# mcdermatt/ICET

Measured on AMD Instinct MI355X. Metric: scan-pairs/sec + ms/pair, 64-ch 75x24 voxels 7 iters; HBM GB/s vs peak, higher is better.
Workload: dtype f32; 1 GPU; configs[2]/[3]: 256 independent 64-ch synthetic scan pairs per GPU (~116k pts/scan, ring-major), 75x24 voxels, 7 iters, pair k -> rank k mod N, RCCL all-gather of 48 floats/pair when N>1; pairs_per_gpu=256, pairs_total=256, points_scan1_mean=116273, points_scan2_mean=116258, bins_theta=75, bins_phi=24, iters=7, parallelism=pairs round-robin x1, processes=1, mode=one process per GPU, rccl_ranks=0

## Files before the change

icet_amd/csrc/icet_accumulate.hip:

```cpp
#include <hip/hip_runtime.h>
#include <math.h>
#include "icet_internal.h"
#include "icet_device_common.h"
#include "icet_solve_body.h"
#include <algorithm>
#include <type_traits>

namespace icet {
namespace {

#ifndef ICET_ACC_BLOCK
#define ICET_ACC_BLOCK 512
#endif
#ifndef ICET_ACC_WAVES
#define ICET_ACC_WAVES 6
#endif
#ifndef ICET_ACC_PTS
#define ICET_ACC_PTS 4
#endif
static_assert(ICET_ACC_PTS == 4, "phase C of k_gn_accumulate is written for 4 consecutive points per lane");
constexpr int kAccPts = ICET_ACC_PTS;
constexpr int kAccBlock = ICET_ACC_BLOCK;
constexpr int kAccWavesPerSimd = ICET_ACC_WAVES;
constexpr int kHotWords = 8;

__device__ __noinline__ void spill_flush(uint32_t* A, uint32_t nraw, uint32_t nin, float S0, float S1, float S2, float S3, float S4,
                                         float S5, float S6, float S7, float S8) {
    acc_add_hbm(A, nraw, nin, S0, S1, S2, S3, S4, S5, S6, S7, S8);
}

__device__ __noinline__ void flush_wide(unsigned long long* F, float a0, float a1, float a2, float a3, float a4, float a5, float a6, float a7, float a8) {
    atomicAdd(&F[1], to_fix_wide_biased(a0)); atomicAdd(&F[2], to_fix_wide_biased(a1)); atomicAdd(&F[3], to_fix_wide_biased(a2)); atomicAdd(&F[4], to_fix_wide_biased(a3));
    atomicAdd(&F[5], to_fix_wide_biased(a4)); atomicAdd(&F[6], to_fix_wide_biased(a5)); atomicAdd(&F[7], to_fix_wide_biased(a6)); atomicAdd(&F[8], to_fix_wide_biased(a7));
    atomicAdd(&F[9], to_fix_wide_biased(a8));
}

constexpr int kCntBits = 21;
constexpr unsigned long long kCntMask = (1ull << kCntBits) - 1ull;
constexpr uint32_t kNearCap = 512;
constexpr uint32_t kNearCapSmall = 2048;

typedef __attribute__((address_space(1))) const float gfloat;
typedef float vfloat4 __attribute__((ext_vector_type(4)));
typedef __attribute__((address_space(1))) const vfloat4 gfloat4;

struct KeepDev { unsigned long long* mask; const uint32_t* list; const float* edges; const int32_t* modes; float c1, c2, capT, capP, invT; };
__device__ __forceinline__ int keep_pair_of_slot(const int32_t* __restrict__ modes, int n_pairs, int s, int& mode_word) {
    const int lane = (int)(threadIdx.x & 63u);
    const int gb = s & ~255, ng = min(256, n_pairs - gb), sl = s - gb;
    int m[4];
#pragma unroll
    for (int c = 0; c < 4; c++) m[c] = (c * 64 + lane < ng) ? modes[gb + c * 64 + lane] : -1;
    int hi = 0, lo = 0x7FFFFFFF;
#pragma unroll
    for (int c = 0; c < 4; c++) { hi = max(hi, m[c]); lo = min(lo, m[c] > 0 ? m[c] : 0x7FFFFFFF); }
    hi = wave_reduce_max_i(hi); lo = wave_reduce_min_i(lo);
    const float scale = 7.999f / (float)max(hi - lo + 1, 1);
    int cls[4], cnt[9];
#pragma unroll
    for (int k = 0; k < 9; k++) cnt[k] = 0;
#pragma unroll
    for (int c = 0; c < 4; c++) {
        cls[c] = m[c] < 0 ? 9 : (m[c] == 0 ? 0 : 1 + (int)((float)(hi - m[c]) * scale));
#pragma unroll
        for (int k = 0; k < 9; k++) cnt[k] += __popcll(__ballot(cls[c] == k));
    }
    int k_of = 0, r = sl;
#pragma unroll
    for (int k = 0; k < 8; k++) { const bool past = (k_of == k) & (r >= cnt[k]); r -= past ? cnt[k] : 0; k_of += past ? 1 : 0; }
    int found = -1, word = 0;
#pragma unroll
    for (int c = 0; c < 4; c++) {
        const unsigned long long bm = __ballot(cls[c] == k_of);
        const int rk = (int)__builtin_amdgcn_mbcnt_hi((uint32_t)(bm >> 32), __builtin_amdgcn_mbcnt_lo((uint32_t)bm, 0u));
        const unsigned long long hit = __ballot(cls[c] == k_of && rk == r);
        if (found < 0 && hit != 0ull) { const int l = __builtin_ctzll(hit); found = gb + c * 64 + l; word = __builtin_amdgcn_readlane(m[c], l); }
        r -= __popcll(bm);
    }
    mode_word = word;
    return found;
}
constexpr int kKeepOwn = 63;

template <bool kVec4, bool kRT2, bool kSmall, bool kKeep, bool kIdx = false>
__device__ __forceinline__ void gn_accumulate_body(const PairDesc* __restrict__ desc, const float* __restrict__ xf_all,
                                                          const int16_t* __restrict__ slot_of_voxel, const int32_t* __restrict__ n_slots,
                                                          const SlotHot* __restrict__ hotS, uint32_t* __restrict__ acc,
                                                          const float* __restrict__ thr, const LutCell* __restrict__ lut,
                                                          int T, int P, int Mt, int Mp, float guard_t, float guard_p,
                                                          int lds_slots, int chunks, int n_pairs, int force_exact,
                                                          uint32_t* __restrict__ near_over, uint32_t* __restrict__ near_over_count, const KeepDev& kd,
                                                          const int32_t* __restrict__ kf_of = nullptr) {
    constexpr uint32_t near_cap = kSmall ? kNearCapSmall : kNearCap;
    constexpr int kW = kAccBlock / 64;
    extern __shared__ __attribute__((aligned(16))) unsigned char smem[];
    const int V = T * P;
    int pair, chunk;
    if (!decode_block(n_pairs, chunks, pair, chunk)) return;
    [[maybe_unused]] int mode_word = 0;
    if constexpr (kKeep) { pair = keep_pair_of_slot(kd.modes, n_pairs, pair, mode_word); if (pair < 0) return; }
    const PairDesc d = desc[pair];
    int cs = (d.n2 + chunks - 1) / chunks;
    cs = (cs + kAccPts * 64 - 1) / (kAccPts * 64) * (kAccPts * 64);
    const int begin = chunk * cs;
    int list_mode = 0, nk = 0, tau_begin = 0, tau_end = 0;
    if constexpr (kKeep) { list_mode = mode_word > 0; nk = mode_word - 1; }
    if (kKeep && list_mode) {
        const int n_trips = nk / kKeepOwn + 1;
        int tpb = (n_trips + chunks - 1) / chunks; tpb = (tpb + kW - 1) / kW * kW;
        tau_begin = chunk * tpb; tau_end = min(n_trips, tau_begin + tpb);
        if (tau_begin >= n_trips) return;
    } else if (begin >= d.n2) return;
    const int end = (kKeep && list_mode) ? d.n2 : min(d.n2, begin + cs);
    const int lane = (int)(threadIdx.x & 63u);
    const uint32_t* L = kd.list + ((size_t)d.off2 >> 2) + pair;
    const int e_max = max(nk - 1, 0);
    auto entry_raw = [&](int tau) -> int { return (int)L[min(max(kKeepOwn * tau - 1 + lane, 0), e_max)]; };
    auto entry_ok = [&](int tau) -> bool { return (tau < tau_end) & ((unsigned)(kKeepOwn * tau - 1 + lane) < (unsigned)nk); };
    [[maybe_unused]] int gc_first = -1, gn_first = -1;
    if (kKeep && list_mode) { gc_first = entry_raw(tau_begin + (int)(threadIdx.x >> 6)); gn_first = entry_raw(tau_begin + (int)(threadIdx.x >> 6) + kW); }

    LutCell* lut_t = reinterpret_cast<LutCell*>(smem);
    LutCell* lut_p = lut_t + (Mt + 1);
    unsigned long long* lacc = reinterpret_cast<unsigned long long*>(lut_p + (Mp + 1));
    float* hot = reinterpret_cast<float*>(smem + (((size_t)(Mt + Mp + 2) * sizeof(LutCell) + (size_t)80 * lds_slots + 15) & ~(size_t)15));
    int16_t* map = reinterpret_cast<int16_t*>(hot + lds_slots * kHotWords);
    const int map_words = (V + 1) / 2;
    uint32_t* nearq = reinterpret_cast<uint32_t*>(map) + (V + T + 4) / 2;
    [[maybe_unused]] float* k_edge_t = reinterpret_cast<float*>(nearq + near_cap + 5);
    [[maybe_unused]] float* k_edge_p = k_edge_t + (T + 2);
    [[maybe_unused]] uint8_t* k_nb = reinterpret_cast<uint8_t*>(k_edge_p + (P + 2)) + T;
    int kf = pair;
    if constexpr (kIdx) kf = __builtin_amdgcn_readfirstlane(kf_of[pair]);
    const int ns = n_slots[kf];
    const int nl = min(ns, lds_slots);
    const SlotHot* hs = hotS + (size_t)kf * V;
    {
        const uint32_t* gm = reinterpret_cast<const uint32_t*>(slot_of_voxel + (size_t)kf * ((V + 1) & ~1));
        uint32_t* lm = reinterpret_cast<uint32_t*>(map);
        const uint2* gl = reinterpret_cast<const uint2*>(lut);
        uint2* ll = reinterpret_cast<uint2*>(lut_t);
        const int n_lut = Mt + Mp + 2;
        constexpr int kMapAhead = 2, kLutAhead = 3;
        uint32_t mreg[kMapAhead]; uint2 lreg[kLutAhead];
#pragma unroll
        for (int k = 0; k < kMapAhead; k++) { const int i = (int)threadIdx.x + k * kAccBlock; mreg[k] = (i < map_words) ? gm[i] : 0u; }
#pragma unroll
        for (int k = 0; k < kLutAhead; k++) { const int i = (int)threadIdx.x + k * kAccBlock; lreg[k] = (i < n_lut) ? gl[i] : make_uint2(0u, 0u); }
        SlotHot g0{};
        if ((int)threadIdx.x < nl) g0 = hs[threadIdx.x];
#pragma unroll
        for (int k = 0; k < kMapAhead; k++) { const int i = (int)threadIdx.x + k * kAccBlock; if (i < map_words) lm[i] = mreg[k]; }
        for (int i = (int)threadIdx.x + kMapAhead * kAccBlock; i < map_words; i += kAccBlock) lm[i] = gm[i];
        for (int i = 2 * map_words + threadIdx.x; i < V + T + 2; i += kAccBlock) map[i] = (int16_t)-1;
#pragma unroll
        for (int k = 0; k < kLutAhead; k++) { const int i = (int)threadIdx.x + k * kAccBlock; if (i < n_lut) ll[i] = lreg[k]; }
        for (int i = (int)threadIdx.x + kLutAhead * kAccBlock; i < n_lut; i += kAccBlock) ll[i] = gl[i];
        for (int i = threadIdx.x; i < nl; i += kAccBlock) {
            const SlotHot g = (i == (int)threadIdx.x) ? g0 : hs[i];
            float* h = hot + i * kHotWords;
            h[0] = g.inner; h[1] = g.outer; h[2] = g.mu[0]; h[3] = g.mu[1]; h[4] = g.mu[2];
        }
        for (int i = threadIdx.x; i < 10 * nl; i += kAccBlock) lacc[i] = 0ull;
        if (threadIdx.x < 5) nearq[near_cap + threadIdx.x] = 0u;
    }
    const float* xf = xf_all + pair * kXf;
    const float tx = xf[0], ty = xf[1], tz = xf[2];
    const float R00 = xf[3], R01 = xf[4], R02 = xf[5], R10 = xf[6], R11 = xf[7], R12 = xf[8], R20 = xf[9], R21 = xf[10], R22 = xf[11];
    const float cell_t = (float)Mt * 0.25f, cell_p = (float)Mp * 0.5f;
    __syncthreads();
    if constexpr (kKeep) {
        if (!list_mode) {
            for (int i = threadIdx.x; i < T + P + 4; i += kAccBlock) {
                const int k = i < T + 2 ? i : i - (T + 2);
                k_edge_t[i] = (i < T + 2) ? kd.edges[min(k, T)] : kd.edges[T + 1 + min(k, P)];
            }
            for (int v = (int)threadIdx.x - T; v < V + 2 * T + 1; v += kAccBlock) {
                uint32_t code = 0u;
                if (v >= 0 && v < V) {
                    const int bt = v % T, r0 = v - bt;
                    code = (map[v] >= 0 ? 1u : 0u) | (map[r0 + (bt == 0 ? T - 1 : bt - 1)] >= 0 ? 2u : 0u) | (map[r0 + (bt == T - 1 ? 0 : bt + 1)] >= 0 ? 4u : 0u);
                }
                k_nb[v] = (uint8_t)code;
            }
            __syncthreads();
        }
    }

    gfloat* px = (gfloat*)d.s2; gfloat* py = px + d.ld2; gfloat* pz = px + 2 * (size_t)d.ld2;
    uint32_t* gacc = acc + (size_t)pair * V * kAccWords;

    auto load4 = [&](int i0, float (&X)[4], float (&Y)[4], float (&Z)[4]) {
        if (kVec4 && i0 + 3 < end) {
            const vfloat4 a = __builtin_nontemporal_load((gfloat4*)(px + i0)), b = __builtin_nontemporal_load((gfloat4*)(py + i0)), c = __builtin_nontemporal_load((gfloat4*)(pz + i0));
            X[0] = a.x; X[1] = a.y; X[2] = a.z; X[3] = a.w; Y[0] = b.x; Y[1] = b.y; Y[2] = b.z; Y[3] = b.w; Z[0] = c.x; Z[1] = c.y; Z[2] = c.z; Z[3] = c.w;
        } else {
#pragma unroll
            for (int j = 0; j < 4; j++) { const bool ok = i0 + j < end; X[j] = ok ? px[i0 + j] : __builtin_nanf(""); Y[j] = ok ? py[i0 + j] : 0.f; Z[j] = ok ? pz[i0 + j] : 0.f; }
        }
    };
#ifndef ICET_ACC_PHASE
#define ICET_ACC_PHASE 9
#endif
    [[maybe_unused]] float sink = 0.f;
    float XN[4], YN[4], ZN[4];
    auto trip = [&](auto mode_c, const int i0, const bool have_next, const int i0_next, [[maybe_unused]] const int grp) {
      constexpr int kMode = decltype(mode_c)::value;
      [[maybe_unused]] const bool ghost = kMode == 2 && lane == 0;
      auto flush = [&](int slot, uint32_t cr, uint32_t ci, float a0, float a1, float a2, float a3, float a4, float a5, float a6, float a7, float a8) {
          if (ICET_ACC_PHASE == 4) { sink += (float)(slot + (int)cr + (int)ci) + a0 + a1 + a2 + a3 + a4 + a5 + a6 + a7 + a8; return; }
          if (slot >= 0) {
              if (slot < nl) {
                  unsigned long long* F = lacc + slot * 10;
                  atomicAdd(&F[0], (unsigned long long)cr | ((unsigned long long)ci << kCntBits) | ((ci ? 1ull : 0ull) << (2 * kCntBits)));
                  if (ci) {
                      if (__ballot(!(fmaxf(fmaxf(a3, a6), a8) < kFixFastMax)) == 0ull) {
                          atomicAdd(&F[1], to_fix_biased(a0)); atomicAdd(&F[2], to_fix_biased(a1)); atomicAdd(&F[3], to_fix_biased(a2)); atomicAdd(&F[4], to_fix_biased(a3));
                          atomicAdd(&F[5], to_fix_biased(a4)); atomicAdd(&F[6], to_fix_biased(a5)); atomicAdd(&F[7], to_fix_biased(a6)); atomicAdd(&F[8], to_fix_biased(a7));
                          atomicAdd(&F[9], to_fix_biased(a8));
                      } else {
                          flush_wide(F, a0, a1, a2, a3, a4, a5, a6, a7, a8);
                      }
                  }
              } else {
                  spill_flush(gacc + (size_t)slot * kAccWords, cr, ci, a0, a1, a2, a3, a4, a5, a6, a7, a8);
              }
          }
      };
      {
        PointClass pc[4];
        float QX[4], QY[4], QZ[4], RR[4];
        {
            typedef float f2 __attribute__((ext_vector_type(2)));
            f2 q[6];
#pragma unroll
            for (int h = 0; h < 2; h++) {
                const f2 a = f2{XN[2 * h], XN[2 * h + 1]} + f2{tx, tx}, b = f2{YN[2 * h], YN[2 * h + 1]} + f2{ty, ty}, c = f2{ZN[2 * h], ZN[2 * h + 1]} + f2{tz, tz};
                q[3 * h + 0] = __builtin_elementwise_fma(c, f2{R20, R20}, __builtin_elementwise_fma(b, f2{R10, R10}, a * f2{R00, R00}));
                q[3 * h + 1] = __builtin_elementwise_fma(c, f2{R21, R21}, __builtin_elementwise_fma(b, f2{R11, R11}, a * f2{R01, R01}));
                q[3 * h + 2] = __builtin_elementwise_fma(c, f2{R22, R22}, __builtin_elementwise_fma(b, f2{R12, R12}, a * f2{R02, R02}));
            }
            asm volatile("" : "+v"(q[0]), "+v"(q[1]), "+v"(q[2]), "+v"(q[3]), "+v"(q[4]), "+v"(q[5]) : : "memory");
#pragma unroll
            for (int h = 0; h < 2; h++) { QX[2 * h] = q[3 * h].x; QX[2 * h + 1] = q[3 * h].y; QY[2 * h] = q[3 * h + 1].x; QY[2 * h + 1] = q[3 * h + 1].y; QZ[2 * h] = q[3 * h + 2].x; QZ[2 * h + 1] = q[3 * h + 2].y; }
        }
        if (have_next) load4(i0_next, XN, YN, ZN);
        if (ICET_ACC_PHASE == 0) { sink += (QX[0] + QX[1] + QX[2] + QX[3]) + (QY[0] + QY[1] + QY[2] + QY[3]) + (QZ[0] + QZ[1] + QZ[2] + QZ[3]); return; }
        int SM[4];
        bool nr[4];
        float R2[4];
        [[maybe_unused]] bool keep_any = false;
#pragma unroll
        for (int j = 0; j < 4; j++) {
            const float qx = QX[j], qy = QY[j], qz = QZ[j];
            const float r2 = qx * qx + qy * qy + qz * qz;
            const float rs = __builtin_amdgcn_rsqf(r2);
            RR[j] = r2 * rs;
            const float w = -qz * rs;
            const float q1 = qy * __builtin_amdgcn_rcpf(fabsf(qx) + fabsf(qy));
            const float pa = (qx >= 0.f) ? ((qy >= 0.f) ? q1 : 4.f + q1) : 2.f - q1;
            const LutCell et = lut_t[static_cast<int>(pa * cell_t)];
            const LutCell ep = lut_p[static_cast<int>((w + 1.f) * cell_p)];
            const int bt = et.idx - ((pa < et.edge) ? 1 : 0);
            const int row = ep.idx - ((w < ep.edge) ? T : 0);
            SM[j] = map[row + bt];
            nr[j] = (force_exact != 0) | !(fabsf(pa - et.edge) >= guard_t) | !(fabsf(w - ep.edge) >= guard_p);
            R2[j] = r2;
            if constexpr (kMode == 1) {
                const float irho = __builtin_amdgcn_rsqf(fmaf(qx, qx, qy * qy));
                const float Mpol = fmaf(kd.c2, rs, kd.c1), Maz = fmaf(kd.c1, RR[j], kd.c2) * irho;
                const float lo_t = k_edge_t[bt], hi_t = k_edge_t[bt + 1];
                const int bpi = static_cast<int>(fmaf((float)row, kd.invT, 0.5f));
                const float lo_p = k_edge_p[bpi], hi_p = k_edge_p[bpi + 1];
                const bool nlt = !((pa - lo_t) >= Maz), nht = !((hi_t - pa) >= Maz), nlp = !((w - lo_p) >= Mpol), nhp = !((hi_p - w) >= Mpol);
                const bool unsure = !(Maz <= kd.capT) | !(Mpol <= kd.capP) | (bt >= T) | (row >= V) | nr[j] | !((r2 >= kR2Min) & (r2 <= kR2Max));
                const int v = row + bt;
                const uint32_t c0 = k_nb[v], cm = k_nb[v - T], cp = k_nb[v + T];
                const uint32_t msk = 1u | (nlt ? 2u : 0u) | (nht ? 4u : 0u);
                const uint32_t hit = (c0 & msk) | (nlp ? (cm & msk) : 0u) | (nhp ? (cp & msk) : 0u);
                keep_any |= (i0 + j < end) & (unsure | (hit != 0u));
            }
        }
        if constexpr (kMode == 1) {
            const unsigned long long km = __ballot(keep_any);
            if (lane == 0 && i0 < end) kd.mask[((size_t)d.off2 >> 8) + pair + (i0 >> 8)] = km;
        }
#pragma unroll
        for (int j = 0; j < 4; j++) nr[j] |= !((R2[j] >= kR2Min) & (R2[j] <= kR2Max));
        const int E0 = nr[0] ? -1 : SM[0], E1 = nr[1] ? -1 : SM[1], E2 = nr[2] ? -1 : SM[2], E3 = nr[3] ? -1 : SM[3];
        if (ICET_ACC_PHASE == 1) { sink += (float)(E0 + E1 + E2 + E3) + RR[0] + RR[1] + RR[2] + RR[3] + QX[0] + QY[1] + QZ[2]; return; }
        if (__ballot((E0 & E1 & E2 & E3) >= 0) != 0ull) {
            const bool beyond = __ballot(max(max(E0, E1), max(E2, E3)) >= nl) != 0ull;
            const int E[4] = {E0, E1, E2, E3};
#pragma unroll
            for (int j = 0; j < 4; j++) {
                const int sm = E[j];
                const bool has = sm >= 0;
                const float* h = hot + min(max(sm, 0), lds_slots - 1) * kHotWords;
                float inner = h[0], outer = h[1], m0 = h[2], m1 = h[3], m2 = h[4];
                if (beyond) {
                    if (sm >= nl) { const SlotHot g = hs[sm]; inner = g.inner; outer = g.outer; m0 = g.mu[0]; m1 = g.mu[1]; m2 = g.mu[2]; }
                    asm volatile("" : "+v"(inner), "+v"(outer), "+v"(m0), "+v"(m1), "+v"(m2));
                }
                const float r = RR[j];
                const float gr = 1e-6f * r;
                const float m = fminf(r - inner, outer - r);
                const bool edge = has & !(fabsf(m) >= gr);
                nr[j] |= edge;
                pc[j].s = edge ? -1 : sm;
                pc[j].inb = has & (m >= 0.f);
                float ux = QX[j], uy = QY[j], uz = QZ[j];
                if (kRT2) { if (pc[j].inb & !edge) roundtrip_any(ux, uy, uz, ux, uy, uz); }
                pc[j].dx = ux - m0; pc[j].dy = uy - m1; pc[j].dz = uz - m2;
            }
        } else {
#pragma unroll
            for (int j = 0; j < 4; j++) { pc[j].s = -1; pc[j].inb = false; pc[j].dx = pc[j].dy = pc[j].dz = 0.f; }
        }
        if (ICET_ACC_PHASE == 2) { for (int j = 0; j < 4; j++) sink += (float)pc[j].s + pc[j].dx + pc[j].dy + pc[j].dz + (pc[j].inb ? 1.f : 0.f) + (nr[j] ? 1.f : 0.f); return; }
        if (__ballot(nr[0] | nr[1] | nr[2] | nr[3]) != 0ull) {
            if (__ballot((R2[0] == 0.f) | (R2[1] == 0.f) | (R2[2] == 0.f) | (R2[3] == 0.f)) != 0ull) {
#pragma unroll
                for (int j = 0; j < 4; j++) {
                    const bool zq = (R2[j] == 0.f) & (QX[j] == 0.f) & (QY[j] == 0.f) & (i0 + j < end);
                    const bool zc = zq & !ghost;
                    const int patt = (__builtin_signbit(QY[j]) ? 2 : 0) | (__builtin_signbit(QX[j]) ? 1 : 0);
#pragma unroll
                    for (int k = 0; k < 4; k++) {
                        const unsigned long long m = __ballot(zc & (patt == k));
                        if (m != 0ull && (threadIdx.x & 63) == 0) atomicAdd(&nearq[near_cap + 1 + k], (uint32_t)__popcll(m));
                    }
                    nr[j] &= !zq;
                }
            }
#pragma unroll
            for (int j = 0; j < 4; j++) {
                if (nr[j] & (i0 + j < end) & !ghost) {
                    const uint32_t e = atomicAdd(&nearq[near_cap], 1u);
                    if (e < near_cap) nearq[e] = (uint32_t)(i0 + j);
                    else near_over[(size_t)d.off2 + atomicAdd(&near_over_count[pair], 1u)] = (uint32_t)(i0 + j);
                }
            }
        }
        if (ICET_ACC_PHASE == 3) { for (int j = 0; j < 4; j++) sink += (float)pc[j].s + pc[j].dx + pc[j].dy + pc[j].dz + (pc[j].inb ? 1.f : 0.f); return; }
        const int s0 = pc[0].s, s1 = pc[1].s, s2 = pc[2].s, s3 = pc[3].s;
        if (__ballot((s0 >= 0) | (s1 >= 0) | (s2 >= 0) | (s3 >= 0)) == 0ull) return;
        {
            const bool e1 = s1 == s0, e2 = s2 == s1, e3 = s3 == s2;
            const bool a1 = e1, a2 = a1 & e2, a3 = a2 & e3;
            const bool z3 = !a3, z2 = z3 & e3, z1 = z2 & e2;
            const bool i0 = pc[0].inb, i1 = pc[1].inb, i2 = pc[2].inb, i3 = pc[3].inb;
            typedef float f2 __attribute__((ext_vector_type(2)));
            const uint32_t zr = 1u + (z2 ? 1u : 0u) + (z1 ? 1u : 0u);
            const uint32_t zi = (i3 ? 1u : 0u) + ((z2 & i2) ? 1u : 0u) + ((z1 & i1) ? 1u : 0u);
            bool fw = z3 & (s3 >= 0) & (wave_shl1(s0, -2) == s3);
            if constexpr (kMode == 2) fw &= (wave_shl1(grp, -7) == grp + 1) & (((grp + 1) & 63) != 0);
            const bool h1 = fw & z1 & i1, h2 = fw & z2 & i2, h3 = fw & i3;
            const float g1x = wave_shr1_zero(h1 ? pc[1].dx : 0.f), g1y = wave_shr1_zero(h1 ? pc[1].dy : 0.f), g1z = wave_shr1_zero(h1 ? pc[1].dz : 0.f);
            const float g2x = wave_shr1_zero(h2 ? pc[2].dx : 0.f), g2y = wave_shr1_zero(h2 ? pc[2].dy : 0.f), g2z = wave_shr1_zero(h2 ? pc[2].dz : 0.f);
            const float g3x = wave_shr1_zero(h3 ? pc[3].dx : 0.f), g3y = wave_shr1_zero(h3 ? pc[3].dy : 0.f), g3z = wave_shr1_zero(h3 ? pc[3].dz : 0.f);
            const uint32_t gc = (uint32_t)wave_shr1_zero((int)(fw ? (zr | (zi << 8)) : 0u));
            f2 Axy, Asq, Acz; float A2, A4, A8;
            {
                Axy = f2{g1x, g1y}; A2 = g1z; Asq = Axy * Axy; Acz = f2{g1z, g1z} * Axy; A4 = g1x * g1y; A8 = g1z * g1z;
            }
#define ICET_ACC_ADD(S, vx_, vy_, vz_)                                                                                                       \
            {                                                                                                                                \
                const f2 vxy = f2{vx_, vy_}; const float vz = vz_;                                                                           \
                S##xy += vxy; S##2 += vz;                                                                                                    \
                S##sq = __builtin_elementwise_fma(vxy, vxy, S##sq); S##cz = __builtin_elementwise_fma(vxy, f2{vz, vz}, S##cz);               \
                S##4 = fmaf(vxy.x, vxy.y, S##4); S##8 = fmaf(vz, vz, S##8);                                                                  \
            }
            ICET_ACC_ADD(A, g2x, g2y, g2z)
            ICET_ACC_ADD(A, g3x, g3y, g3z)
            { const bool m = i0;      ICET_ACC_ADD(A, m ? pc[0].dx : 0.f, m ? pc[0].dy : 0.f, m ? pc[0].dz : 0.f) }
            { const bool m = a1 & i1; ICET_ACC_ADD(A, m ? pc[1].dx : 0.f, m ? pc[1].dy : 0.f, m ? pc[1].dz : 0.f) }
            { const bool m = a2 & i2; ICET_ACC_ADD(A, m ? pc[2].dx : 0.f, m ? pc[2].dy : 0.f, m ? pc[2].dz : 0.f) }
            { const bool m = a3 & i3; ICET_ACC_ADD(A, m ? pc[3].dx : 0.f, m ? pc[3].dy : 0.f, m ? pc[3].dz : 0.f) }
            const float A0 = Axy.x, A1 = Axy.y, A3 = Asq.x, A6 = Asq.y, A5 = Acz.x, A7 = Acz.y;
            const uint32_t ar = 1u + (a1 ? 1u : 0u) + (a2 ? 1u : 0u) + (a3 ? 1u : 0u) + (gc & 0xFFu);
            const uint32_t ai = (i0 ? 1u : 0u) + ((a1 & i1) ? 1u : 0u) + ((a2 & i2) ? 1u : 0u) + ((a3 & i3) ? 1u : 0u) + (gc >> 8);
            flush(ghost ? -1 : s0, ar, ai, A0, A1, A2, A3, A4, A5, A6, A7, A8);
            if (__ballot(z3 & (s3 >= 0) & !fw) != 0ull) {
                f2 Zxy, Zsq, Zcz; float Z2, Z4, Z8;
                { const bool m = z1 & i1; const float x = m ? pc[1].dx : 0.f, y = m ? pc[1].dy : 0.f, z = m ? pc[1].dz : 0.f;
                  Zxy = f2{x, y}; Z2 = z; Zsq = Zxy * Zxy; Zcz = f2{z, z} * Zxy; Z4 = x * y; Z8 = z * z; }
                { const bool m = z2 & i2; ICET_ACC_ADD(Z, m ? pc[2].dx : 0.f, m ? pc[2].dy : 0.f, m ? pc[2].dz : 0.f) }
                { const bool m = i3;      ICET_ACC_ADD(Z, m ? pc[3].dx : 0.f, m ? pc[3].dy : 0.f, m ? pc[3].dz : 0.f) }
                flush((z3 & !fw & !(kMode == 2 && lane == 63)) ? s3 : -1, zr, zi, Zxy.x, Zxy.y, Z2, Zsq.x, Z4, Zcz.x, Zsq.y, Zcz.y, Z8);
            }
#undef ICET_ACC_ADD
            const bool m1 = !a1 & !z1, m2 = !a2 & !z2;
            if (__ballot((m1 & (s1 >= 0)) | (m2 & (s2 >= 0))) != 0ull) {
                const bool joint = m1 & m2 & e2;
                const float bx = i1 ? pc[1].dx : 0.f, by = i1 ? pc[1].dy : 0.f, bz = i1 ? pc[1].dz : 0.f;
                const float cx = i2 ? pc[2].dx : 0.f, cy = i2 ? pc[2].dy : 0.f, cz = i2 ? pc[2].dz : 0.f;
                if (m1 & !joint) flush(ghost ? -1 : s1, 1u, i1 ? 1u : 0u, bx, by, bz, bx * bx, bx * by, bx * bz, by * by, by * bz, bz * bz);
                if (m2) {
                    const float jx = joint ? bx : 0.f, jy = joint ? by : 0.f, jz = joint ? bz : 0.f;
                    flush(ghost ? -1 : s2, joint ? 2u : 1u, (i2 ? 1u : 0u) + ((joint & i1) ? 1u : 0u), jx + cx, jy + cy, jz + cz,
                          fmaf(cx, cx, jx * jx), fmaf(cx, cy, jx * jy), fmaf(cx, cz, jx * jz), fmaf(cy, cy, jy * jy), fmaf(cy, cz, jy * jz), fmaf(cz, cz, jz * jz));
                }
            }
        }
      }
    };
    if (kKeep && list_mode) {
        int tau = tau_begin + (int)(threadIdx.x >> 6);
        int gc = gc_first, gn_raw = gn_first;
        gc = entry_ok(tau) ? gc : -1;
        load4(gc >= 0 ? 4 * gc : end, XN, YN, ZN);
        for (; tau < tau_end; tau += kW) {
            const int gnn_raw = entry_raw(tau + 2 * kW);
            const int gn = entry_ok(tau + kW) ? gn_raw : -1;
            trip(std::integral_constant<int, 2>{}, gc >= 0 ? 4 * gc : end, tau + kW < tau_end, gn >= 0 ? 4 * gn : end, gc);
            gc = gn; gn_raw = gnn_raw;
        }
    } else {
        load4(begin + kAccPts * (int)threadIdx.x, XN, YN, ZN);
        for (int t0 = begin + kAccPts * threadIdx.x; t0 < begin + cs; t0 += kAccPts * kAccBlock)
            trip(std::integral_constant<int, kKeep ? 1 : 0>{}, t0, t0 + kAccPts * kAccBlock < begin + cs, t0 + kAccPts * kAccBlock, -1);
    }
    if (ICET_ACC_PHASE != 9 && sink == 1.2345e-30f) near_over_count[pair] = 1u;
    __syncthreads();
    {
        const uint32_t nq = min(nearq[near_cap], near_cap);
        for (uint32_t e = threadIdx.x; e < nq; e += kAccBlock) {
            const int i = (int)nearq[e];
            float qx, qy, qz;
            transform_point(px[i], py[i], pz[i], xf, qx, qy, qz);
            PointClass pc1;
            classify_literal(qx, qy, qz, map, thr, T, P, hs, pc1, kRT2);
            if (pc1.s >= 0) {
                const float dx = pc1.dx, dy = pc1.dy, dz = pc1.dz;
                unsigned long long* F = lacc + min(pc1.s, nl > 0 ? nl - 1 : 0) * 10;
                if (pc1.s < nl) {
                    atomicAdd(&F[0], 1ull | ((unsigned long long)(pc1.inb ? 1u : 0u) << kCntBits));
                    if (pc1.inb) {
                        atomicAdd(&F[1], to_fix(dx)); atomicAdd(&F[2], to_fix(dy)); atomicAdd(&F[3], to_fix(dz));
                        atomicAdd(&F[4], to_fix(dx * dx)); atomicAdd(&F[5], to_fix(dx * dy)); atomicAdd(&F[6], to_fix(dx * dz));
                        atomicAdd(&F[7], to_fix(dy * dy)); atomicAdd(&F[8], to_fix(dy * dz)); atomicAdd(&F[9], to_fix(dz * dz));
                    }
                } else {
                    acc_add_hbm(gacc + (size_t)pc1.s * kAccWords, 1u, pc1.inb ? 1u : 0u, dx, dy, dz, dx * dx, dx * dy, dx * dz, dy * dy, dy * dz, dz * dz);
                }
            }
        }
        if (threadIdx.x < 4 && nearq[near_cap + 1 + threadIdx.x] != 0u) {
            PointClass pz;
            classify_literal((threadIdx.x & 1) ? -0.f : 0.f, (threadIdx.x & 2) ? -0.f : 0.f, 0.f, map, thr, T, P, hs, pz, false);
            const uint32_t cnt = nearq[near_cap + 1 + threadIdx.x];
            if (pz.s >= 0) {
                if (pz.s < nl) atomicAdd(&lacc[pz.s * 10], (unsigned long long)cnt);
                else atomicAdd(reinterpret_cast<unsigned long long*>(gacc + (size_t)pz.s * kAccWords), (unsigned long long)cnt);
            }
        }
    }
    __syncthreads();
    for (int s = threadIdx.x; s < nl; s += kAccBlock) {
        const unsigned long long* L = lacc + s * 10;
        const unsigned long long cnt = L[0];
        const unsigned long long raw = cnt & kCntMask, in = (cnt >> kCntBits) & kCntMask, conv = cnt >> (2 * kCntBits);
        if (raw == 0ull) continue;
        unsigned long long* G = reinterpret_cast<unsigned long long*>(gacc + (size_t)s * kAccWords);
        atomicAdd(&G[0], raw | (in << 32));
        if (in) {
            const unsigned long long bias = conv * kFixBias;
#pragma unroll
            for (int k = 1; k < 10; k++) atomicAdd(&G[k], L[k] - bias);
        }
    }
}

template <bool kVec4, bool kRT2, bool kSmall>
__global__ __launch_bounds__(kAccBlock, kRT2 ? 1 : (kSmall ? 2 : kAccWavesPerSimd)) void k_gn_accumulate(const PairDesc* __restrict__ desc, const float* __restrict__ xf_all,
                                                          const int16_t* __restrict__ slot_of_voxel, const int32_t* __restrict__ n_slots,
                                                          const SlotHot* __restrict__ hotS, uint32_t* __restrict__ acc,
                                                          const float* __restrict__ thr, const LutCell* __restrict__ lut,
                                                          int T, int P, int Mt, int Mp, float guard_t, float guard_p,
                                                          int lds_slots, int chunks, int n_pairs, int force_exact,
                                                          uint32_t* __restrict__ near_over, uint32_t* __restrict__ near_over_count) {
    gn_accumulate_body<kVec4, kRT2, kSmall, false>(desc, xf_all, slot_of_voxel, n_slots, hotS, acc, thr, lut, T, P, Mt, Mp, guard_t, guard_p, lds_slots, chunks, n_pairs, force_exact, near_over, near_over_count, KeepDev{});
}

template <bool kVec4, bool kRT2, bool kSmall>
__global__ __launch_bounds__(kAccBlock, kRT2 ? 1 : (kSmall ? 2 : kAccWavesPerSimd)) void k_gn_accumulate_indexed(const PairDesc* __restrict__ desc, const float* __restrict__ xf_all,
                                                          const int16_t* __restrict__ slot_of_voxel, const int32_t* __restrict__ n_slots,
                                                          const SlotHot* __restrict__ hotS, uint32_t* __restrict__ acc,
                                                          const float* __restrict__ thr, const LutCell* __restrict__ lut,
                                                          int T, int P, int Mt, int Mp, float guard_t, float guard_p,
                                                          int lds_slots, int chunks, int n_pairs, int force_exact,
                                                          uint32_t* __restrict__ near_over, uint32_t* __restrict__ near_over_count, const int32_t* __restrict__ kf_of) {
    gn_accumulate_body<kVec4, kRT2, kSmall, false, true>(desc, xf_all, slot_of_voxel, n_slots, hotS, acc, thr, lut, T, P, Mt, Mp, guard_t, guard_p, lds_slots, chunks, n_pairs, force_exact, near_over, near_over_count, KeepDev{}, kf_of);
}

template <bool kVec4>
__global__ __launch_bounds__(kAccBlock, kAccWavesPerSimd) void k_gn_accumulate_keep(const PairDesc* __restrict__ desc, const float* __restrict__ xf_all,
                                                          const int16_t* __restrict__ slot_of_voxel, const int32_t* __restrict__ n_slots,
                                                          const SlotHot* __restrict__ hotS, uint32_t* __restrict__ acc,
                                                          const float* __restrict__ thr, const LutCell* __restrict__ lut,
                                                          int T, int P, int Mt, int Mp, float guard_t, float guard_p,
                                                          int lds_slots, int chunks, int n_pairs, int force_exact,
                                                          uint32_t* __restrict__ near_over, uint32_t* __restrict__ near_over_count, KeepDev kd) {
    gn_accumulate_body<kVec4, false, false, true>(desc, xf_all, slot_of_voxel, n_slots, hotS, acc, thr, lut, T, P, Mt, Mp, guard_t, guard_p, lds_slots, chunks, n_pairs, force_exact, near_over, near_over_count, kd);
}

struct SolveFuse { const SlotFit* fitS; float* X; float* out; AuxDev aux; int n, iter, runlen, reject_moving; float cond_bound2; uint32_t* done; };
template <bool kVec4>
__global__ __launch_bounds__(kAccBlock, 2) void k_gn_accumulate_solve(const PairDesc* desc, float* xf_all, const int16_t* slot_of_voxel, const int32_t* n_slots,
                                                                      const SlotHot* hotS, uint32_t* acc, const float* thr, const LutCell* lut,
                                                                      int T, int P, int Mt, int Mp, float guard_t, float guard_p,
                                                                      int lds_slots, int chunks, int n_pairs, int force_exact,
                                                                      uint32_t* near_over, uint32_t* near_over_count, SolveFuse sf) {
    gn_accumulate_body<kVec4, false, true, false>(desc, xf_all, slot_of_voxel, n_slots, hotS, acc, thr, lut, T, P, Mt, Mp, guard_t, guard_p, lds_slots, chunks, n_pairs, force_exact, near_over, near_over_count, KeepDev{});
    int pair, chunk;
    if (!decode_block(n_pairs, chunks, pair, chunk)) return;
    __shared__ uint32_t s_last;
    __builtin_amdgcn_fence(__ATOMIC_RELEASE, "workgroup");
    __syncthreads();
    if (threadIdx.x == 0) {
        __builtin_amdgcn_fence(__ATOMIC_RELEASE, "agent");
        const uint32_t t = atomicAdd(&sf.done[pair], 1u);
        s_last = (t == (uint32_t)chunks - 1u) ? 1u : 0u;
        if (s_last) { sf.done[pair] = 0u; __builtin_amdgcn_fence(__ATOMIC_ACQUIRE, "agent"); }
    }
    __syncthreads();
    if (!s_last) return;
    __builtin_amdgcn_fence(__ATOMIC_ACQUIRE, "workgroup");
    const NearOverflow over{desc, slot_of_voxel, hotS, thr, near_over, near_over_count, T, P, 0};
    gn_solve_body<256, 0, kAccBlock, true>(n_slots, sf.fitS, acc, sf.X, xf_all, sf.out, sf.aux, T * P, sf.n, sf.iter, sf.runlen, over, sf.reject_moving, nullptr, 1, sf.cond_bound2, KeepArgs{}, pair);
}

inline int chunks_for(int n_pairs, int max_n, int per_block_min, int target_blocks) {
    int by_work = (max_n + per_block_min - 1) / per_block_min;
    int want = (target_blocks + n_pairs - 1) / n_pairs;
    int c = want < by_work ? want : by_work;
    return c < 1 ? 1 : c;
}

}

#define ICET_LAUNCH_CHECK() do { hipError_t e_ = hipGetLastError(); if (e_ != hipSuccess) return e_; } while (0)

hipError_t init_accumulate_kernels() {
    hipError_t e = hipSuccess;
#define ICET_ACC_ATTR(V4, RT, SM) if (e == hipSuccess) e = hipFuncSetAttribute(reinterpret_cast<const void*>(k_gn_accumulate<V4, RT, SM>), hipFuncAttributeMaxDynamicSharedMemorySize, 160 * 1024)
    ICET_ACC_ATTR(true, false, false); ICET_ACC_ATTR(false, false, false); ICET_ACC_ATTR(true, true, false); ICET_ACC_ATTR(false, true, false);
    ICET_ACC_ATTR(true, false, true); ICET_ACC_ATTR(false, false, true); ICET_ACC_ATTR(true, true, true); ICET_ACC_ATTR(false, true, true);
#undef ICET_ACC_ATTR
#define ICET_ACC_ATTR(V4, RT, SM) if (e == hipSuccess) e = hipFuncSetAttribute(reinterpret_cast<const void*>(k_gn_accumulate_indexed<V4, RT, SM>), hipFuncAttributeMaxDynamicSharedMemorySize, 160 * 1024)
    ICET_ACC_ATTR(true, false, false); ICET_ACC_ATTR(false, false, false); ICET_ACC_ATTR(true, true, false); ICET_ACC_ATTR(false, true, false);
    ICET_ACC_ATTR(true, false, true); ICET_ACC_ATTR(false, false, true); ICET_ACC_ATTR(true, true, true); ICET_ACC_ATTR(false, true, true);
#undef ICET_ACC_ATTR
    if (e == hipSuccess) e = hipFuncSetAttribute(reinterpret_cast<const void*>(k_gn_accumulate_keep<true>), hipFuncAttributeMaxDynamicSharedMemorySize, 160 * 1024);
    if (e == hipSuccess) e = hipFuncSetAttribute(reinterpret_cast<const void*>(k_gn_accumulate_keep<false>), hipFuncAttributeMaxDynamicSharedMemorySize, 160 * 1024);
    if (e == hipSuccess) e = hipFuncSetAttribute(reinterpret_cast<const void*>(k_gn_accumulate_solve<true>), hipFuncAttributeMaxDynamicSharedMemorySize, 150 * 1024);
    if (e == hipSuccess) e = hipFuncSetAttribute(reinterpret_cast<const void*>(k_gn_accumulate_solve<false>), hipFuncAttributeMaxDynamicSharedMemorySize, 150 * 1024);
    return e;
}

__global__ __launch_bounds__(kBlock) void k_rt2_prepare(const PairDesc* __restrict__ desc, const PairDesc* __restrict__ desc_rt, int n_pairs, int chunks) {
    int pair, chunk;
    if (!decode_block(n_pairs, chunks, pair, chunk)) return;
    const PairDesc d = desc[pair], o = desc_rt[pair];
    float* ox = const_cast<float*>(o.s2); float* oy = ox + o.ld2; float* oz = ox + 2 * (size_t)o.ld2;
    const float* px = d.s2; const float* py = px + d.ld2; const float* pz = px + 2 * (size_t)d.ld2;
    int cs = (d.n2 + chunks - 1) / chunks; cs = (cs + kBlock - 1) / kBlock * kBlock;
    const int lo = chunk * cs, hi = min(d.n2, lo + cs);
    for (int i = lo + threadIdx.x; i < hi; i += kBlock) {
        float x, y, z;
        roundtrip_any(px[i], py[i], pz[i], x, y, z);
        ox[i] = x; oy[i] = y; oz[i] = z;
    }
}

hipError_t launch_rt2_prepare(const Workspace& w, const LaunchCfg& c, hipStream_t st) {
    const int chunks = std::max(1, std::min(64, (c.max_n2 + 4 * kBlock - 1) / (4 * kBlock)));
    k_rt2_prepare<<<grid_groups(c.n_pairs) * chunks, kBlock, 0, st>>>(w.desc, w.desc_rt, c.n_pairs, chunks);
    ICET_LAUNCH_CHECK();
    return hipSuccess;
}

size_t acc_fixed_lds_bytes(int T, int P, int Mt, int Mp, bool small_batch, bool keep) {
    const uint32_t near_cap = small_batch ? kNearCapSmall : kNearCap;
    const size_t keep_bytes = keep ? (size_t)(T + P + 4) * 4 + (((size_t)T * P + 3 * (size_t)T + 1 + 3) & ~(size_t)3) : 0;
    return (size_t)(Mt + Mp + 2) * sizeof(LutCell) + (size_t)(((size_t)T * P + T + 4) / 2) * 4 + (near_cap + 5) * 4 + 32 + keep_bytes;
}
size_t acc_row_lds_bytes() { return (kHotWords + kAccLds) * 4; }

hipError_t launch_gn_accumulate(const Workspace& w, const LaunchCfg& c, hipStream_t st, const FuseArgs* fuse, bool* fused, int keep_pass) {
    if (fused) *fused = false;
    if ((keep_pass || fuse) && c.kf_of) return hipErrorInvalidValue;
    if (keep_pass && (c.n_pairs < 32 || c.rt2 || !w.keep_state || !w.keep_mask || !w.keep_list || !w.edges || !w.keep_modes)) return hipErrorInvalidValue;
    const uint32_t near_cap = (c.n_pairs >= 32) ? kNearCap : kNearCapSmall;
    const size_t fixed = acc_fixed_lds_bytes(c.T, c.P, w.lut_Mt, w.lut_Mp, near_cap == kNearCapSmall, keep_pass != 0);
    const size_t row = acc_row_lds_bytes();
    const bool fuse_it = fuse && c.fuse_solve && near_cap == kNearCapSmall && c.V <= 4096 && !c.rt2 && c.ref_w && w.gn_done() && fixed + 32 * row <= (size_t)148 * 1024;
    const size_t budget = (c.n_pairs >= 32) ? fixed + 320 * row : (fuse_it ? 144 : 156) * 1024;
    int lds_slots = c.lds_slots > 0 ? c.lds_slots : (int)((budget > fixed ? budget - fixed : 0) / row);
    lds_slots = lds_slots < 32 ? 32 : lds_slots;
    const int fit = (int)(((fuse_it ? 148 : 160) * 1024 - fixed) / row);
    if (lds_slots > fit) lds_slots = fit;
    if (lds_slots > c.V) lds_slots = c.V;
    int chunks = chunks_for(c.n_pairs, c.max_n2, kAccBlock * c.acc_min_pts_per_thread, c.acc_target_blocks);
    chunks = std::max(chunks, (int)(((long long)c.max_n2 + (1 << 20) - 1) >> 20));
    const size_t lds = fixed + (size_t)lds_slots * row;
    dim3 grid(grid_groups(c.n_pairs) * chunks), blk(kAccBlock);
    const LutCell* lut = reinterpret_cast<const LutCell*>(w.lut);
#define ICET_ACC_LAUNCH(V4, RT, SM) do { if (c.kf_of) k_gn_accumulate_indexed<V4, RT, SM><<<grid, blk, lds, st>>>(w.desc, w.xf, w.slot_of_voxel, w.n_slots, w.hotS, w.acc, w.thr, lut, c.T, c.P, w.lut_Mt, w.lut_Mp, \
                                                     w.guard_t, w.guard_p, lds_slots, chunks, c.n_pairs, c.force_exact, w.near_over, w.near_over_count, c.kf_of); \
                                      else k_gn_accumulate<V4, RT, SM><<<grid, blk, lds, st>>>(w.desc, w.xf, w.slot_of_voxel, w.n_slots, w.hotS, w.acc, w.thr, lut, c.T, c.P, w.lut_Mt, w.lut_Mp, \
                                                     w.guard_t, w.guard_p, lds_slots, chunks, c.n_pairs, c.force_exact, w.near_over, w.near_over_count); } while (0)
    if (fuse_it) {
        AuxDev aux{}; if (fuse->aux) aux = *fuse->aux;
        aux.pair_user = c.pair_user; aux.done_flag = (fuse->iter == c.runlen - 1) ? c.done_flag : nullptr;
        aux.done_count = aux.done_flag ? w.done_count() : nullptr; aux.done_pairs = c.n_pairs;
        const SolveFuse sf{w.fitS, w.X, fuse->d_out, aux, c.n, fuse->iter, c.runlen, c.reject_moving, c.gn_cond_bound2, w.gn_done()};
        if (c.vec4_ok) k_gn_accumulate_solve<true><<<grid, blk, lds, st>>>(w.desc, w.xf, w.slot_of_voxel, w.n_slots, w.hotS, w.acc, w.thr, lut, c.T, c.P, w.lut_Mt, w.lut_Mp, w.guard_t, w.guard_p, lds_slots, chunks, c.n_pairs, c.force_exact, w.near_over, w.near_over_count, sf);
        else k_gn_accumulate_solve<false><<<grid, blk, lds, st>>>(w.desc, w.xf, w.slot_of_voxel, w.n_slots, w.hotS, w.acc, w.thr, lut, c.T, c.P, w.lut_Mt, w.lut_Mp, w.guard_t, w.guard_p, lds_slots, chunks, c.n_pairs, c.force_exact, w.near_over, w.near_over_count, sf);
        ICET_LAUNCH_CHECK();
        if (fused) *fused = true;
        return hipSuccess;
    }
    if (keep_pass) {
        const double two_pi = 6.283185307179586476925286766559;
        const KeepDev kd{w.keep_mask, w.keep_list, w.edges, w.keep_modes + (size_t)(keep_pass >> 1) * c.n_pairs, 1.05f * c.keep_br + 1e-4f, 1.05f * c.keep_bt,
                         (float)std::min(two_pi / c.T, 0.5), (float)std::min(0.5 * two_pi / c.P, 0.5), 1.0f / (float)c.T};
        if (c.vec4_ok) k_gn_accumulate_keep<true><<<grid, blk, lds, st>>>(w.desc, w.xf, w.slot_of_voxel, w.n_slots, w.hotS, w.acc, w.thr, lut, c.T, c.P, w.lut_Mt, w.lut_Mp, w.guard_t, w.guard_p, lds_slots, chunks, c.n_pairs, c.force_exact, w.near_over, w.near_over_count, kd);
        else k_gn_accumulate_keep<false><<<grid, blk, lds, st>>>(w.desc, w.xf, w.slot_of_voxel, w.n_slots, w.hotS, w.acc, w.thr, lut, c.T, c.P, w.lut_Mt, w.lut_Mp, w.guard_t, w.guard_p, lds_slots, chunks, c.n_pairs, c.force_exact, w.near_over, w.near_over_count, kd);
        ICET_LAUNCH_CHECK();
        return hipSuccess;
    }
#define ICET_ACC_LAUNCH2(V4, RT) do { if (near_cap == kNearCapSmall) ICET_ACC_LAUNCH(V4, RT, true); else ICET_ACC_LAUNCH(V4, RT, false); } while (0)
    if (c.rt2) { if (c.vec4_ok) ICET_ACC_LAUNCH2(true, true); else ICET_ACC_LAUNCH2(false, true); }
    else { if (c.vec4_ok) ICET_ACC_LAUNCH2(true, false); else ICET_ACC_LAUNCH2(false, false); }
#undef ICET_ACC_LAUNCH2
#undef ICET_ACC_LAUNCH
    ICET_LAUNCH_CHECK();
    return hipSuccess;
}

}
```

icet_amd/csrc/icet_capi.hip:

```cpp
#include "../../include/icet_hip.h"
#include "../../include/icet_nodes.h"
#include "icet_internal.h"
#include "icet_layout.h"
#include "icet_closure.h"
#include "icet_appearance.h"

#include <hip/hip_runtime.h>
#include <cstdio>
#include <cstdlib>
#include <cmath>
#include <cstring>
#include <string>
#include <vector>
#include <algorithm>
#include <cstdint>
#include <new>
#include <atomic>

using namespace icet;

struct icet_ctx {
    int device = 0;
    hipStream_t stream = nullptr;
    bool own_stream = false;
    Workspace w;
    Tuning tune;
    int32_t kf_pairs = 0; icet_params kf_params{};
    int max_lds = 160 * 1024;
    int lds_rank_ok = 0;
    std::string err;
    PairDesc* h_desc = nullptr; int32_t* h_seg = nullptr; int32_t h_cap_pairs = 0;
    bool desc_kf_valid = false, desc_reg_valid = false;
    PairDesc* h_desc_rt = nullptr; int32_t h_cap_rt = 0;
    PairDesc* h_desc_reg = nullptr; int32_t* h_kf_of = nullptr;
    int64_t ws_gen = 0;
    float* d_stage1 = nullptr; float* d_stage2 = nullptr; int64_t cap_stage1 = 0, cap_stage2 = 0;
    float* d_out = nullptr; float* d_x0 = nullptr; int32_t cap_out_pairs = 0;
    float* h_out = nullptr;
    AuxDev aux_dev{}; int aux_V = 0, aux_runlen = 0;
    uint32_t* d_pack = nullptr; uint32_t* h_pack = nullptr; size_t cap_pack = 0;
    float* h_pts2 = nullptr; float* d_pts2 = nullptr; size_t cap_pts2 = 0;
    float* h_x0 = nullptr;
    icet_score* d_score = nullptr; icet_score* h_score = nullptr; int32_t cap_score = 0;
    int32_t* d_sel = nullptr; int32_t* h_sel = nullptr; int64_t cap_sel = 0;
    hipEvent_t ev_sel = nullptr; bool sel_in_flight = false;
    float* d_sph1 = nullptr; int32_t* d_idx1 = nullptr; size_t cap_side1 = 0;
    float* d_sph2 = nullptr; int32_t* d_vox2 = nullptr; size_t cap_side2 = 0;
    hipStream_t st_copy = nullptr; hipEvent_t ev_s2 = nullptr;
    hipEvent_t ev_kf = nullptr, ev_kfd = nullptr, ev_prev = nullptr, ev_pts2 = nullptr;
    struct Pending { bool active = false; float* x_out = nullptr; float* ps_out = nullptr; float* cov_out = nullptr; icet_aux aux{}; bool has_aux = false;
                     int V = 0, rl = 0; int64_t n2 = 0; bool kf_tables = false, kf_done = false, pts2 = false, pts2_dev = false, tail_ints = false, side1 = false, side2 = false; int64_t n1 = 0;
                     const float* scan2 = nullptr; int64_t ld2 = 0; } pend;
    hipEvent_t ev_a = nullptr, ev_b = nullptr, ev_c = nullptr;
    std::vector<hipEvent_t> ev_acc;
    float last_ms[4] = {0, 0, 0, 0};
    bool timing_valid = false;
    int last_iters = 0;
    std::vector<icet_ctx*> helpers;
    hipEvent_t ev_fork = nullptr, ev_join = nullptr;
    hipEvent_t ev_stage = nullptr; int stage_at = 0;
    hipEvent_t ev_desc = nullptr; bool desc_in_flight = false;
    struct GraphKey { int64_t v[47]; };
    struct GraphSlot { hipGraph_t graph = nullptr; hipGraphExec_t exec = nullptr; GraphKey key{}, seen{}; bool have_seen = false, have_graph = false; };
    bool capturing = false; int graph_mode = -1;
    GraphSlot g_solve, g_keyframe, g_loop, g_indexed;
    GraphSlot g_scored, g_score;
    hipEvent_t ev_graph = nullptr; bool graph_in_flight = false;
    bool perm_active = false; int32_t perm_pairs = 0;
    hipError_t (*prologue)(void*, hipStream_t) = nullptr; void* prologue_user = nullptr; int64_t prologue_key = 0;
    int32_t* done_flag = nullptr;
    int32_t* h_sync_word = nullptr; int armed_calls = 2;
};

struct icet_keyframe_store {
    icet_ctx* ctx = nullptr;
    icet_params shape{};
    int V = 0; int32_t capacity = 0;
    SlotHot* hotS = nullptr; SlotFit* fitS = nullptr; int16_t* slot_of_voxel = nullptr; int32_t* n_slots = nullptr;
    std::vector<uint8_t> occupied;
    int64_t id = 0, gen = 0;
    std::string err;
    int64_t* pose_stamp = nullptr;
    PoseTable pose_table() const { return PoseTable{pose_stamp, reinterpret_cast<float*>(pose_stamp + capacity), capacity}; }
    PoseUpload* h_pose = nullptr; int32_t cap_h_pose = 0; hipEvent_t ev_pose = nullptr; bool pose_in_flight = false;
    unsigned long long* q_part = nullptr; size_t cap_part = 0;
    unsigned long long* q_keys = nullptr; int32_t* q_cand = nullptr; int32_t cap_qk = 0;
    float* q_x0 = nullptr; float* q_out = nullptr; icet_score* q_score = nullptr; int32_t* q_kf_of = nullptr; int32_t* q_rows = nullptr; int32_t* q_members = nullptr; int32_t cap_qr = 0;
    int32_t* q_offs = nullptr; int32_t* q_best = nullptr;
    struct Appearance {
        icet_appearance_rule::Consts k{}; int Rp = 0;
        uint32_t* desc = nullptr; float* w = nullptr; int32_t* has = nullptr;
        std::vector<uint8_t> has_h;
        uint32_t* scratch = nullptr;
        uint32_t* qdesc = nullptr; float* qw = nullptr; int32_t* qhas = nullptr;
        unsigned long long* keys_all = nullptr; uint16_t* shift_all = nullptr; size_t cap_all = 0;
        int32_t* shift_of = nullptr;
    };
    Appearance* app = nullptr;
    AppTable app_table() const { return AppTable{app->desc, app->w, app->has, capacity, app->k.A, app->Rp}; }
};

namespace {

#define HIPCHK(ctx, call) do { hipError_t e_ = (call); if (e_ != hipSuccess) { \
    (ctx)->err = std::string(#call) + ": " + hipGetErrorString(e_); \
    return e_ == hipErrorOutOfMemory ? ICET_ERR_NOMEM : ICET_ERR_HIP; } } while (0)

template <typename T> hipError_t dev_realloc(T*& p, size_t count) {
    if (p) { hipError_t e = hipFree(p); p = nullptr; if (e != hipSuccess) return e; }
    if (count == 0) return hipSuccess;
    return hipMalloc(reinterpret_cast<void**>(&p), count * sizeof(T));
}

bool params_ok(const icet_params* p) {
    if (!p) return false;
    if (p->runlen < 0 || p->runlen > 4096) return false;
    if (p->bins_phi <= 0 || p->bins_theta <= 0 || p->n < 1) return false;
    return true;
}

icet_status ensure_regs(icet_ctx* c, int32_t n_regs, int V) {
    Workspace& w = c->w;
    if (n_regs <= w.cap_regs && V <= w.cap_reg_V) return ICET_OK;
    const int np = n_regs > w.cap_regs ? n_regs : w.cap_regs;
    const int VV = V > w.cap_reg_V ? V : w.cap_reg_V;
    const size_t pv = (size_t)np * VV;
    HIPCHK(c, hipStreamSynchronize(c->stream));
    HIPCHK(c, dev_realloc(w.acc, pv * kAccWords));
    HIPCHK(c, hipMemset(w.acc, 0, pv * kAccWords * sizeof(uint32_t)));
    HIPCHK(c, dev_realloc(w.near_over_count, 2 * (size_t)np + 1));
    HIPCHK(c, hipMemset(w.near_over_count, 0, (2 * (size_t)np + 1) * sizeof(uint32_t)));
    HIPCHK(c, dev_realloc(w.xf, (size_t)np * 48));
    HIPCHK(c, dev_realloc(w.X, (size_t)np * 6));
    HIPCHK(c, dev_realloc(w.desc_reg, np));
    HIPCHK(c, dev_realloc(w.kf_of, (size_t)np + 1));
    if (c->h_desc_reg) { HIPCHK(c, hipHostFree(c->h_desc_reg)); c->h_desc_reg = nullptr; }
    if (c->h_kf_of) { HIPCHK(c, hipHostFree(c->h_kf_of)); c->h_kf_of = nullptr; }
    HIPCHK(c, hipHostMalloc(reinterpret_cast<void**>(&c->h_desc_reg), sizeof(PairDesc) * np));
    HIPCHK(c, hipHostMalloc(reinterpret_cast<void**>(&c->h_kf_of), sizeof(int32_t) * ((size_t)np + 1)));
    w.cap_regs = np; w.cap_reg_V = VV;
    c->ws_gen++;
    return ICET_OK;
}

icet_status ensure_scan2(icet_ctx* c, int64_t total_n2) {
    Workspace& w = c->w;
    if (total_n2 >= (int64_t)1 << 31) { c->err = "total scan-2 points per call must be < 2^31"; return ICET_ERR_UNSUPPORTED; }
    if (total_n2 > w.cap_n2) {
        HIPCHK(c, hipStreamSynchronize(c->stream));
        HIPCHK(c, dev_realloc(w.near_over, (size_t)total_n2));
        w.cap_n2 = total_n2;
        c->ws_gen++;
    }
    return ICET_OK;
}

icet_status ensure_workspace(icet_ctx* c, const icet_params* p, int32_t n_pairs, int64_t total_n1, int64_t total_n2) {
    Workspace& w = c->w;
    const int V = p->bins_phi * p->bins_theta;
    if ((int64_t)p->bins_phi * p->bins_theta > kMaxVoxels) { c->err = "bins_phi*bins_theta exceeds the voxel limit (10000: the multi-split keeps 12 B per voxel, the Gauss-Newton pass a 2-byte map entry and its look-up tables, in one block's LDS)"; return ICET_ERR_UNSUPPORTED; }
    if ((size_t)V * 12 + 8 + 4096 > (size_t)c->max_lds) { c->err = "grid too fine for this device's LDS (k_bin_scatter keeps 12 B per voxel in one block)"; return ICET_ERR_UNSUPPORTED; }
    if (total_n1 >= (int64_t)1 << 31) { c->err = "total scan-1 points per call must be < 2^31"; return ICET_ERR_UNSUPPORTED; }
    const bool grow_pairs = n_pairs > w.cap_pairs || V > w.cap_V;
    if (grow_pairs) {
        c->kf_pairs = 0;
        const int np = n_pairs > w.cap_pairs ? n_pairs : w.cap_pairs;
        const int VV = V > w.cap_V ? V : w.cap_V;
        const size_t pv = (size_t)np * VV;
        HIPCHK(c, hipStreamSynchronize(c->stream));
        HIPCHK(c, dev_realloc(w.desc, np));
        HIPCHK(c, dev_realloc(w.seg_off, 2 * (size_t)np + 1));
        HIPCHK(c, dev_realloc(w.bin_count, pv));
        HIPCHK(c, dev_realloc(w.bin_start, (size_t)np * (VV + 1)));
        HIPCHK(c, dev_realloc(w.live_bins, pv * 4)); HIPCHK(c, dev_realloc(w.n_live, np));
        HIPCHK(c, dev_realloc(w.hotD, pv)); HIPCHK(c, dev_realloc(w.fitD, pv)); HIPCHK(c, dev_realloc(w.activeD, pv)); HIPCHK(c, dev_realloc(w.midD, pv));
        HIPCHK(c, dev_realloc(w.hotS, pv)); HIPCHK(c, dev_realloc(w.fitS, pv));
        HIPCHK(c, dev_realloc(w.slot_of_voxel, (size_t)np * ((VV + 1) & ~1)));
        HIPCHK(c, dev_realloc(w.n_slots, np));
        HIPCHK(c, dev_realloc(w.gn_part, (size_t)kGnPartWords));
        HIPCHK(c, dev_realloc(w.flags, np));
        HIPCHK(c, dev_realloc(w.zero_rows, (size_t)np * 4));
        HIPCHK(c, dev_realloc(w.vrange, (size_t)np * 2));
        HIPCHK(c, dev_realloc(w.splitters, (size_t)np * kRankSortMaxBuckets)); HIPCHK(c, dev_realloc(w.n_buckets, np)); HIPCHK(c, dev_realloc(w.bucket_start, (size_t)np * (kRankSortMaxBuckets + 1)));
        if (c->h_desc) { HIPCHK(c, hipHostFree(c->h_desc)); c->h_desc = nullptr; }
        if (c->h_seg) { HIPCHK(c, hipHostFree(c->h_seg)); c->h_seg = nullptr; }
        HIPCHK(c, hipHostMalloc(reinterpret_cast<void**>(&c->h_desc), sizeof(PairDesc) * np));
        std::memset(c->h_desc, 0, sizeof(PairDesc) * np); c->desc_kf_valid = c->desc_reg_valid = false;
        HIPCHK(c, hipHostMalloc(reinterpret_cast<void**>(&c->h_seg), sizeof(int32_t) * (2 * (size_t)np + 1)));
        c->h_cap_pairs = np;
        w.cap_pairs = np; w.cap_V = VV;
        c->ws_gen++;
    }
    { const icet_status rs = ensure_regs(c, n_pairs, V); if (rs != ICET_OK) return rs; }
    { const icet_status ss = ensure_scan2(c, total_n2); if (ss != ICET_OK) return ss; }
    if (total_n1 > w.cap_n1 || grow_pairs) {
        c->ws_gen++;
        const int64_t n = total_n1 > w.cap_n1 ? total_n1 : w.cap_n1;
        HIPCHK(c, hipStreamSynchronize(c->stream));
        if (n > w.cap_n1) {
            c->kf_pairs = 0;
            HIPCHK(c, dev_realloc(w.r1, n)); HIPCHK(c, dev_realloc(w.cart1, (size_t)3 * n));
            HIPCHK(c, dev_realloc(w.key64A, n)); HIPCHK(c, dev_realloc(w.key64B, n)); HIPCHK(c, dev_realloc(w.bin16, n)); HIPCHK(c, dev_realloc(w.binpos, n)); HIPCHK(c, dev_realloc(w.bkt, n));
            HIPCHK(c, dev_realloc(w.keyA, n)); HIPCHK(c, dev_realloc(w.keyB, n)); HIPCHK(c, dev_realloc(w.valA, n)); HIPCHK(c, dev_realloc(w.valB, n));
            HIPCHK(c, dev_realloc(w.pred, n)); HIPCHK(c, dev_realloc(w.src, n));
            w.cap_n1 = n;
        }
        HIPCHK(c, dev_realloc(w.execbits, (size_t)(w.cap_n1 / 64 + w.cap_pairs + 2)));
        {
            const size_t need_items = (size_t)(w.cap_n1 / 64 + (int64_t)w.cap_pairs * (w.cap_V + 1) + 64);
            if (need_items > w.cap_fit_items) {
                if (w.fit_items) { HIPCHK(c, hipFree(w.fit_items)); w.fit_items = nullptr; }
                HIPCHK(c, hipMalloc(&w.fit_items, need_items * 16));
                w.cap_fit_items = need_items;
            }
            HIPCHK(c, dev_realloc(w.fit_n_items, (size_t)w.cap_pairs));
        }
#ifdef ICET_DIAG_LIBSORT
        const size_t need = sort_temp_bytes(w.cap_n1);
        if (need > w.sort_tmp_bytes) {
            if (w.sort_tmp) { HIPCHK(c, hipFree(w.sort_tmp)); w.sort_tmp = nullptr; }
            HIPCHK(c, hipMalloc(&w.sort_tmp, need));
            w.sort_tmp_bytes = need;
        }
#endif
    }
    return ICET_OK;
}

void build_thresholds(int nb, double period, float* out) {
    auto bin = [&](float t) { return static_cast<long long>(((double)t / period) * nb); };
    out[0] = 0.f;
    for (int k = 1; k <= nb; k++) {
        float t = (float)(period * (double)k / (double)nb);
        while (bin(t) >= k) t = std::nextafterf(t, -INFINITY);
        while (bin(t) < k) t = std::nextafterf(t, INFINITY);
        out[k] = t;
    }
}

struct HostCell { float edge; int32_t idx; };
int build_lut(const std::vector<double>& edges, double lo, double range, double quantile, double guard, std::vector<HostCell>& out, int max_cells = 1 << 16) {
    std::vector<double> widths;
    for (size_t k = 1; k < edges.size(); k++) widths.push_back(edges[k] - edges[k - 1]);
    std::sort(widths.begin(), widths.end());
    const double w_ref = widths.empty() ? range : widths[(size_t)(quantile * (double)(widths.size() - 1))];
    int M = 64;
    while (range / M > 0.45 * w_ref && 2 * M <= max_cells) M *= 2;
    out.resize(M);
    const double cw = range / M, slack = 0.02 * cw + guard;
    for (int c = 0; c < M; c++) {
        const double ctr = lo + (c + 0.5) * cw;
        size_t best = 0;
        for (size_t k = 1; k < edges.size(); k++) if (std::fabs(edges[k] - ctr) < std::fabs(edges[best] - ctr)) best = k;
        const double e = edges[best];
        const double h0 = std::min(lo + c * cw - slack, e) - guard, h1 = std::max(lo + (c + 1) * cw + slack, e) + guard;
        bool ambiguous = false;
        for (size_t k = 0; k < edges.size(); k++) if (k != best && edges[k] >= h0 && edges[k] <= h1) ambiguous = true;
        out[c].edge = ambiguous ? std::nanf("") : (float)e; out[c].idx = (int32_t)best;
    }
    return M;
}

icet_status ensure_thresholds(icet_ctx* c, int T, int P) {
    Workspace& w = c->w;
    if (w.thr && w.thr_T == T && w.thr_P == P) return ICET_OK;
    HIPCHK(c, hipStreamSynchronize(c->stream));
    {
        std::vector<double> et(T + 1), ep(P + 1);
        for (int k = 0; k <= T; k++) {
            const double th = 2 * M_PI * k / T, x = std::cos(th), y = std::sin(th), q = y / (std::fabs(x) + std::fabs(y));
            et[k] = (k == T) ? 4.0 : (k == 0 ? 0.0 : (x >= 0 ? (y >= 0 ? q : 4.0 + q) : 2.0 - q));
        }
        for (int k = 0; k <= P; k++) ep[k] = (k == 0) ? -1.0 : (k == P ? 1.0 : -std::cos(M_PI * k / P));
        w.guard_t = 5e-6f * (float)c->tune.guard_scale; w.guard_p = 2.5e-6f * (float)c->tune.guard_scale;
        std::vector<HostCell> lt, lp;
        const double qp = c->tune.lut_polar_quantile;
        int cap_t = 1 << 16, cap_p = 1 << 16, Mt = 0, Mp = 0;
        for (;;) {
            Mt = build_lut(et, 0.0, 4.0, 0.0, w.guard_t, lt, cap_t); Mp = build_lut(ep, -1.0, 2.0, qp, w.guard_p, lp, cap_p);
            const size_t need_acc = acc_fixed_lds_bytes(T, P, Mt, Mp, true) + 32 * acc_row_lds_bytes();
            const size_t need_scan1 = (size_t)(Mt + Mp + 2) * sizeof(HostCell) + 4096;
            if (std::max(need_acc, need_scan1) <= (size_t)c->max_lds) break;
            if (Mt <= 64 && Mp <= 64) { c->err = "grid too fine for this device's LDS (voxel map + look-up tables of one block)"; return ICET_ERR_UNSUPPORTED; }
            if (Mt >= Mp) cap_t = Mt / 2; else cap_p = Mp / 2;
        }
        for (HostCell& c : lp) c.idx *= T;
        std::vector<HostCell> all(lt); all.push_back(HostCell{4.0f, T}); all.insert(all.end(), lp.begin(), lp.end()); all.push_back(HostCell{1.0f, P * T});
        if (w.lut) { HIPCHK(c, hipFree(w.lut)); w.lut = nullptr; }
        HIPCHK(c, hipMalloc(&w.lut, all.size() * sizeof(HostCell)));
        HIPCHK(c, hipMemcpy(w.lut, all.data(), all.size() * sizeof(HostCell), hipMemcpyHostToDevice));
        w.lut_Mt = Mt; w.lut_Mp = Mp;
        std::vector<float> ef; for (double e : et) ef.push_back((float)e); for (double e : ep) ef.push_back((float)e);
        HIPCHK(c, dev_realloc(w.edges, ef.size()));
        HIPCHK(c, hipMemcpy(w.edges, ef.data(), ef.size() * sizeof(float), hipMemcpyHostToDevice));
    }
    std::vector<float> h((size_t)T + P + 2);
    build_thresholds(T, 2 * M_PI, h.data());
    build_thresholds(P, M_PI, h.data() + T + 1);
    HIPCHK(c, dev_realloc(w.thr, h.size()));
    HIPCHK(c, hipMemcpy(w.thr, h.data(), h.size() * sizeof(float), hipMemcpyHostToDevice));
    for (int k = 0; k < 4; k++) {
        float th = (float)std::atan2((k & 2) ? -0.0 : 0.0, (k & 1) ? -0.0 : 0.0);
        if (th < 0.0f) th = (float)((double)th + 2.0 * M_PI);
        const float ph = 1000.0f;
        const int bt = static_cast<int>(((double)th / (2.0 * M_PI)) * (double)T) % T, bp = static_cast<int>(((double)ph / M_PI) * (double)P) % P;
        w.zero_voxel[k] = T * bp + bt;
    }
    w.thr_T = T; w.thr_P = P;
    return ICET_OK;
}

icet_status ensure_out(icet_ctx* c, int32_t n_pairs) {
    if (n_pairs <= c->cap_out_pairs) return ICET_OK;
    HIPCHK(c, hipStreamSynchronize(c->stream));
    HIPCHK(c, dev_realloc(c->d_out, (size_t)n_pairs * 48));
    HIPCHK(c, dev_realloc(c->d_x0, (size_t)n_pairs * 6));
    if (c->h_out) { HIPCHK(c, hipHostFree(c->h_out)); c->h_out = nullptr; }
    if (c->h_x0) { HIPCHK(c, hipHostFree(c->h_x0)); c->h_x0 = nullptr; }
    HIPCHK(c, hipHostMalloc(reinterpret_cast<void**>(&c->h_out), sizeof(float) * 48 * (size_t)n_pairs));
    HIPCHK(c, hipHostMalloc(reinterpret_cast<void**>(&c->h_x0), sizeof(float) * 6 * (size_t)n_pairs));
    c->cap_out_pairs = n_pairs;
    return ICET_OK;
}

icet_status ensure_host_path(icet_ctx* c) {
    if (!c->st_copy) HIPCHK(c, hipStreamCreateWithFlags(&c->st_copy, hipStreamNonBlocking));
    for (hipEvent_t* e : {&c->ev_s2, &c->ev_kf, &c->ev_kfd, &c->ev_prev, &c->ev_pts2})
        if (!*e) HIPCHK(c, hipEventCreateWithFlags(e, hipEventDisableTiming));
    return ICET_OK;
}

hipError_t upload_scan(float* dst, int64_t l, const float* src, int64_t n, int64_t ld, hipStream_t st) {
    if (n <= 0) return hipSuccess;
    return hipMemcpy2DAsync(dst, l * sizeof(float), src, ld * sizeof(float), n * sizeof(float), 3, hipMemcpyHostToDevice, st);
}

#define ICET_POINTS2_BODY                                                                                                     \
    const float tx = xf[0], ty = xf[1], tz = xf[2];                                                                           \
    const float R00 = xf[3], R01 = xf[4], R02 = xf[5], R10 = xf[6], R11 = xf[7], R12 = xf[8], R20 = xf[9], R21 = xf[10], R22 = xf[11]; \
    const float* __restrict__ px = s; const float* __restrict__ py = s + ld; const float* __restrict__ pz = s + 2 * ld;      \
    float* __restrict__ ox = out; float* __restrict__ oy = out + n; float* __restrict__ oz = out + 2 * n;                    \
    for (int64_t i = 0; i < n; i++) {                                                                                         \
        const float a = px[i] + tx, b = py[i] + ty, c = pz[i] + tz;                                                           \
        ox[i] = a * R00 + b * R10 + c * R20; oy[i] = a * R01 + b * R11 + c * R21; oz[i] = a * R02 + b * R12 + c * R22;       \
    }
#if defined(__x86_64__)
__attribute__((target("avx2,fma"))) void host_points2_avx2(const float* xf, const float* s, int64_t ld, int64_t n, float* out) { ICET_POINTS2_BODY }
#endif
void host_points2(const float* xf, const float* s, int64_t ld, int64_t n, float* out) {
#if defined(__x86_64__)
    if (__builtin_cpu_supports("avx2") && __builtin_cpu_supports("fma")) { host_points2_avx2(xf, s, ld, n, out); return; }
#endif
    ICET_POINTS2_BODY
}
#undef ICET_POINTS2_BODY

struct AuxLayout { size_t out, xf_last, x_hist, htwh, htwdz, cond, small_end, bounds, has_fit, mu1, sigma1, evecs1, l_diag, test_points, kf_end, n1_raw, n2_raw, n2_in, ints_end, total; };
AuxLayout aux_layout(int V, int runlen) {
    AuxLayout L{}; size_t o = 0;
    auto take = [&o](size_t n) { const size_t at = o; o += (n + 3) & ~(size_t)3; return at; };
    const size_t rl = runlen > 0 ? runlen : 1, v = (size_t)V;
    L.out = take(48); L.x_hist = take(rl * 6); L.htwh = take(rl * 36); L.htwdz = take(rl * 6); L.cond = take(rl * 8); L.small_end = o; L.xf_last = take(48);
    L.bounds = take(v * 6); L.has_fit = take(v); L.mu1 = take(v * 3); L.sigma1 = take(v * 9); L.evecs1 = take(v * 9); L.l_diag = take(v * 3);
    L.test_points = take(v * 18); L.kf_end = o; L.n1_raw = take(v); L.n2_raw = take(rl * v); L.n2_in = take(rl * v); L.ints_end = o;
    L.total = o;
    return L;
}

void free_aux(icet_ctx* c) {
    if (c->d_pack) { (void)hipFree(c->d_pack); c->d_pack = nullptr; }
    if (c->h_pack) { (void)hipHostFree(c->h_pack); c->h_pack = nullptr; }
    c->cap_pack = 0;
    c->aux_dev = AuxDev{};
    c->aux_V = 0; c->aux_runlen = 0;
}

icet_status ensure_pack(icet_ctx* c, int V, int runlen) {
    const AuxLayout L = aux_layout(V, runlen);
    if (L.total > c->cap_pack) {
        HIPCHK(c, hipStreamSynchronize(c->stream));
        free_aux(c);
        HIPCHK(c, dev_realloc(c->d_pack, L.total));
        HIPCHK(c, hipHostMalloc(reinterpret_cast<void**>(&c->h_pack), L.total * sizeof(uint32_t)));
        c->cap_pack = L.total;
    }
    if (c->aux_V != V || c->aux_runlen != runlen) {
        AuxDev& a = c->aux_dev; uint32_t* d = c->d_pack;
        auto F = [d](size_t at) { return reinterpret_cast<float*>(d + at); };
        auto I = [d](size_t at) { return reinterpret_cast<int32_t*>(d + at); };
        float* hs = reinterpret_cast<float*>(c->h_pack);
        a.bounds = F(L.bounds); a.n1_raw = I(L.n1_raw); a.has_fit = I(L.has_fit); a.mu1 = F(L.mu1); a.sigma1 = F(L.sigma1); a.evecs1 = F(L.evecs1);
        a.l_diag = F(L.l_diag); a.x_hist = F(L.x_hist); a.htwh = F(L.htwh); a.htwdz = F(L.htwdz); a.cond = F(L.cond); a.n2_raw = I(L.n2_raw); a.n2_in = I(L.n2_in);
        a.test_points = F(L.test_points); a.xf_last = hs + L.xf_last;
        c->aux_V = V; c->aux_runlen = runlen;
    }
    return ICET_OK;
}

LaunchCfg make_cfg(icet_ctx* c, const icet_params* p, int32_t n_pairs, PairDesc* hd = nullptr, int32_t* hs = nullptr) {
    if (!hd) { hd = c->h_desc; hs = c->h_seg; }
    LaunchCfg cfg{};
    cfg.T = p->bins_theta; cfg.P = p->bins_phi; cfg.V = cfg.T * cfg.P; cfg.n = p->n; cfg.runlen = p->runlen;
    cfg.thresh = p->thresh; cfg.buff = p->buff; cfg.n_pairs = n_pairs;
    cfg.half_gap = (p->flags & ICET_FLAG_HALF_GAP_BOUNDS) ? 1 : 0;
    cfg.true_sort = (p->flags & (ICET_FLAG_TRUE_SORT | ICET_FLAG_HALF_GAP_BOUNDS)) ? 1 : 0;
    cfg.reject_moving = (p->flags & ICET_FLAG_REJECT_MOVING) ? 1 : 0;
    cfg.rt2 = (p->flags & ICET_FLAG_ROUNDTRIP_SCAN2) ? 1 : 0;
    cfg.ref_w = (p->flags & ICET_FLAG_DOUBLE_W) ? 0 : 1;
    cfg.lds_slots = c->tune.lds_slots; cfg.acc_min_pts_per_thread = c->tune.acc_pts; cfg.acc_target_blocks = c->tune.acc_blocks;
    cfg.force_exact = c->tune.force_exact; cfg.use_library_sort = c->tune.library_sort; cfg.kf_pts_per_thread = c->tune.kf_pts; cfg.rs_cap = c->tune.rs_cap; cfg.rs_max_cell = c->tune.rs_max_cell; cfg.exec_bits_lds = c->tune.exec_bits_lds; cfg.exec_pairwise = c->tune.exec_pairwise; cfg.fuse_solve = c->tune.fuse_solve != 0 ? 1 : 0; cfg.lds_rank = (c->tune.lds_rank != 0 && c->lds_rank_ok) ? 1 : 0;
    cfg.gn_cond_bound2 = (float)(c->tune.gn_cond_bound * c->tune.gn_cond_bound);
    cfg.pair_user = (c->perm_active && c->perm_pairs == n_pairs) ? c->w.seg_off + n_pairs + 1 : nullptr;
    cfg.done_flag = c->done_flag;
    cfg.keep_from = c->tune.keep_from < 0 ? 0 : c->tune.keep_from; cfg.keep_bt = (float)c->tune.keep_budget_t; cfg.keep_br = (float)c->tune.keep_budget_r; cfg.keep_check_scale = (float)c->tune.keep_check_scale;
    cfg.keep = (c->tune.keep != 0 && n_pairs >= 32 && !cfg.rt2 && p->runlen >= cfg.keep_from + 3 && c->w.lut_Mt > 0 &&
                acc_fixed_lds_bytes(cfg.T, cfg.P, c->w.lut_Mt, c->w.lut_Mp, false, true) + 64 * acc_row_lds_bytes() <= (size_t)c->max_lds) ? 1 : 0;
    if (cfg.kf_pts_per_thread > kKfMaxPtsPerThread) cfg.kf_pts_per_thread = kKfMaxPtsPerThread;
    if (cfg.kf_pts_per_thread < 1) cfg.kf_pts_per_thread = 1;
    cfg.stage_event = c->stage_at ? c->ev_stage : nullptr; cfg.stage_at = c->stage_at;
    cfg.vec4_ok = 1;
    int64_t tot = 0, tot2 = 0; int mx1 = 0, mx2 = 0;
    for (int k = 0; k < n_pairs; k++) {
        if ((reinterpret_cast<uintptr_t>(hd[k].s2) & 15u) || (hd[k].ld2 & 3)) cfg.vec4_ok = 0;
        if (hs) hs[k] = (int32_t)tot;
        hd[k].off1 = (int32_t)tot; tot += hd[k].n1;
        hd[k].off2 = (int32_t)tot2; tot2 += hd[k].n2;
        if (hd[k].n1 > mx1) mx1 = hd[k].n1;
        if (hd[k].n2 > mx2) mx2 = hd[k].n2;
    }
    if (hs) hs[n_pairs] = (int32_t)tot;
    cfg.total_n1 = tot; cfg.max_n1 = mx1; cfg.max_n2 = mx2;
    if (cfg.kf_pts_per_thread == kKfMaxPtsPerThread && kKfMaxPtsPerThread >= 8 && (int64_t)n_pairs * ((mx1 + 256 * kKfMaxPtsPerThread - 1) / (256 * kKfMaxPtsPerThread)) < 128)
        cfg.kf_pts_per_thread = kKfMaxPtsPerThread / 2;
    cfg.kf_chunks = (mx1 + 256 * cfg.kf_pts_per_thread - 1) / (256 * cfg.kf_pts_per_thread);
    if (cfg.kf_chunks < 1) cfg.kf_chunks = 1;
    return cfg;
}

icet_status upload_desc(icet_ctx* c, int32_t n_pairs, bool by_next_kernel = false) {
    Workspace& w = c->w;
    if (by_next_kernel) {
    } else if (n_pairs <= kUploadDescMaxPairs) {
        HIPCHK(c, launch_upload_desc(w, c->h_desc, c->h_seg, n_pairs, c->stream));
    } else {
        HIPCHK(c, hipMemcpyAsync(w.desc, c->h_desc, sizeof(PairDesc) * n_pairs, hipMemcpyHostToDevice, c->stream));
        HIPCHK(c, hipMemcpyAsync(w.seg_off, c->h_seg, sizeof(int32_t) * (n_pairs + 1 + (c->perm_active ? n_pairs : 0)), hipMemcpyHostToDevice, c->stream));
    }
    if (!c->ev_desc) HIPCHK(c, hipEventCreateWithFlags(&c->ev_desc, hipEventDisableTiming));
    if (!c->capturing) { HIPCHK(c, hipEventRecord(c->ev_desc, c->stream)); c->desc_in_flight = true; }
    return ICET_OK;
}

icet_status enqueue_keyframe(icet_ctx* c, const icet_params* p, int32_t n_pairs, const AuxDev* aux, const int32_t* d_counts1 = nullptr) {
    Workspace& w = c->w;
    { icet_status ts = ensure_thresholds(c, p->bins_theta, p->bins_phi); if (ts != ICET_OK) return ts; }
    const LaunchCfg cfg = make_cfg(c, p, n_pairs);
    {
        const size_t need = (size_t)n_pairs * cfg.kf_chunks * (cfg.V > kRankSortMaxBuckets ? cfg.V : kRankSortMaxBuckets);
        if (need > w.cap_counts) {
            HIPCHK(c, hipStreamSynchronize(c->stream));
            HIPCHK(c, dev_realloc(w.counts, need)); HIPCHK(c, dev_realloc(w.tile_base, need));
            w.cap_counts = need;
        }
        const size_t need_vr = (size_t)n_pairs * cfg.kf_chunks * 2;
        if (need_vr > w.cap_tile_vr) {
            HIPCHK(c, hipStreamSynchronize(c->stream));
            HIPCHK(c, dev_realloc(w.tile_vr, need_vr));
            w.cap_tile_vr = need_vr;
        }
    }
    const bool first_uploads = n_pairs <= kUploadDescMaxPairs && !cfg.use_library_sort;
    { icet_status us = upload_desc(c, n_pairs, first_uploads); if (us != ICET_OK) return us; }
    if (!c->capturing) HIPCHK(c, hipEventRecord(c->ev_a, c->stream));
    LaunchCfg kcfg = cfg; if (first_uploads) { kcfg.h_desc_up = c->h_desc; kcfg.h_seg_up = c->h_seg; }
    HIPCHK(c, launch_keyframe(w, kcfg, aux, c->stream, d_counts1));
    if (first_uploads && !c->capturing) { HIPCHK(c, hipEventRecord(c->ev_desc, c->stream)); c->desc_in_flight = true; }
    return ICET_OK;
}

icet_status enqueue_rt2(icet_ctx* c, const LaunchCfg& cfg, int32_t n_pairs, const PairDesc* hd, Workspace& wl, hipEvent_t scan2_ready) {
    Workspace& w = c->w;
    int64_t tot = 0;
    for (int k = 0; k < n_pairs; k++) tot += (hd[k].n2 + 63) / 64 * 64;
    if (tot > w.cap_rt2 || !w.desc_rt || n_pairs > c->h_cap_rt) {
        HIPCHK(c, hipStreamSynchronize(c->stream));
        if (tot > w.cap_rt2) { HIPCHK(c, dev_realloc(w.rt2, (size_t)3 * tot)); w.cap_rt2 = tot; }
        if (n_pairs > c->h_cap_rt || !w.desc_rt) {
            const int np = n_pairs > w.cap_pairs ? n_pairs : w.cap_pairs;
            HIPCHK(c, dev_realloc(w.desc_rt, np));
            if (c->h_desc_rt) { HIPCHK(c, hipHostFree(c->h_desc_rt)); c->h_desc_rt = nullptr; }
            HIPCHK(c, hipHostMalloc(reinterpret_cast<void**>(&c->h_desc_rt), sizeof(PairDesc) * np));
            c->h_cap_rt = np;
        }
    } else if (c->desc_in_flight) { HIPCHK(c, hipEventSynchronize(c->ev_desc)); c->desc_in_flight = false; }
    int64_t o = 0;
    for (int k = 0; k < n_pairs; k++) {
        const int64_t l = (hd[k].n2 + 63) / 64 * 64;
        PairDesc dr = hd[k];
        dr.s2 = w.rt2 + 3 * o; dr.ld2 = (int32_t)l;
        c->h_desc_rt[k] = dr; o += l;
    }
    HIPCHK(c, hipMemcpyAsync(w.desc_rt, c->h_desc_rt, sizeof(PairDesc) * n_pairs, hipMemcpyHostToDevice, c->stream));
    HIPCHK(c, hipEventRecord(c->ev_desc, c->stream)); c->desc_in_flight = true;
    if (scan2_ready) HIPCHK(c, hipStreamWaitEvent(c->stream, scan2_ready, 0));
    wl.desc_rt = w.desc_rt; wl.rt2 = w.rt2; wl.cap_rt2 = w.cap_rt2;
    HIPCHK(c, launch_rt2_prepare(wl, cfg, c->stream));
    wl.desc = w.desc_rt;
    return ICET_OK;
}

icet_status enqueue_loop(icet_ctx* c, const icet_params* p, int32_t n_pairs, const float* d_x0, float* d_out, const AuxDev* aux, bool reupload, float* pts2_out = nullptr, hipEvent_t scan2_ready = nullptr, const int32_t* d_counts2 = nullptr) {
    const bool want_pts2 = aux && aux->xf_last && p->runlen > 0;
    Workspace& w = c->w;
    const LaunchCfg cfg = make_cfg(c, p, n_pairs);
    const bool init_uploads = reupload && n_pairs <= kUploadDescMaxPairs && !cfg.rt2 && !cfg.keep;
    if (reupload) { icet_status us = upload_desc(c, n_pairs, init_uploads); if (us != ICET_OK) return us; }
    if (d_counts2 && cfg.rt2) HIPCHK(c, launch_patch_counts(w, cfg, nullptr, d_counts2, c->stream));
    while ((int)c->ev_acc.size() < 2 * p->runlen) { hipEvent_t e; HIPCHK(c, hipEventCreate(&e)); c->ev_acc.push_back(e); }
    Workspace wl = w;
    if (!c->capturing) HIPCHK(c, hipEventRecord(c->ev_b, c->stream));
    if (cfg.rt2) { const icet_status rs = enqueue_rt2(c, cfg, n_pairs, c->h_desc, wl, scan2_ready); if (rs != ICET_OK) return rs; }
    LaunchCfg lcfg = cfg; if (cfg.rt2) lcfg.vec4_ok = 1;
    if (cfg.keep) {
        int64_t tot2 = 0; for (int k = 0; k < n_pairs; k++) tot2 += c->h_desc[k].n2;
        const size_t need_mask = (size_t)(tot2 >> 8) + (size_t)n_pairs + 2, need_list = (size_t)(tot2 >> 2) + (size_t)n_pairs + 4;
        if (need_mask > w.cap_keep_mask || need_list > w.cap_keep_list || n_pairs > w.cap_keep_pairs) {
            if (c->capturing) { c->err = "keep list: workspace growth during capture"; return ICET_ERR_HIP; }
            HIPCHK(c, hipStreamSynchronize(c->stream));
            if (need_mask > w.cap_keep_mask) { HIPCHK(c, dev_realloc(w.keep_mask, need_mask)); w.cap_keep_mask = need_mask; }
            if (need_list > w.cap_keep_list) { HIPCHK(c, dev_realloc(w.keep_list, need_list)); w.cap_keep_list = need_list; }
            if (n_pairs > w.cap_keep_pairs) { HIPCHK(c, dev_realloc(w.keep_state, (size_t)n_pairs)); HIPCHK(c, dev_realloc(w.keep_modes, 2 * (size_t)n_pairs)); w.cap_keep_pairs = n_pairs; }
            wl.keep_modes = w.keep_modes; wl.keep_mask = w.keep_mask; wl.keep_list = w.keep_list; wl.keep_state = w.keep_state; wl.cap_keep_mask = w.cap_keep_mask; wl.cap_keep_list = w.cap_keep_list; wl.cap_keep_pairs = w.cap_keep_pairs;
        }
    }
    HIPCHK(c, launch_init_state(w, cfg, d_x0, c->stream, want_pts2 ? aux->xf_last : nullptr, cfg.rt2 ? nullptr : d_counts2, init_uploads ? c->h_desc : nullptr, init_uploads ? c->h_seg : nullptr));
    if (init_uploads && !c->capturing) { HIPCHK(c, hipEventRecord(c->ev_desc, c->stream)); c->desc_in_flight = true; }
    auto enqueue_points2 = [&]() -> icet_status {
        HIPCHK(c, hipEventRecord(c->ev_prev, c->stream));
        if (!pts2_out) return ICET_OK;
        HIPCHK(c, hipStreamWaitEvent(c->st_copy, c->ev_prev, 0));
        HIPCHK(c, launch_points2(wl, lcfg, aux->xf_last, c->d_pts2, c->st_copy));
        HIPCHK(c, hipMemcpyAsync(pts2_out, c->d_pts2, sizeof(float) * 3 * (size_t)c->h_desc[0].n2, hipMemcpyDeviceToHost, c->st_copy));
        HIPCHK(c, hipEventRecord(c->ev_pts2, c->st_copy));
        return ICET_OK;
    };
    if (scan2_ready) HIPCHK(c, hipStreamWaitEvent(c->stream, scan2_ready, 0));
    if (want_pts2 && p->runlen == 1) { const icet_status ps = enqueue_points2(); if (ps != ICET_OK) return ps; }
    const bool per_iter = (p->flags & ICET_FLAG_TIMING) != 0;
    for (int it = 0; it < p->runlen; it++) {
        if (per_iter) HIPCHK(c, hipEventRecord(c->ev_acc[2 * it], c->stream));
        const FuseArgs fa{it, d_out, aux};
        bool fused = false;
        const int keep_pass = (lcfg.keep && it >= lcfg.keep_from) ? 1 : 0;
        HIPCHK(c, launch_gn_accumulate(wl, lcfg, c->stream, per_iter ? nullptr : &fa, &fused, keep_pass ? 1 + 2 * (it & 1) : 0));
        if (per_iter) HIPCHK(c, hipEventRecord(c->ev_acc[2 * it + 1], c->stream));
        if (!fused) HIPCHK(c, launch_gn_solve(wl, lcfg, it, d_out, aux, c->stream, keep_pass ? (it + 1 < p->runlen ? 1 : 2) : 0));
        if (want_pts2 && it == p->runlen - 2) { const icet_status ps = enqueue_points2(); if (ps != ICET_OK) return ps; }
    }
    if (!c->capturing) { HIPCHK(c, hipEventRecord(c->ev_c, c->stream)); c->timing_valid = true; c->last_iters = per_iter ? p->runlen : 0; }
    return ICET_OK;
}

icet_status enqueue(icet_ctx* c, const icet_params* p, int32_t n_pairs, const float* d_x0, float* d_out, const AuxDev* aux) {
    c->kf_pairs = 0;
    icet_status s = enqueue_keyframe(c, p, n_pairs, aux);
    if (s != ICET_OK) return s;
    return enqueue_loop(c, p, n_pairs, d_x0, d_out, aux, false);
}

struct IndexedDev { const int32_t* kf_of; const int32_t* rows; };
icet_status enqueue_indexed(icet_ctx* c, const icet_params* p, int32_t n_regs, const float* d_x0, float* d_out, icet_score* d_score = nullptr, int iters = -1,
                            const icet_keyframe_store* src = nullptr, const IndexedDev* dev = nullptr) {
    if (iters < 0) iters = p->runlen;
    Workspace& w = c->w;
    LaunchCfg cfg = make_cfg(c, p, n_regs, c->h_desc_reg, nullptr);
    cfg.pair_user = nullptr; cfg.done_flag = nullptr; cfg.keep = 0; cfg.fuse_solve = 0; cfg.kf_of = w.kf_of;
    Workspace wl = w; wl.desc = w.desc_reg; wl.seg_off = w.kf_of;
    if (src) { wl.hotS = src->hotS; wl.fitS = src->fitS; wl.slot_of_voxel = src->slot_of_voxel; wl.n_slots = src->n_slots; }
    const bool init_uploads = n_regs <= kUploadDescMaxPairs && !cfg.rt2;
    if (!init_uploads) {
        if (n_regs <= kUploadDescMaxPairs) HIPCHK(c, launch_upload_desc(wl, c->h_desc_reg, c->h_kf_of, n_regs, c->stream));
        else {
            HIPCHK(c, hipMemcpyAsync(w.desc_reg, c->h_desc_reg, sizeof(PairDesc) * n_regs, hipMemcpyHostToDevice, c->stream));
            HIPCHK(c, hipMemcpyAsync(w.kf_of, c->h_kf_of, sizeof(int32_t) * (n_regs + 1), hipMemcpyHostToDevice, c->stream));
        }
        if (!c->ev_desc) HIPCHK(c, hipEventCreateWithFlags(&c->ev_desc, hipEventDisableTiming));
        HIPCHK(c, hipEventRecord(c->ev_desc, c->stream)); c->desc_in_flight = true;
    }
    while ((int)c->ev_acc.size() < 2 * p->runlen) { hipEvent_t e; HIPCHK(c, hipEventCreate(&e)); c->ev_acc.push_back(e); }
    if (!c->capturing) HIPCHK(c, hipEventRecord(c->ev_a, c->stream));
    if (!c->capturing) HIPCHK(c, hipEventRecord(c->ev_b, c->stream));
    if (cfg.rt2 && dev) HIPCHK(c, launch_patch_counts(wl, cfg, nullptr, dev->rows, c->stream));
    if (cfg.rt2) { const icet_status rs = enqueue_rt2(c, cfg, n_regs, c->h_desc_reg, wl, nullptr); if (rs != ICET_OK) return rs; }
    LaunchCfg lcfg = cfg; if (cfg.rt2) lcfg.vec4_ok = 1;
    HIPCHK(c, launch_init_state(wl, lcfg, d_x0, c->stream, nullptr, dev ? dev->rows : nullptr, init_uploads ? c->h_desc_reg : nullptr, init_uploads ? c->h_kf_of : nullptr));
    if (dev) HIPCHK(c, launch_closure_apply(w.kf_of, dev->kf_of, n_regs, c->stream));
    if (init_uploads && !c->capturing) {
        if (!c->ev_desc) HIPCHK(c, hipEventCreateWithFlags(&c->ev_desc, hipEventDisableTiming));
        HIPCHK(c, hipEventRecord(c->ev_desc, c->stream)); c->desc_in_flight = true;
    }
    const bool per_iter = (p->flags & ICET_FLAG_TIMING) != 0;
    for (int it = 0; it < iters; it++) {
        if (per_iter) HIPCHK(c, hipEventRecord(c->ev_acc[2 * it], c->stream));
        HIPCHK(c, launch_gn_accumulate(wl, lcfg, c->stream));
        if (per_iter) HIPCHK(c, hipEventRecord(c->ev_acc[2 * it + 1], c->stream));
        HIPCHK(c, launch_gn_solve(wl, lcfg, it, d_out, nullptr, c->stream));
    }
    if (d_score) {
        HIPCHK(c, launch_gn_accumulate(wl, lcfg, c->stream));
        HIPCHK(c, launch_gn_score(wl, lcfg, p->runlen, d_score, c->stream));
    }
    if (!c->capturing) { HIPCHK(c, hipEventRecord(c->ev_c, c->stream)); c->timing_valid = true; c->last_iters = per_iter ? p->runlen : 0; }
    return ICET_OK;
}

icet_status ensure_stage(icet_ctx* c, int64_t tot1, int64_t tot2) {
    if (3 * tot1 > c->cap_stage1 || 3 * tot2 > c->cap_stage2) {
        HIPCHK(c, hipStreamSynchronize(c->stream));
        if (c->st_copy) HIPCHK(c, hipStreamSynchronize(c->st_copy));
        if (3 * tot1 > c->cap_stage1) { HIPCHK(c, dev_realloc(c->d_stage1, (size_t)3 * tot1)); c->cap_stage1 = 3 * tot1; }
        if (3 * tot2 > c->cap_stage2) { HIPCHK(c, dev_realloc(c->d_stage2, (size_t)3 * tot2)); c->cap_stage2 = 3 * tot2; }
    }
    return ICET_OK;
}

icet_status write_runlen0(icet_ctx* c, int32_t n_pairs, const float* d_x0, float* d_out) {
    HIPCHK(c, hipMemsetAsync(d_out, 0, sizeof(float) * 48 * (size_t)n_pairs, c->stream));
    if (d_x0) HIPCHK(c, hipMemcpy2DAsync(d_out, 48 * sizeof(float), d_x0, 6 * sizeof(float), 6 * sizeof(float), n_pairs, hipMemcpyDeviceToDevice, c->stream));
    return ICET_OK;
}

}

extern "C" {

const char* icet_version(void) { return "icet_hip 0.1 (gfx950)"; }

const char* icet_last_error(const icet_ctx* ctx) { return ctx ? ctx->err.c_str() : "null context"; }

icet_status icet_create(icet_ctx** out, int device_id, void* hip_stream) {
    if (!out) return ICET_ERR_BAD_ARG;
    *out = nullptr;
    int ndev = 0;
    if (hipGetDeviceCount(&ndev) != hipSuccess || ndev <= 0) return ICET_ERR_NO_DEVICE;
    if (device_id < 0 || device_id >= ndev) return ICET_ERR_NO_DEVICE;
    if (hipSetDevice(device_id) != hipSuccess) return ICET_ERR_NO_DEVICE;
    icet_ctx* c = new (std::nothrow) icet_ctx();
    if (!c) return ICET_ERR_NOMEM;
    c->device = device_id;
    if (hip_stream) { c->stream = reinterpret_cast<hipStream_t>(hip_stream); c->own_stream = false; }
    else {
        if (hipStreamCreateWithFlags(&c->stream, hipStreamNonBlocking) != hipSuccess) { delete c; return ICET_ERR_HIP; }
        c->own_stream = true;
    }
    if (hipEventCreate(&c->ev_a) != hipSuccess || hipEventCreate(&c->ev_b) != hipSuccess || hipEventCreate(&c->ev_c) != hipSuccess) { delete c; return ICET_ERR_HIP; }
    int lds = 0;
    if (hipDeviceGetAttribute(&lds, hipDeviceAttributeMaxSharedMemoryPerBlock, device_id) == hipSuccess && lds > 0) c->max_lds = lds;
    if (init_keyframe_kernels() != hipSuccess || init_accumulate_kernels() != hipSuccess || init_rank_sort_kernels() != hipSuccess) {
        (void)hipGetLastError();
        if (c->own_stream) (void)hipStreamDestroy(c->stream);
        delete c; return ICET_ERR_HIP;
    }
    {
        int32_t* d_t = nullptr; int ok = 0;
        if (hipMalloc(reinterpret_cast<void**>(&d_t), sizeof(int32_t)) == hipSuccess) { if (lds_rank_selftest(d_t, c->stream, &ok) != hipSuccess) { ok = 0; (void)hipGetLastError(); } (void)hipFree(d_t); }
        c->lds_rank_ok = ok;
    }
    if (hipHostMalloc(reinterpret_cast<void**>(&c->h_sync_word), sizeof(int32_t), hipHostMallocCoherent) == hipSuccess) *c->h_sync_word = 0;
    else { c->h_sync_word = nullptr; (void)hipGetLastError(); }
    *out = c;
    return ICET_OK;
}

icet_status icet_destroy(icet_ctx* c) {
    if (!c) return ICET_ERR_BAD_ARG;
    (void)hipSetDevice(c->device);
    (void)hipStreamSynchronize(c->stream);
    Workspace& w = c->w;
    void* ps[] = {w.key64A, w.key64B, w.bin16, w.execbits, w.binpos, w.bkt, w.splitters, w.n_buckets, w.bucket_start, w.counts, w.tile_base, w.desc, w.seg_off, w.r1, w.cart1, w.keyA, w.keyB, w.valA, w.valB, w.pred, w.src,
                  w.desc_rt, w.rt2, w.gn_part, w.bin_count, w.bin_start, w.hotD, w.fitD, w.activeD, w.midD, w.hotS, w.fitS, w.slot_of_voxel, w.n_slots, w.near_over, w.near_over_count, w.acc, w.xf, w.X, w.flags, w.zero_rows, w.vrange, w.tile_vr,
                  w.sort_tmp, w.fit_items, w.fit_n_items, w.live_bins, w.n_live, w.thr, w.lut, w.keep_mask, w.keep_list, w.keep_state, w.keep_modes, w.edges, w.desc_reg, w.kf_of, c->d_stage1, c->d_stage2, c->d_out, c->d_x0};
    for (void* p : ps) if (p) (void)hipFree(p);
    free_aux(c);
    if (c->st_copy) (void)hipStreamSynchronize(c->st_copy);
    if (c->h_pts2) (void)hipHostFree(c->h_pts2);
    if (c->d_pts2) (void)hipFree(c->d_pts2);
    for (void* q : {(void*)c->d_sph1, (void*)c->d_idx1, (void*)c->d_sph2, (void*)c->d_vox2}) if (q) (void)hipFree(q);
    if (c->h_x0) (void)hipHostFree(c->h_x0);
    if (c->d_score) (void)hipFree(c->d_score);
    if (c->h_score) (void)hipHostFree(c->h_score);
    if (c->d_sel) (void)hipFree(c->d_sel);
    if (c->h_sel) (void)hipHostFree(c->h_sel);
    if (c->ev_sel) (void)hipEventDestroy(c->ev_sel);
    if (c->h_sync_word) (void)hipHostFree(c->h_sync_word);
    for (hipEvent_t e : {c->ev_s2, c->ev_kf, c->ev_kfd, c->ev_prev, c->ev_pts2}) if (e) (void)hipEventDestroy(e);
    if (c->st_copy) (void)hipStreamDestroy(c->st_copy);
    if (c->h_desc) (void)hipHostFree(c->h_desc);
    if (c->h_seg) (void)hipHostFree(c->h_seg);
    if (c->h_desc_rt) (void)hipHostFree(c->h_desc_rt);
    if (c->h_desc_reg) (void)hipHostFree(c->h_desc_reg);
    if (c->h_kf_of) (void)hipHostFree(c->h_kf_of);
    if (c->h_out) (void)hipHostFree(c->h_out);
    for (hipEvent_t e : c->ev_acc) (void)hipEventDestroy(e);
    if (c->ev_a) (void)hipEventDestroy(c->ev_a);
    if (c->ev_b) (void)hipEventDestroy(c->ev_b);
    if (c->ev_c) (void)hipEventDestroy(c->ev_c);
    for (icet_ctx* h : c->helpers) (void)icet_destroy(h);
    if (c->ev_fork) (void)hipEventDestroy(c->ev_fork);
    if (c->ev_desc) (void)hipEventDestroy(c->ev_desc);
    for (icet_ctx::GraphSlot* g : {&c->g_solve, &c->g_keyframe, &c->g_loop, &c->g_indexed, &c->g_scored, &c->g_score}) if (g->have_graph) { (void)hipGraphExecDestroy(g->exec); (void)hipGraphDestroy(g->graph); }
    if (c->ev_graph) (void)hipEventDestroy(c->ev_graph);
    if (c->ev_stage) (void)hipEventDestroy(c->ev_stage);
    if (c->ev_join) (void)hipEventDestroy(c->ev_join);
    if (c->own_stream && c->stream) (void)hipStreamDestroy(c->stream);
    delete c;
    return ICET_OK;
}

icet_status icet_sync(icet_ctx* c) {
    if (!c) return ICET_ERR_BAD_ARG;
    if (c->armed_calls == 1 && c->h_sync_word) {
        volatile int32_t* w = c->h_sync_word;
        for (long spins = 1; *w == 0; spins++)
            if ((spins & 8191) == 0 && hipStreamQuery(c->stream) != hipErrorNotReady) break;
        (void)hipGetLastError();
        if (*w != 0) { __atomic_thread_fence(__ATOMIC_ACQUIRE); c->armed_calls = 0; return ICET_OK; }
    }
    HIPCHK(c, hipStreamSynchronize(c->stream));
    c->armed_calls = 0;
    return ICET_OK;
}

static int batch_parts(const icet_ctx* c, const icet_params* p, int32_t n_pairs);
static icet_status ensure_helpers(icet_ctx* c, int parts);

icet_status icet_reserve(icet_ctx* c, const icet_params* p, int32_t n_pairs, int64_t total_n1, int64_t total_n2) {
    if (!c || !params_ok(p) || n_pairs < 0 || total_n1 < 0 || total_n2 < 0) return ICET_ERR_BAD_ARG;
    HIPCHK(c, hipSetDevice(c->device));
    const int parts = batch_parts(c, p, n_pairs);
    if (parts > 1) {
        icet_status hs = ensure_helpers(c, parts);
        if (hs != ICET_OK) return hs;
        const int np = (n_pairs + parts - 1) / parts;
        const int64_t n1 = total_n1 / parts + total_n1 / (8 * parts) + 1;
        const int64_t n2 = total_n2 / parts + total_n2 / (8 * parts) + 1;
        for (icet_ctx* h : c->helpers) { hs = ensure_workspace(h, p, np, n1, n2); if (hs != ICET_OK) { c->err = h->err; return hs; } }
        hs = ensure_workspace(c, p, np, n1, n2);
        if (hs != ICET_OK) return hs;
        return ensure_out(c, n_pairs);
    }
    icet_status s = ensure_workspace(c, p, n_pairs, total_n1, total_n2);
    if (s != ICET_OK) return s;
    return ensure_out(c, n_pairs);
}

static int batch_parts(const icet_ctx* c, const icet_params* p, int32_t n_pairs) {
    if (p->flags & ICET_FLAG_TIMING) return 1;
    int parts = 1;
    if (c->tune.batch_parts > 0) parts = c->tune.batch_parts > 8 ? 8 : c->tune.batch_parts;
    if (parts > n_pairs) parts = n_pairs > 0 ? n_pairs : 1;
    return parts;
}

static icet_status ensure_helpers(icet_ctx* c, int parts) {
    while ((int)c->helpers.size() < parts - 1) {
        icet_ctx* h = nullptr;
        icet_status s = icet_create(&h, c->device, nullptr);
        if (s != ICET_OK) { c->err = "helper context: cannot create"; return s; }
        if (hipEventCreateWithFlags(&h->ev_join, hipEventDisableTiming) != hipSuccess) { icet_destroy(h); c->err = "helper context: event"; return ICET_ERR_HIP; }
        c->helpers.push_back(h);
    }
    if (!c->ev_fork) HIPCHK(c, hipEventCreateWithFlags(&c->ev_fork, hipEventDisableTiming));
    return ICET_OK;
}

static icet_status solve_device_part(icet_ctx* c, const icet_params* p, int32_t n_pairs, const icet_dev_scan* scan1, const icet_dev_scan* scan2,
                                     const float* d_x0, float* d_out, int64_t tot1);

icet_status icet_solve_batch_device(icet_ctx* c, const icet_params* p, int32_t n_pairs,
                                    const icet_dev_scan* scan1, const icet_dev_scan* scan2,
                                    const float* d_x0, float* d_out) {
    if (!c) return ICET_ERR_BAD_ARG;
    if (!params_ok(p) || n_pairs < 0 || (n_pairs > 0 && (!scan1 || !scan2 || !d_out))) { c->err = "bad argument"; return ICET_ERR_BAD_ARG; }
    if (n_pairs == 0) return ICET_OK;
    for (int k = 0; k < n_pairs; k++) {
        const icet_dev_scan &a = scan1[k], &b = scan2[k];
        if (a.n < 0 || b.n < 0 || a.ld < a.n || b.ld < b.n || (a.n > 0 && !a.ptr) || (b.n > 0 && !b.ptr) ||
            a.ld >= ((int64_t)1 << 30) || b.ld >= ((int64_t)1 << 30)) { c->err = "bad scan descriptor"; return ICET_ERR_BAD_ARG; }
    }
    HIPCHK(c, hipSetDevice(c->device));
    const int parts = (p->runlen == 0) ? 1 : batch_parts(c, p, n_pairs);
    auto range_tot = [&](int b, int e) { int64_t t = 0; for (int k = b; k < e; k++) t += scan1[k].n; return t; };
    if (parts == 1) return solve_device_part(c, p, n_pairs, scan1, scan2, d_x0, d_out, range_tot(0, n_pairs));
    c->armed_calls = 2;
    { icet_status s = ensure_helpers(c, parts); if (s != ICET_OK) return s; }
    HIPCHK(c, hipEventRecord(c->ev_fork, c->stream));
    const int stage = c->tune.batch_stage;
    icet_status status = ICET_OK;
    int started = 0;
    for (int i = 0; i < parts && status == ICET_OK; i++) {
        const int b = (int)((int64_t)n_pairs * i / parts), e = (int)((int64_t)n_pairs * (i + 1) / parts);
        icet_ctx* h = (i == 0) ? c : c->helpers[i - 1];
        if (h != c) { const bool relut = h->tune.guard_scale != c->tune.guard_scale || h->tune.lut_polar_quantile != c->tune.lut_polar_quantile; h->tune = c->tune; if (relut) h->w.thr_T = 0; }
        hipError_t he = hipSuccess;
        if (stage && !h->ev_stage) he = hipEventCreateWithFlags(&h->ev_stage, hipEventDisableTiming);
        h->stage_at = (i + 1 < parts) ? stage : 0;
        if (he == hipSuccess && i > 0) {
            he = hipStreamWaitEvent(h->stream, c->ev_fork, 0);
            if (he == hipSuccess && stage) { icet_ctx* prev = (i == 1) ? c : c->helpers[i - 2]; he = hipStreamWaitEvent(h->stream, prev->ev_stage, 0); }
        }
        if (he != hipSuccess) { c->err = std::string("batch part fork: ") + hipGetErrorString(he); status = ICET_ERR_HIP; break; }
        if (i > 0) started = i;
        status = solve_device_part(h, p, e - b, scan1 + b, scan2 + b, d_x0 ? d_x0 + 6 * (size_t)b : nullptr, d_out + 48 * (size_t)b, range_tot(b, e));
        if (status != ICET_OK && h != c) c->err = h->err;
    }
    for (int i = 1; i <= started; i++) {
        icet_ctx* h = c->helpers[i - 1];
        if (hipEventRecord(h->ev_join, h->stream) != hipSuccess || hipStreamWaitEvent(c->stream, h->ev_join, 0) != hipSuccess) {
            (void)hipStreamSynchronize(h->stream);
            if (status == ICET_OK) { c->err = "batch part join failed"; status = ICET_ERR_HIP; }
        }
    }
    return status;
}

extern "C++" {
static icet_ctx::GraphKey graph_key_of(icet_ctx* c, const icet_params* p, int32_t n_pairs, const void* a0, const void* a1, const void* a2, const void* a3, PairDesc* hd = nullptr,
                                       int64_t src_id = 0, int64_t src_gen = 0) {
    icet_ctx::GraphKey key{};
    const LaunchCfg k = make_cfg(c, p, n_pairs, hd, hd ? nullptr : c->h_seg);
    auto bits = [](float f) { int32_t i; std::memcpy(&i, &f, 4); return (int64_t)i; };
    const int64_t vals[] = {k.T, k.P, k.V, k.n, k.runlen, bits(k.thresh), bits(k.buff), k.n_pairs, k.max_n1, k.max_n2, k.total_n1, k.lds_slots, k.acc_min_pts_per_thread,
                            k.acc_target_blocks, k.kf_chunks, k.kf_pts_per_thread, k.use_library_sort, k.vec4_ok, k.true_sort, k.force_exact, k.rs_cap, k.rs_max_cell,
                            k.exec_bits_lds, k.exec_pairwise, k.lds_rank, k.reject_moving, k.half_gap, k.rt2 + 2 * k.ref_w, p->flags, (int64_t)(intptr_t)a0, (int64_t)(intptr_t)a1, (int64_t)(intptr_t)a2, (int64_t)(intptr_t)a3,
                            (int64_t)(intptr_t)c->w.desc, (int64_t)(intptr_t)c->w.thr, (int64_t)(intptr_t)c->w.lut, (int64_t)(intptr_t)c->w.r1, (int64_t)(intptr_t)c->w.counts,
                            (int64_t)(intptr_t)c->w.near_over, (int64_t)(intptr_t)c->w.acc, (int64_t)(intptr_t)c->w.fit_items, (int64_t)(intptr_t)c->w.sort_tmp, (int64_t)(intptr_t)c->w.tile_vr,
                            c->prologue ? c->prologue_key : 0, (int64_t)(intptr_t)c->done_flag, src_id, src_gen};
    static_assert(sizeof(vals) == sizeof(key.v), "GraphKey size");
    std::memcpy(key.v, vals, sizeof(vals));
    return key;
}
static bool graph_eligible(const icet_ctx* c, const icet_params* p, int32_t n_pairs) {
#ifdef ICET_DIAG_ENV
    static const bool env_off = getenv("ICET_NO_GRAPH") != nullptr;
#else
    constexpr bool env_off = false;
#endif
    return !env_off && c->graph_mode && n_pairs <= 8 && !(p->flags & (ICET_FLAG_TIMING | ICET_FLAG_ROUNDTRIP_SCAN2)) && !c->stage_at;
}
template <typename Enq> static icet_status run_or_replay(icet_ctx* c, icet_ctx::GraphSlot& slot, const icet_ctx::GraphKey& key, Enq enq) {
    auto same = [](const icet_ctx::GraphKey& a, const icet_ctx::GraphKey& b) { return std::memcmp(&a, &b, sizeof(a)) == 0; };
    if (slot.have_graph && same(key, slot.key)) {
        HIPCHK(c, hipGraphLaunch(slot.exec, c->stream));
        HIPCHK(c, hipEventRecord(c->ev_graph, c->stream)); c->graph_in_flight = true;
        c->timing_valid = false;
        return ICET_OK;
    }
    if (slot.have_seen && same(key, slot.seen)) {
        if (slot.have_graph) { (void)hipGraphExecDestroy(slot.exec); (void)hipGraphDestroy(slot.graph); slot.have_graph = false; }
        if (!c->ev_graph) HIPCHK(c, hipEventCreateWithFlags(&c->ev_graph, hipEventDisableTiming));
        HIPCHK(c, hipStreamBeginCapture(c->stream, hipStreamCaptureModeThreadLocal));
        c->capturing = true;
        const icet_status es = enq();
        c->capturing = false;
        hipGraph_t g = nullptr;
        const hipError_t ee = hipStreamEndCapture(c->stream, &g);
        if (es != ICET_OK || ee != hipSuccess || !g) {
            if (g) (void)hipGraphDestroy(g);
            (void)hipGetLastError();
            slot.have_seen = false;
            return enq();
        }
        hipGraphExec_t ge = nullptr;
        if (hipGraphInstantiate(&ge, g, nullptr, nullptr, 0) != hipSuccess) { (void)hipGraphDestroy(g); (void)hipGetLastError(); slot.have_seen = false; return enq(); }
        slot.graph = g; slot.exec = ge; slot.key = key; slot.have_graph = true;
        HIPCHK(c, hipGraphLaunch(slot.exec, c->stream));
        HIPCHK(c, hipEventRecord(c->ev_graph, c->stream)); c->graph_in_flight = true;
        c->timing_valid = false;
        return ICET_OK;
    }
    slot.seen = key; slot.have_seen = true;
    return enq();
}
}

static icet_status solve_device_part(icet_ctx* c, const icet_params* p, int32_t n_pairs, const icet_dev_scan* scan1, const icet_dev_scan* scan2,
                                     const float* d_x0, float* d_out, int64_t tot1) {
    int64_t tot2 = 0; for (int k = 0; k < n_pairs; k++) tot2 += scan2[k].n;
    c->kf_pairs = 0;
    icet_status s = ensure_workspace(c, p, n_pairs, tot1, tot2);
    if (s != ICET_OK) return s;
    if (c->desc_in_flight) { HIPCHK(c, hipEventSynchronize(c->ev_desc)); c->desc_in_flight = false; }
    if (c->graph_in_flight) { HIPCHK(c, hipEventSynchronize(c->ev_graph)); c->graph_in_flight = false; }
    c->desc_kf_valid = c->desc_reg_valid = false;
    c->perm_active = false; c->perm_pairs = n_pairs;
    std::vector<int32_t> order((size_t)n_pairs);
    for (int k = 0; k < n_pairs; k++) order[(size_t)k] = k;
    if (n_pairs > kUploadDescMaxPairs && p->runlen > 0) {
        std::vector<int64_t> size((size_t)n_pairs);
        for (int k = 0; k < n_pairs; k++) size[(size_t)k] = scan1[k].n + scan2[k].n;
        if (icet_layout::is_ragged(size)) {
            order = icet_layout::balanced_slot_order(size);
            for (int s = 0; s < n_pairs; s++) c->h_seg[n_pairs + 1 + s] = order[(size_t)s];
            c->perm_active = true;
        }
    }
    for (int s = 0; s < n_pairs; s++) {
        const int k = order[(size_t)s];
        PairDesc& d = c->h_desc[s];
        d.s1 = scan1[k].ptr; d.s2 = scan2[k].ptr;
        d.n1 = (int32_t)scan1[k].n; d.ld1 = (int32_t)scan1[k].ld; d.n2 = (int32_t)scan2[k].n; d.ld2 = (int32_t)scan2[k].ld;
        d.off1 = 0; d.off2 = 0;
    }
    if (p->runlen == 0) { c->armed_calls = 2; return write_runlen0(c, n_pairs, d_x0, d_out); }
    if (graph_eligible(c, p, n_pairs)) {
        icet_status ts = ensure_thresholds(c, p->bins_theta, p->bins_phi);
        if (ts != ICET_OK) return ts;
        const bool own_word = !c->done_flag && c->h_sync_word;
        if (own_word) { if (c->armed_calls == 0) *static_cast<volatile int32_t*>(c->h_sync_word) = 0; c->done_flag = c->h_sync_word; }
        const icet_status rs = run_or_replay(c, c->g_solve, graph_key_of(c, p, n_pairs, d_x0, d_out, nullptr, nullptr), [&]() { return enqueue(c, p, n_pairs, d_x0, d_out, nullptr); });
        if (own_word) { c->done_flag = nullptr; c->armed_calls = (rs == ICET_OK && c->g_solve.have_graph) ? c->armed_calls + 1 : 2; }
        return rs;
    }
    c->armed_calls = 2;
    return enqueue(c, p, n_pairs, d_x0, d_out, nullptr);
}

icet_status icet_keyframe_device(icet_ctx* c, const icet_params* p, int32_t n_pairs, const icet_dev_scan* scan1) {
    return icet_keyframe_device_n(c, p, n_pairs, scan1, nullptr);
}

icet_status icet_keyframe_device_n(icet_ctx* c, const icet_params* p, int32_t n_pairs, const icet_dev_scan* scan1, const int32_t* d_rows) {
    if (!c) return ICET_ERR_BAD_ARG;
    if (!params_ok(p) || n_pairs < 1 || !scan1) { c->err = "bad argument"; return ICET_ERR_BAD_ARG; }
    int64_t tot1 = 0;
    for (int k = 0; k < n_pairs; k++) {
        const icet_dev_scan& a = scan1[k];
        if (a.n < 0 || a.ld < a.n || (a.n > 0 && !a.ptr) || a.ld >= ((int64_t)1 << 30)) { c->err = "bad scan descriptor"; return ICET_ERR_BAD_ARG; }
        tot1 += a.n;
    }
    HIPCHK(c, hipSetDevice(c->device));
    c->kf_pairs = 0; c->perm_active = false; c->armed_calls = 2;
    icet_status s = ensure_workspace(c, p, n_pairs, tot1, 0);
    if (s != ICET_OK) return s;
    bool same_desc = c->desc_kf_valid;
    for (int k = 0; k < n_pairs && same_desc; k++) {
        const PairDesc& d = c->h_desc[k];
        same_desc = d.s1 == scan1[k].ptr && d.n1 == (int32_t)scan1[k].n && d.ld1 == (int32_t)scan1[k].ld;
    }
    if (!same_desc) {
        c->desc_reg_valid = false;
        if (c->desc_in_flight) { HIPCHK(c, hipEventSynchronize(c->ev_desc)); c->desc_in_flight = false; }
        if (c->graph_in_flight) { HIPCHK(c, hipEventSynchronize(c->ev_graph)); c->graph_in_flight = false; }
        for (int k = 0; k < n_pairs; k++) {
            PairDesc& d = c->h_desc[k];
            d.s1 = scan1[k].ptr; d.n1 = (int32_t)scan1[k].n; d.ld1 = (int32_t)scan1[k].ld;
            d.s2 = nullptr; d.n2 = 0; d.ld2 = 0; d.off1 = 0; d.off2 = 0;
        }
        c->desc_kf_valid = true;
    }
    if (graph_eligible(c, p, n_pairs)) {
        s = ensure_thresholds(c, p->bins_theta, p->bins_phi);
        if (s == ICET_OK) s = run_or_replay(c, c->g_keyframe, graph_key_of(c, p, n_pairs, d_rows, nullptr, nullptr, (const void*)1), [&]() { return enqueue_keyframe(c, p, n_pairs, nullptr, d_rows); });
    } else s = enqueue_keyframe(c, p, n_pairs, nullptr, d_rows);
    if (s != ICET_OK) return s;
    c->kf_pairs = n_pairs; c->kf_params = *p;
    return ICET_OK;
}

icet_status icet_register_device(icet_ctx* c, const icet_params* p, int32_t n_pairs, const icet_dev_scan* scan2, const float* d_x0, float* d_out) {
    return icet_register_device_n(c, p, n_pairs, scan2, nullptr, d_x0, d_out);
}

icet_status icet_register_device_n(icet_ctx* c, const icet_params* p, int32_t n_pairs, const icet_dev_scan* scan2, const int32_t* d_rows, const float* d_x0, float* d_out) {
    if (!c) return ICET_ERR_BAD_ARG;
    if (!params_ok(p) || n_pairs < 1 || !scan2 || !d_out) { c->err = "bad argument"; return ICET_ERR_BAD_ARG; }
    const icet_params& q = c->kf_params;
    if (c->kf_pairs != n_pairs || q.bins_phi != p->bins_phi || q.bins_theta != p->bins_theta || q.n != p->n || q.thresh != p->thresh || q.buff != p->buff ||
        ((q.flags ^ p->flags) & (ICET_FLAG_TRUE_SORT | ICET_FLAG_HALF_GAP_BOUNDS))) { c->err = "no keyframe with these parameters is parked in this context (icet_keyframe_device)"; return ICET_ERR_BAD_ARG; }
    int64_t tot2 = 0;
    for (int k = 0; k < n_pairs; k++) {
        const icet_dev_scan& b = scan2[k];
        if (b.n < 0 || b.ld < b.n || (b.n > 0 && !b.ptr) || b.ld >= ((int64_t)1 << 30)) { c->err = "bad scan descriptor"; return ICET_ERR_BAD_ARG; }
        tot2 += b.n;
    }
    HIPCHK(c, hipSetDevice(c->device));
    c->armed_calls = 2;
    if (p->runlen == 0) return write_runlen0(c, n_pairs, d_x0, d_out);
    icet_status s = ensure_workspace(c, p, n_pairs, 0, tot2);
    if (s != ICET_OK) return s;
    bool same_desc = c->desc_reg_valid;
    for (int k = 0; k < n_pairs && same_desc; k++) {
        const PairDesc& d = c->h_desc[k];
        same_desc = d.s2 == scan2[k].ptr && d.n2 == (int32_t)scan2[k].n && d.ld2 == (int32_t)scan2[k].ld;
    }
    if (!same_desc) {
        if (c->desc_in_flight) { HIPCHK(c, hipEventSynchronize(c->ev_desc)); c->desc_in_flight = false; }
        if (c->graph_in_flight) { HIPCHK(c, hipEventSynchronize(c->ev_graph)); c->graph_in_flight = false; }
        for (int k = 0; k < n_pairs; k++) { PairDesc& d = c->h_desc[k]; d.s2 = scan2[k].ptr; d.n2 = (int32_t)scan2[k].n; d.ld2 = (int32_t)scan2[k].ld; }
        c->desc_reg_valid = true;
    }
    s = ensure_thresholds(c, p->bins_theta, p->bins_phi);
    if (s != ICET_OK) return s;
    auto enq = [&]() -> icet_status {
        if (c->prologue) HIPCHK(c, c->prologue(c->prologue_user, c->stream));
        return enqueue_loop(c, p, n_pairs, d_x0, d_out, nullptr, true, nullptr, nullptr, d_rows);
    };
    if (graph_eligible(c, p, n_pairs)) return run_or_replay(c, c->g_loop, graph_key_of(c, p, n_pairs, d_x0, d_out, d_rows, (const void*)2), enq);
    return enq();
}

enum IndexedMode { kIdxRegister = 0, kIdxScored = 1, kIdxScoreOnly = 2 };
static icet_status register_indexed(icet_ctx* c, const icet_params* p, int32_t n_regs, const int32_t* kf_index, const icet_dev_scan* scan2, const float* d_x0, float* d_out,
                                    icet_score* d_score, IndexedMode mode, const icet_keyframe_store* src = nullptr, const IndexedDev* dev = nullptr) {
    if (!c) return ICET_ERR_BAD_ARG;
    const bool need_out = mode != kIdxScoreOnly, need_score = mode != kIdxRegister;
    if (!params_ok(p) || n_regs < 0 || (n_regs > 0 && (!kf_index || !scan2 || (need_out && !d_out) || (need_score && !d_score) || (mode == kIdxScoreOnly && !d_x0)))) { c->err = "bad argument"; return ICET_ERR_BAD_ARG; }
    if (n_regs == 0) return ICET_OK;
    const icet_params& q = src ? src->shape : c->kf_params;
    const int32_t n_kf = src ? src->capacity : c->kf_pairs;
    if (n_kf < 1 || q.bins_phi != p->bins_phi || q.bins_theta != p->bins_theta || q.n != p->n || q.thresh != p->thresh || q.buff != p->buff ||
        ((q.flags ^ p->flags) & (ICET_FLAG_TRUE_SORT | ICET_FLAG_HALF_GAP_BOUNDS))) {
        c->err = src ? "the grid, n, thresh, buff or keyframe-shaping flags differ from the keyframe store's shape" : "no keyframe with these parameters is parked in this context (icet_keyframe_device)";
        return ICET_ERR_BAD_ARG;
    }
    int64_t tot2 = 0;
    for (int r = 0; r < n_regs; r++) {
        if (src && (kf_index[r] < 0 || kf_index[r] >= n_kf || !src->occupied[(size_t)kf_index[r]])) {
            c->err = "slot_index[" + std::to_string(r) + "] = " + std::to_string(kf_index[r]) + " is not an occupied slot of the store (capacity " + std::to_string(n_kf) + ")"; return ICET_ERR_BAD_ARG;
        }
        if (kf_index[r] < 0 || kf_index[r] >= n_kf) { c->err = "kf_index[" + std::to_string(r) + "] = " + std::to_string(kf_index[r]) + " is not a parked keyframe (0 .. " + std::to_string(c->kf_pairs - 1) + ")"; return ICET_ERR_BAD_ARG; }
        const icet_dev_scan& b = scan2[r];
        if (b.n < 0 || b.ld < b.n || (b.n > 0 && !b.ptr) || b.ld >= ((int64_t)1 << 30)) { c->err = "bad scan descriptor"; return ICET_ERR_BAD_ARG; }
        tot2 += b.n;
    }
    if (c->tune.keep != 0) { c->err = "indexed registrations run the plain point pass: option \"keep\" must be 0"; return ICET_ERR_UNSUPPORTED; }
    HIPCHK(c, hipSetDevice(c->device));
    c->armed_calls = 2;
    if (mode == kIdxRegister && p->runlen == 0) return write_runlen0(c, n_regs, d_x0, d_out);
    icet_status s = ensure_regs(c, n_regs, p->bins_phi * p->bins_theta);
    if (s == ICET_OK) s = ensure_scan2(c, tot2);
    if (s == ICET_OK) s = ensure_thresholds(c, p->bins_theta, p->bins_phi);
    if (s != ICET_OK) return s;
    if (c->desc_in_flight) { HIPCHK(c, hipEventSynchronize(c->ev_desc)); c->desc_in_flight = false; }
    if (c->graph_in_flight) { HIPCHK(c, hipEventSynchronize(c->ev_graph)); c->graph_in_flight = false; }
    for (int r = 0; r < n_regs; r++) {
        PairDesc& d = c->h_desc_reg[r];
        d.s1 = nullptr; d.n1 = 0; d.ld1 = 0; d.off1 = 0; d.off2 = 0;
        d.s2 = scan2[r].ptr; d.n2 = (int32_t)scan2[r].n; d.ld2 = (int32_t)scan2[r].ld;
        c->h_kf_of[r] = kf_index[r];
    }
    c->h_kf_of[n_regs] = 0;
    if (mode == kIdxRegister) {
        auto enq = [&]() { return enqueue_indexed(c, p, n_regs, d_x0, d_out, nullptr, -1, src, dev); };
        if (!dev && graph_eligible(c, p, n_regs)) return run_or_replay(c, c->g_indexed, graph_key_of(c, p, n_regs, d_x0, d_out, reinterpret_cast<const void*>((intptr_t)c->ws_gen), (const void*)3, c->h_desc_reg,
                                                                  src ? src->id : 0, src ? src->gen : 0), enq);
        return enq();
    }
    const bool no_iters = mode == kIdxScoreOnly || p->runlen == 0;
    auto enq = [&]() -> icet_status {
        if (mode == kIdxScored && p->runlen == 0) { const icet_status ws = write_runlen0(c, n_regs, d_x0, d_out); if (ws != ICET_OK) return ws; }
        return enqueue_indexed(c, p, n_regs, d_x0, d_out, d_score, no_iters ? 0 : p->runlen, src, dev);
    };
    if (!dev && graph_eligible(c, p, n_regs)) {
        const intptr_t tag = (intptr_t)c->ws_gen | ((intptr_t)mode << 56);
        return run_or_replay(c, mode == kIdxScored ? c->g_scored : c->g_score,
                             graph_key_of(c, p, n_regs, d_x0, d_out, reinterpret_cast<const void*>(tag), d_score, c->h_desc_reg, src ? src->id : 0, src ? src->gen : 0), enq);
    }
    return enq();
}

icet_status icet_register_indexed_device(icet_ctx* c, const icet_params* p, int32_t n_regs, const int32_t* kf_index, const icet_dev_scan* scan2, const float* d_x0, float* d_out) {
    return register_indexed(c, p, n_regs, kf_index, scan2, d_x0, d_out, nullptr, kIdxRegister);
}

icet_status icet_register_indexed_scored_device(icet_ctx* c, const icet_params* p, int32_t n_regs, const int32_t* kf_index, const icet_dev_scan* scan2,
                                                const float* d_x0, float* d_out, icet_score* d_score) {
    return register_indexed(c, p, n_regs, kf_index, scan2, d_x0, d_out, d_score, kIdxScored);
}

icet_status icet_score_indexed_device(icet_ctx* c, const icet_params* p, int32_t n_regs, const int32_t* kf_index, const icet_dev_scan* scan2,
                                      const float* d_X, icet_score* d_score) {
    return register_indexed(c, p, n_regs, kf_index, scan2, d_X, nullptr, d_score, kIdxScoreOnly);
}

#define STORECHK(s, call) do { hipError_t e_ = (call); if (e_ != hipSuccess) { \
    (s)->err = std::string(#call) + ": " + hipGetErrorString(e_); \
    return e_ == hipErrorOutOfMemory ? ICET_ERR_NOMEM : ICET_ERR_HIP; } } while (0)

constexpr size_t kPoseBytes = sizeof(int64_t) + 12 * sizeof(float);

static hipError_t store_alloc(int V, int32_t cap, SlotHot*& hot, SlotFit*& fit, int16_t*& sov, int32_t*& ns) {
    hot = nullptr; fit = nullptr; sov = nullptr; ns = nullptr;
    hipError_t e = hipMalloc(reinterpret_cast<void**>(&hot), sizeof(SlotHot) * (size_t)cap * V);
    if (e == hipSuccess) e = hipMalloc(reinterpret_cast<void**>(&fit), sizeof(SlotFit) * (size_t)cap * V);
    if (e == hipSuccess) e = hipMalloc(reinterpret_cast<void**>(&sov), sizeof(int16_t) * (size_t)cap * ((V + 1) & ~1));
    if (e == hipSuccess) e = hipMalloc(reinterpret_cast<void**>(&ns), sizeof(int32_t) * (size_t)cap);
    if (e != hipSuccess) {
        for (void* q : {(void*)hot, (void*)fit, (void*)sov, (void*)ns}) if (q) (void)hipFree(q);
        hot = nullptr; fit = nullptr; sov = nullptr; ns = nullptr;
        (void)hipGetLastError();
    }
    return e;
}

static hipError_t app_alloc_table(size_t row_words, size_t cols, int32_t cap, uint32_t*& desc, float*& w, int32_t*& has) {
    desc = nullptr; w = nullptr; has = nullptr;
    hipError_t e = hipMalloc(reinterpret_cast<void**>(&desc), sizeof(uint32_t) * row_words * (size_t)cap);
    if (e == hipSuccess) e = hipMalloc(reinterpret_cast<void**>(&w), sizeof(float) * cols * (size_t)cap);
    if (e == hipSuccess) e = hipMalloc(reinterpret_cast<void**>(&has), sizeof(int32_t) * (size_t)cap);
    if (e != hipSuccess) {
        for (void* q : {(void*)desc, (void*)w, (void*)has}) if (q) (void)hipFree(q);
        desc = nullptr; w = nullptr; has = nullptr;
        (void)hipGetLastError();
    }
    return e;
}

const char* icet_keyframe_store_last_error(const icet_keyframe_store* s) { return s ? s->err.c_str() : "null store"; }

icet_status icet_keyframe_store_create(icet_ctx* c, const icet_params* p, int32_t capacity, icet_keyframe_store** out) {
    if (out) *out = nullptr;
    if (!c) return ICET_ERR_BAD_ARG;
    if (!out || !p || p->bins_phi <= 0 || p->bins_theta <= 0 || p->n < 1 || capacity < 1) { c->err = "bad argument"; return ICET_ERR_BAD_ARG; }
    if ((int64_t)p->bins_phi * p->bins_theta > kMaxVoxels) { c->err = "bins_phi*bins_theta exceeds the voxel limit (10000)"; return ICET_ERR_UNSUPPORTED; }
    const int V = p->bins_phi * p->bins_theta;
    if ((size_t)V * 12 + 8 + 4096 > (size_t)c->max_lds) { c->err = "grid too fine for this device's LDS (k_bin_scatter keeps 12 B per voxel in one block)"; return ICET_ERR_UNSUPPORTED; }
    HIPCHK(c, hipSetDevice(c->device));
    icet_keyframe_store* s = new (std::nothrow) icet_keyframe_store();
    if (!s) { c->err = "host allocation failed"; return ICET_ERR_NOMEM; }
    static std::atomic<int64_t> next_id{1};
    s->ctx = c; s->V = V; s->capacity = capacity; s->id = next_id++;
    s->shape = *p; s->shape.runlen = 0; s->shape.flags = p->flags & (ICET_FLAG_TRUE_SORT | ICET_FLAG_HALF_GAP_BOUNDS);
    const hipError_t e = store_alloc(V, capacity, s->hotS, s->fitS, s->slot_of_voxel, s->n_slots);
    if (e != hipSuccess) { c->err = std::string("keyframe store: ") + hipGetErrorString(e); delete s; return e == hipErrorOutOfMemory ? ICET_ERR_NOMEM : ICET_ERR_HIP; }
    s->occupied.assign((size_t)capacity, 0);
// ... 668 lines not shown
    if (!params_ok(p) || n_pairs < 0 || (n_pairs > 0 && (!scan1 || !n1 || !scan2 || !n2 || !x_out || !pred_stds_out))) { c->err = "bad argument"; return ICET_ERR_BAD_ARG; }
    if (c->pend.active) { c->err = "icet_solve_begin without icet_solve_end on this context"; return ICET_ERR_BAD_ARG; }
    if (n_pairs == 0) return ICET_OK;
    int64_t tot1 = 0, tot2 = 0;
    for (int k = 0; k < n_pairs; k++) {
        if (n1[k] < 0 || n2[k] < 0 || (n1[k] > 0 && !scan1[k]) || (n2[k] > 0 && !scan2[k])) { c->err = "bad scan"; return ICET_ERR_BAD_ARG; }
        tot1 += (n1[k] + 63) / 64 * 64; tot2 += (n2[k] + 63) / 64 * 64;
    }
    HIPCHK(c, hipSetDevice(c->device));
    icet_status s = ensure_workspace(c, p, n_pairs, tot1, tot2);
    if (s == ICET_OK) s = ensure_out(c, n_pairs);
    if (s == ICET_OK) s = ensure_host_path(c);
    if (s == ICET_OK) s = ensure_stage(c, tot1, tot2);
    if (s != ICET_OK) return s;
    if (c->desc_in_flight) { HIPCHK(c, hipEventSynchronize(c->ev_desc)); c->desc_in_flight = false; }
    int64_t o1 = 0, o2 = 0;
    c->desc_kf_valid = c->desc_reg_valid = false;
    for (int k = 0; k < n_pairs; k++) {
        const int64_t l1 = (n1[k] + 63) / 64 * 64, l2 = (n2[k] + 63) / 64 * 64;
        PairDesc& d = c->h_desc[k];
        d.s1 = c->d_stage1 + 3 * o1; d.s2 = c->d_stage2 + 3 * o2;
        d.n1 = (int32_t)n1[k]; d.ld1 = (int32_t)l1; d.n2 = (int32_t)n2[k]; d.ld2 = (int32_t)l2; d.off1 = 0; d.off2 = 0;
        HIPCHK(c, upload_scan(c->d_stage1 + 3 * o1, l1, scan1[k], n1[k], n1[k], c->stream));
        o1 += l1; o2 += l2;
    }
    const float* dx0 = nullptr;
    if (x0) { std::memcpy(c->h_x0, x0, sizeof(float) * 6 * n_pairs); HIPCHK(c, hipMemcpyAsync(c->d_x0, c->h_x0, sizeof(float) * 6 * n_pairs, hipMemcpyHostToDevice, c->stream)); dx0 = c->d_x0; }
    auto upload_scan2s = [&]() -> hipError_t {
        for (int k = 0; k < n_pairs; k++) {
            const PairDesc& d = c->h_desc[k];
            hipError_t e = upload_scan(const_cast<float*>(d.s2), d.ld2, scan2[k], n2[k], n2[k], c->st_copy);
            if (e != hipSuccess) return e;
        }
        return hipEventRecord(c->ev_s2, c->st_copy);
    };
    if (p->runlen == 0) s = write_runlen0(c, n_pairs, dx0, c->d_out);
    else {
        c->kf_pairs = 0; c->perm_active = false; c->armed_calls = 2;
        s = enqueue_keyframe(c, p, n_pairs, nullptr);
        if (s == ICET_OK) {
            const hipError_t e = upload_scan2s();
            if (e != hipSuccess) { (void)hipStreamSynchronize(c->stream); (void)hipStreamSynchronize(c->st_copy); c->err = std::string("scan-2 upload: ") + hipGetErrorString(e); return ICET_ERR_HIP; }
            s = enqueue_loop(c, p, n_pairs, dx0, c->d_out, nullptr, false, nullptr, c->ev_s2);
        }
    }
    if (s != ICET_OK) { (void)hipStreamSynchronize(c->stream); (void)hipStreamSynchronize(c->st_copy); return s; }
    HIPCHK(c, hipMemcpyAsync(c->h_out, c->d_out, sizeof(float) * 48 * n_pairs, hipMemcpyDeviceToHost, c->stream));
    HIPCHK(c, hipStreamSynchronize(c->stream));
    for (int k = 0; k < n_pairs; k++) {
        std::memcpy(x_out + 6 * k, c->h_out + 48 * k, 6 * sizeof(float));
        std::memcpy(pred_stds_out + 6 * k, c->h_out + 48 * k + 6, 6 * sizeof(float));
        if (cov_out) std::memcpy(cov_out + 36 * k, c->h_out + 48 * k + 12, 36 * sizeof(float));
    }
    return ICET_OK;
}

icet_status icet_solve_begin(icet_ctx* c, const icet_params* p, const float* scan1, int64_t n1, int64_t ld1,
                             const float* scan2, int64_t n2, int64_t ld2, const float x0[6],
                             float x_out[6], float pred_stds_out[6], float cov_out[36], icet_aux* aux) {
    if (!c) return ICET_ERR_BAD_ARG;
    if (!params_ok(p) || n1 < 0 || n2 < 0 || ld1 < n1 || ld2 < n2 || (n1 > 0 && !scan1) || (n2 > 0 && !scan2) || !x0 || !x_out || !pred_stds_out) {
        c->err = "bad argument"; return ICET_ERR_BAD_ARG;
    }
    if (c->pend.active) { c->err = "icet_solve_begin without icet_solve_end on this context"; return ICET_ERR_BAD_ARG; }
    HIPCHK(c, hipSetDevice(c->device));
    const int V = p->bins_phi * p->bins_theta;
    const int64_t l1 = (n1 + 63) / 64 * 64, l2 = (n2 + 63) / 64 * 64;
    icet_status s = ensure_workspace(c, p, 1, l1, l2);
    if (s == ICET_OK) s = ensure_out(c, 1);
    if (s == ICET_OK) s = ensure_host_path(c);
    if (s == ICET_OK) s = ensure_stage(c, l1, l2);
    if (s == ICET_OK) s = ensure_pack(c, V, p->runlen);
    if (s != ICET_OK) return s;
    const bool want_pts2 = aux && aux->points2 && n2 > 0 && p->runlen > 0;
    if (want_pts2 && (p->flags & ICET_FLAG_ROUNDTRIP_SCAN2) && (size_t)3 * n2 > c->cap_pts2) {
        HIPCHK(c, hipStreamSynchronize(c->stream));
        if (c->st_copy) HIPCHK(c, hipStreamSynchronize(c->st_copy));
        if (c->h_pts2) { HIPCHK(c, hipHostFree(c->h_pts2)); c->h_pts2 = nullptr; c->cap_pts2 = 0; }
        const size_t want = (size_t)3 * n2 + (size_t)3 * n2 / 8;
        HIPCHK(c, dev_realloc(c->d_pts2, want));
        HIPCHK(c, hipHostMalloc(reinterpret_cast<void**>(&c->h_pts2), want * sizeof(float)));
        c->cap_pts2 = want;
    }
    const bool want_side1 = aux && p->runlen > 0 && n1 > 0 && (aux->points1_spherical || aux->point_index1 || aux->bin_start1);
    const bool want_side2 = aux && p->runlen > 0 && n2 > 0 && (aux->points2_spherical || aux->voxel2);
    if (want_side1 && (size_t)n1 > c->cap_side1) {
        HIPCHK(c, hipStreamSynchronize(c->stream));
        HIPCHK(c, dev_realloc(c->d_sph1, (size_t)3 * n1)); HIPCHK(c, dev_realloc(c->d_idx1, (size_t)n1)); c->cap_side1 = (size_t)n1;
    }
    if (want_side2 && ((size_t)n2 > c->cap_side2 || (size_t)3 * n2 > c->cap_pts2)) {
        HIPCHK(c, hipStreamSynchronize(c->stream));
        if (c->st_copy) HIPCHK(c, hipStreamSynchronize(c->st_copy));
        HIPCHK(c, dev_realloc(c->d_sph2, (size_t)3 * n2)); HIPCHK(c, dev_realloc(c->d_vox2, (size_t)n2)); c->cap_side2 = (size_t)n2;
        if ((size_t)3 * n2 > c->cap_pts2) {
            if (c->h_pts2) { HIPCHK(c, hipHostFree(c->h_pts2)); c->h_pts2 = nullptr; }
            HIPCHK(c, dev_realloc(c->d_pts2, (size_t)3 * n2));
            HIPCHK(c, hipHostMalloc(reinterpret_cast<void**>(&c->h_pts2), (size_t)3 * n2 * sizeof(float)));
            c->cap_pts2 = (size_t)3 * n2;
        }
    }
    if (c->desc_in_flight) { HIPCHK(c, hipEventSynchronize(c->ev_desc)); c->desc_in_flight = false; }
    std::memcpy(c->h_x0, x0, 6 * sizeof(float));
    HIPCHK(c, upload_scan(c->d_stage1, l1, scan1, n1, ld1, c->stream));
    c->desc_kf_valid = c->desc_reg_valid = false;
    PairDesc& d = c->h_desc[0];
    d.s1 = c->d_stage1; d.s2 = c->d_stage2; d.n1 = (int32_t)n1; d.ld1 = (int32_t)l1; d.n2 = (int32_t)n2; d.ld2 = (int32_t)l2; d.off1 = 0; d.off2 = 0;
    const AuxLayout L = aux_layout(V, p->runlen);
    float* h_res = reinterpret_cast<float*>(c->h_pack) + L.out;
    float* d_res = reinterpret_cast<float*>(c->d_pack) + L.out;
    AuxDev ad = c->aux_dev;
    icet_ctx::Pending& q = c->pend;
    q = icet_ctx::Pending{};
    icet_status st = ICET_OK;
    if (p->runlen == 0) {
        std::memset(h_res, 0, 48 * sizeof(float)); std::memcpy(h_res, x0, 6 * sizeof(float));
        if (aux && aux->points2 && n2 > 0)
            for (int k = 0; k < 3; k++) std::memcpy(aux->points2 + (size_t)k * n2, scan2 + (size_t)k * ld2, (size_t)n2 * sizeof(float));
    } else {
        if (aux) {
            const size_t rl = p->runlen, v = (size_t)V;
            if (aux->n2_raw) HIPCHK(c, hipMemsetAsync(ad.n2_raw, 0, sizeof(int32_t) * rl * v, c->stream)); else ad.n2_raw = nullptr;
            if (aux->n2_in) HIPCHK(c, hipMemsetAsync(ad.n2_in, 0, sizeof(int32_t) * rl * v, c->stream)); else ad.n2_in = nullptr;
            q.kf_tables = aux->cluster_bounds || aux->has_fit || aux->mu1 || aux->sigma1 || aux->evecs1 || aux->l_diag || aux->test_points;
            q.tail_ints = aux->n1_raw || aux->n2_raw || aux->n2_in;
            q.pts2 = want_pts2 && !want_side2; q.pts2_dev = q.pts2 && (p->flags & ICET_FLAG_ROUNDTRIP_SCAN2) != 0;
            q.side1 = want_side1; q.side2 = want_side2; q.n1 = n1;
            q.scan2 = scan2; q.ld2 = ld2;
            if (!want_pts2 && !want_side2) ad.xf_last = nullptr;
        }
        c->kf_pairs = 0; c->perm_active = false; c->armed_calls = 2;
        st = enqueue_keyframe(c, p, 1, aux ? &ad : nullptr);
        if (st == ICET_OK && want_side1) {
            const LaunchCfg scfg = make_cfg(c, p, 1);
            HIPCHK(c, launch_side_scan1(c->w, scfg, c->d_sph1, c->d_idx1, c->stream));
        }
        if (st == ICET_OK) {
            hipError_t e = upload_scan(c->d_stage2, l2, scan2, n2, ld2, c->st_copy);
            if (e == hipSuccess) e = hipEventRecord(c->ev_s2, c->st_copy);
            if (e == hipSuccess && q.kf_tables) {
                e = hipEventRecord(c->ev_kf, c->stream);
                if (e == hipSuccess) e = hipStreamWaitEvent(c->st_copy, c->ev_kf, 0);
                if (e == hipSuccess) e = hipMemcpyAsync(c->h_pack + L.bounds, c->d_pack + L.bounds, (L.kf_end - L.bounds) * sizeof(uint32_t), hipMemcpyDeviceToHost, c->st_copy);
                if (e == hipSuccess) e = hipEventRecord(c->ev_kfd, c->st_copy);
            }
            if (e != hipSuccess) { (void)hipStreamSynchronize(c->stream); (void)hipStreamSynchronize(c->st_copy); c->err = std::string("scan-2 upload / table download: ") + hipGetErrorString(e); return ICET_ERR_HIP; }
            st = enqueue_loop(c, p, 1, c->h_x0, d_res, aux ? &ad : nullptr, false, q.pts2_dev ? c->h_pts2 : nullptr, c->ev_s2);
            if (st == ICET_OK) HIPCHK(c, hipMemcpyAsync(c->h_pack + L.out, c->d_pack + L.out, (aux ? L.small_end : 48) * sizeof(uint32_t), hipMemcpyDeviceToHost, c->stream));
        }
        if (st == ICET_OK && want_side2) {
            LaunchCfg scfg = make_cfg(c, p, 1);
            Workspace wl = c->w; if (scfg.rt2) wl.desc = c->w.desc_rt;
            HIPCHK(c, launch_side_scan2(wl, scfg, ad.xf_last, c->d_pts2, c->d_sph2, c->d_vox2, c->stream));
        }
        if (st == ICET_OK && q.tail_ints)
            HIPCHK(c, hipMemcpyAsync(c->h_pack + L.n1_raw, c->d_pack + L.n1_raw, (L.ints_end - L.n1_raw) * sizeof(uint32_t), hipMemcpyDeviceToHost, c->stream));
    }
    if (st != ICET_OK) { (void)hipStreamSynchronize(c->stream); (void)hipStreamSynchronize(c->st_copy); return st; }
    q.active = true; q.x_out = x_out; q.ps_out = pred_stds_out; q.cov_out = cov_out; q.has_aux = aux != nullptr && p->runlen > 0;
    q.aux = aux ? *aux : icet_aux{}; q.V = V; q.rl = p->runlen; q.n2 = n2;
    return ICET_OK;
}

icet_status icet_solve_keyframe_tables(icet_ctx* c) {
    if (!c) return ICET_ERR_BAD_ARG;
    icet_ctx::Pending& q = c->pend;
    if (!q.active) { c->err = "icet_solve_keyframe_tables without icet_solve_begin"; return ICET_ERR_BAD_ARG; }
    if (!q.has_aux || !q.kf_tables || q.kf_done) return ICET_OK;
    HIPCHK(c, hipSetDevice(c->device));
    HIPCHK(c, hipEventSynchronize(c->ev_kfd));
    const AuxLayout L = aux_layout(q.V, q.rl);
    const icet_aux& a = q.aux; const size_t v = (size_t)q.V;
    auto add = [&](void* dst, size_t at, size_t n) { if (dst && n) std::memcpy(dst, c->h_pack + at, n * sizeof(uint32_t)); };
    add(a.cluster_bounds, L.bounds, v * 6); add(a.has_fit, L.has_fit, v); add(a.mu1, L.mu1, v * 3); add(a.sigma1, L.sigma1, v * 9);
    add(a.evecs1, L.evecs1, v * 9); add(a.l_diag, L.l_diag, v * 3); add(a.test_points, L.test_points, v * 18);
    q.kf_done = true;
    return ICET_OK;
}

icet_status icet_solve_end(icet_ctx* c) {
    if (!c) return ICET_ERR_BAD_ARG;
    icet_ctx::Pending& q = c->pend;
    if (!q.active) { c->err = "icet_solve_end without icet_solve_begin"; return ICET_ERR_BAD_ARG; }
    HIPCHK(c, hipSetDevice(c->device));
    icet_status ks = icet_solve_keyframe_tables(c);
    q.active = false;
    if (q.has_aux && q.pts2 && ks == ICET_OK) {
        if (q.pts2_dev) {
            HIPCHK(c, hipEventSynchronize(c->ev_pts2));
            std::memcpy(q.aux.points2, c->h_pts2, (size_t)3 * q.n2 * sizeof(float));
        } else {
            HIPCHK(c, hipEventSynchronize(c->ev_prev));
            const AuxLayout Lp = aux_layout(q.V, q.rl);
            host_points2(reinterpret_cast<const float*>(c->h_pack) + Lp.xf_last, q.scan2, q.ld2, q.n2, q.aux.points2);
        }
    }
    HIPCHK(c, hipStreamSynchronize(c->stream));
    if (q.rl > 0) HIPCHK(c, hipStreamSynchronize(c->st_copy));
    if (ks != ICET_OK) return ks;
    const AuxLayout L = aux_layout(q.V, q.rl);
    const float* out = reinterpret_cast<const float*>(c->h_pack) + L.out;
    std::memcpy(q.x_out, out, 6 * sizeof(float));
    std::memcpy(q.ps_out, out + 6, 6 * sizeof(float));
    if (q.cov_out) std::memcpy(q.cov_out, out + 12, 36 * sizeof(float));
    if (q.has_aux) {
        const icet_aux& a = q.aux; const size_t rl = q.rl, v = (size_t)q.V;
        auto add = [&](void* dst, size_t at, size_t n) { if (dst && n) std::memcpy(dst, c->h_pack + at, n * sizeof(uint32_t)); };
        add(a.x_hist, L.x_hist, rl * 6); add(a.htwh, L.htwh, rl * 36); add(a.htwdz, L.htwdz, rl * 6); add(a.cond_info, L.cond, rl * 8);
        add(a.n1_raw, L.n1_raw, v); add(a.n2_raw, L.n2_raw, rl * v); add(a.n2_in, L.n2_in, rl * v);
        if (q.side1) {
            if (a.points1_spherical) HIPCHK(c, hipMemcpy(a.points1_spherical, c->d_sph1, sizeof(float) * 3 * (size_t)q.n1, hipMemcpyDeviceToHost));
            if (a.point_index1) HIPCHK(c, hipMemcpy(a.point_index1, c->d_idx1, sizeof(int32_t) * (size_t)q.n1, hipMemcpyDeviceToHost));
            if (a.bin_start1) HIPCHK(c, hipMemcpy(a.bin_start1, c->w.bin_start, sizeof(int32_t) * (v + 1), hipMemcpyDeviceToHost));
        }
        if (q.side2) {
            if (a.points2) HIPCHK(c, hipMemcpy(a.points2, c->d_pts2, sizeof(float) * 3 * (size_t)q.n2, hipMemcpyDeviceToHost));
            if (a.points2_spherical) HIPCHK(c, hipMemcpy(a.points2_spherical, c->d_sph2, sizeof(float) * 3 * (size_t)q.n2, hipMemcpyDeviceToHost));
            if (a.voxel2) HIPCHK(c, hipMemcpy(a.voxel2, c->d_vox2, sizeof(int32_t) * (size_t)q.n2, hipMemcpyDeviceToHost));
        }
    }
    return ICET_OK;
}

icet_status icet_solve(icet_ctx* c, const icet_params* p, const float* scan1, int64_t n1, int64_t ld1,
                       const float* scan2, int64_t n2, int64_t ld2, const float x0[6],
                       float x_out[6], float pred_stds_out[6], float cov_out[36], icet_aux* aux) {
    const icet_status s = icet_solve_begin(c, p, scan1, n1, ld1, scan2, n2, ld2, x0, x_out, pred_stds_out, cov_out, aux);
    return s == ICET_OK ? icet_solve_end(c) : s;
}

icet_status icet_debug_fetch(icet_ctx* c, int32_t what, void* out, int64_t count) {
    if (!c || !out || count < 0) return ICET_ERR_BAD_ARG;
    const Workspace& w = c->w;
    if (what == 6) { if (count != 1) return ICET_ERR_BAD_ARG; *static_cast<int32_t*>(out) = c->lds_rank_ok; return ICET_OK; }
    const void* src = nullptr; int64_t cap = w.cap_n1; size_t elem = 4;
    switch (what) {
        case 0: src = w.r1; break;
        case 1: src = w.bin16; elem = 2; break;
        case 3: src = w.src; break;
        case 4: src = w.flags; cap = w.cap_pairs; break;
        case 5: src = w.rt2; cap = 3 * w.cap_rt2; break;
        default: c->err = "unknown array id"; return ICET_ERR_BAD_ARG;
    }
    if (!src || count > cap) { c->err = "nothing to fetch / count too large"; return ICET_ERR_BAD_ARG; }
    HIPCHK(c, hipSetDevice(c->device));
    HIPCHK(c, hipStreamSynchronize(c->stream));
    HIPCHK(c, hipMemcpy(out, src, (size_t)count * elem, hipMemcpyDeviceToHost));
    return ICET_OK;
}

icet_status icet_debug_gn_tail(icet_ctx* c, const float* htwh, const float* htwdz, int32_t n, float* out) {
    if (!c || !htwh || !htwdz || !out || n < 0) return ICET_ERR_BAD_ARG;
    if (n == 0) return ICET_OK;
    HIPCHK(c, hipSetDevice(c->device));
    float* d = nullptr;
    HIPCHK(c, hipMalloc(reinterpret_cast<void**>(&d), sizeof(float) * (size_t)n * (36 + 6 + 56)));
    float* d_H = d; float* d_g = d + (size_t)n * 36; float* d_o = d_g + (size_t)n * 6;
    hipError_t e = hipMemcpyAsync(d_H, htwh, sizeof(float) * (size_t)n * 36, hipMemcpyHostToDevice, c->stream);
    if (e == hipSuccess) e = hipMemcpyAsync(d_g, htwdz, sizeof(float) * (size_t)n * 6, hipMemcpyHostToDevice, c->stream);
    if (e == hipSuccess) e = launch_gn_tail_debug(d_H, d_g, d_o, n, (float)(c->tune.gn_cond_bound * c->tune.gn_cond_bound), c->stream);
    if (e == hipSuccess) e = hipMemcpyAsync(out, d_o, sizeof(float) * (size_t)n * 56, hipMemcpyDeviceToHost, c->stream);
    if (e == hipSuccess) e = hipStreamSynchronize(c->stream);
    (void)hipFree(d);
    if (e != hipSuccess) { c->err = std::string("icet_debug_gn_tail: ") + hipGetErrorString(e); return ICET_ERR_HIP; }
    return ICET_OK;
}

icet_status icet_debug_pinv3(icet_ctx* c, const float* a, int32_t n, float* out) {
    if (!c || !a || !out || n < 0) return ICET_ERR_BAD_ARG;
    if (n == 0) return ICET_OK;
    HIPCHK(c, hipSetDevice(c->device));
    float* d = nullptr;
    HIPCHK(c, hipMalloc(reinterpret_cast<void**>(&d), sizeof(float) * (size_t)n * 18));
    hipError_t e = hipMemcpyAsync(d, a, sizeof(float) * (size_t)n * 9, hipMemcpyHostToDevice, c->stream);
    if (e == hipSuccess) e = launch_pinv3_debug(d, d + (size_t)n * 9, n, c->stream);
    if (e == hipSuccess) e = hipMemcpyAsync(out, d + (size_t)n * 9, sizeof(float) * (size_t)n * 9, hipMemcpyDeviceToHost, c->stream);
    if (e == hipSuccess) e = hipStreamSynchronize(c->stream);
    (void)hipFree(d);
    if (e != hipSuccess) { c->err = std::string("icet_debug_pinv3: ") + hipGetErrorString(e); return ICET_ERR_HIP; }
    return ICET_OK;
}

icet_status icet_debug_pinv3_double(icet_ctx* c, const float* a, int32_t n, float* out) {
    if (!c || !a || !out || n < 0) return ICET_ERR_BAD_ARG;
    if (n == 0) return ICET_OK;
    HIPCHK(c, hipSetDevice(c->device));
    float* d = nullptr;
    HIPCHK(c, hipMalloc(reinterpret_cast<void**>(&d), sizeof(float) * (size_t)n * 12));
    hipError_t e = hipMemcpyAsync(d, a, sizeof(float) * (size_t)n * 6, hipMemcpyHostToDevice, c->stream);
    if (e == hipSuccess) e = launch_pinv3_double_debug(d, d + (size_t)n * 6, n, c->stream);
    if (e == hipSuccess) e = hipMemcpyAsync(out, d + (size_t)n * 6, sizeof(float) * (size_t)n * 6, hipMemcpyDeviceToHost, c->stream);
    if (e == hipSuccess) e = hipStreamSynchronize(c->stream);
    (void)hipFree(d);
    if (e != hipSuccess) { c->err = std::string("icet_debug_pinv3_double: ") + hipGetErrorString(e); return ICET_ERR_HIP; }
    return ICET_OK;
}

icet_status icet_set_option(icet_ctx* c, const char* name, double value) {
    if (!c || !name) return ICET_ERR_BAD_ARG;
    Tuning& t = c->tune;
    const std::string k(name);
    const int iv = (int)value;
    if (k == "lds_slots") t.lds_slots = iv < 0 ? 0 : iv;
    else if (k == "acc_pts") t.acc_pts = iv < 1 ? 1 : iv;
    else if (k == "acc_blocks") t.acc_blocks = iv < 1 ? 1 : iv;
    else if (k == "force_exact") t.force_exact = iv != 0;
    else if (k == "library_sort") {
#ifdef ICET_DIAG_LIBSORT
        t.library_sort = iv != 0;
#else
        if (iv != 0) { c->err = "library_sort: this build has ONE sort, the hand-written rank sort (the rocPRIM A/B backend is compiled in with `make EXTRA=-DICET_DIAG_LIBSORT`)"; return ICET_ERR_UNSUPPORTED; }
#endif
    }
    else if (k == "kf_pts") t.kf_pts = iv < 1 ? 1 : (iv > kKfMaxPtsPerThread ? kKfMaxPtsPerThread : iv);
    else if (k == "batch_parts") t.batch_parts = iv < 0 ? 0 : (iv > 8 ? 8 : iv);
    else if (k == "batch_stage") t.batch_stage = (iv < 0 || iv > 4) ? 0 : iv;
    else if (k == "rs_cap") t.rs_cap = iv < 0 ? 0 : iv;
    else if (k == "rs_max_cell") t.rs_max_cell = iv < 0 ? 0 : iv;
    else if (k == "exec_bits_lds") t.exec_bits_lds = iv != 0;
    else if (k == "lds_rank") t.lds_rank = iv < 0 ? -1 : (iv != 0);
    else if (k == "exec_pairwise") t.exec_pairwise = iv < 0 ? -1 : (iv != 0);
    else if (k == "fuse_solve") { t.fuse_solve = iv < 0 ? -1 : (iv != 0); c->g_solve.have_seen = c->g_keyframe.have_seen = c->g_loop.have_seen = false; }
    else if (k == "keep") t.keep = iv != 0;
    else if (k == "keep_from") t.keep_from = iv < 0 ? 0 : iv;
    else if (k == "keep_budget_t") { if (!(value > 0.0 && value <= 100.0)) { c->err = "keep_budget_t must lie in (0, 100]"; return ICET_ERR_BAD_ARG; } t.keep_budget_t = value; }
    else if (k == "keep_budget_r") { if (!(value > 0.0 && value <= 1.0)) { c->err = "keep_budget_r must lie in (0, 1]"; return ICET_ERR_BAD_ARG; } t.keep_budget_r = value; }
    else if (k == "keep_check_scale") t.keep_check_scale = value > 0 ? value : 1.0;
    else if (k == "graph") { c->graph_mode = iv < 0 ? -1 : (iv != 0); c->g_solve.have_seen = c->g_keyframe.have_seen = c->g_loop.have_seen = false; }
    else if (k == "gn_cond_bound") { if (!(value >= 0.0 && value <= 1e6)) { c->err = "gn_cond_bound must lie in [0, 1e6]"; return ICET_ERR_BAD_ARG; } t.gn_cond_bound = value; c->g_solve.have_seen = c->g_keyframe.have_seen = c->g_loop.have_seen = false; }
    else if (k == "guard_scale") { if (!(value >= 1.0 && value <= 1024.0)) { c->err = "guard_scale must lie in [1, 1024]"; return ICET_ERR_BAD_ARG; } t.guard_scale = value; c->w.thr_T = 0; }
    else if (k == "lut_polar_quantile") { if (!(value >= 0.0 && value <= 1.0)) { c->err = "lut_polar_quantile must lie in [0, 1]"; return ICET_ERR_BAD_ARG; } t.lut_polar_quantile = value; c->w.thr_T = 0; }
    else { c->err = "unknown option: " + k; return ICET_ERR_BAD_ARG; }
    return ICET_OK;
}

}
void icet_ctx_set_stream(icet_ctx* c, hipStream_t s) { if (c) c->stream = s; }
void icet_ctx_set_done_flag(icet_ctx* c, int32_t* pinned_word) { if (c) c->done_flag = pinned_word; }
void icet_ctx_set_prologue(icet_ctx* c, hipError_t (*fn)(void*, hipStream_t), void* user, int64_t key) { if (c) { c->prologue = fn; c->prologue_user = user; c->prologue_key = key; } }
extern "C" {
void* icet_stream(icet_ctx* c) { return c ? reinterpret_cast<void*>(c->stream) : nullptr; }
int icet_device(const icet_ctx* c) { return c ? c->device : -1; }

icet_status icet_last_timing(icet_ctx* c, float out_ms[4]) {
    if (!c || !out_ms) return ICET_ERR_BAD_ARG;
    if (!c->timing_valid) { c->err = "no timed call yet"; return ICET_ERR_BAD_ARG; }
    HIPCHK(c, hipStreamSynchronize(c->stream));
    float a = 0, b = 0, acc = 0;
    HIPCHK(c, hipEventElapsedTime(&a, c->ev_a, c->ev_b));
    HIPCHK(c, hipEventElapsedTime(&b, c->ev_b, c->ev_c));
    for (int it = 0; it < c->last_iters; it++) { float t = 0; HIPCHK(c, hipEventElapsedTime(&t, c->ev_acc[2 * it], c->ev_acc[2 * it + 1])); acc += t; }
    out_ms[0] = a; out_ms[1] = b; out_ms[2] = c->last_iters ? acc : -1.f; out_ms[3] = (float)c->last_iters;
    return ICET_OK;
}

icet_status icet_last_timing_iters(icet_ctx* c, float* acc_ms, int32_t cap, int32_t* n_out) {
    if (!c || !acc_ms || !n_out || cap < 0) return ICET_ERR_BAD_ARG;
    if (!c->timing_valid) { c->err = "no timed call yet"; return ICET_ERR_BAD_ARG; }
    HIPCHK(c, hipStreamSynchronize(c->stream));
    const int n = c->last_iters < cap ? c->last_iters : cap;
    for (int it = 0; it < n; it++) HIPCHK(c, hipEventElapsedTime(&acc_ms[it], c->ev_acc[2 * it], c->ev_acc[2 * it + 1]));
    *n_out = n;
    return ICET_OK;
}

icet_status icet_keep_stats(icet_ctx* c, int32_t n_pairs, int32_t* out) {
    if (!c || !out || n_pairs < 0) return ICET_ERR_BAD_ARG;
    if (!c->w.keep_state || n_pairs > c->w.cap_keep_pairs) { c->err = "no keep-list state for that many pairs (the last call did not use the keep list)"; return ICET_ERR_BAD_ARG; }
    HIPCHK(c, hipSetDevice(c->device));
    HIPCHK(c, hipStreamSynchronize(c->stream));
    std::vector<KeepState> h((size_t)n_pairs);
    HIPCHK(c, hipMemcpy(h.data(), c->w.keep_state, sizeof(KeepState) * (size_t)n_pairs, hipMemcpyDeviceToHost));
    for (int s = 0; s < n_pairs; s++) {
        const int k = (c->perm_active && c->perm_pairs == n_pairs) ? c->h_seg[n_pairs + 1 + s] : s;
        out[4 * k] = h[s].mode; out[4 * k + 1] = h[s].n_keep; out[4 * k + 2] = h[s].list_passes; out[4 * k + 3] = h[s].builds;
    }
    return ICET_OK;
}

}
```

icet_amd/csrc/icet_internal.h:

```cpp
#pragma once
#include <hip/hip_runtime.h>
#include <stdint.h>

struct icet_score;

namespace icet {

constexpr int kAccWords = 20;
constexpr int kAccLds   = 20;
constexpr float kFixScale = 68719476736.0f;
constexpr double kFixInv = 1.0 / 68719476736.0;
#ifndef ICET_RS_BUCKET_BITS
#define ICET_RS_BUCKET_BITS 8
#endif
constexpr int kRankSortBucketBits = ICET_RS_BUCKET_BITS;
constexpr int kRankSortMaxBuckets = 1 << kRankSortBucketBits;
#ifndef ICET_KF_MAXPTS
#define ICET_KF_MAXPTS 8
#endif
constexpr int kKfMaxPtsPerThread = ICET_KF_MAXPTS;
constexpr int kMaxVoxels = 10000;
constexpr int kGnPartWords = 4 * 20 * 27;
constexpr uint16_t kRowZeroBit = 0x8000u;
constexpr uint16_t kRowNearBit = 0x4000u;
constexpr uint16_t kRowBinMask = 0x3FFFu;
constexpr uint32_t kSortedNearBit = 0x80000000u;
constexpr uint32_t kSortedZeroBit = 0x40000000u;
constexpr uint32_t kSortedRowMask = ~(kSortedNearBit | kSortedZeroBit);

struct PairDesc {
    const float* s1; const float* s2;
    int32_t n1, ld1, n2, ld2;
    int32_t off1;
    int32_t off2;
};

struct SlotHot {
    float az0, az1, el0, el1, inner, outer;
    float mu[3];
    int32_t v;
    int32_t pad[2];
};

struct SlotFit {
    float mu[3];
    float s1n[6];
    float M[9];
    int32_t n1;
    int32_t v;
};

struct FitMid {
    float mean[3];
    float cov[6];
    float inner, outer;
    int32_t cnt;
    int32_t has_fit;
    int32_t pad[3];
};
static_assert(sizeof(FitMid) == 64, "k_fit_scan1 stages this record as 16 words");

static_assert(sizeof(SlotHot) == 48 && sizeof(SlotFit) == 80, "k_compact_slots copies these records as 12 + 20 words");

struct KeepState {
    int32_t mode;
    int32_t n_keep;
    int32_t list_passes, builds;
    float ref[12];
};
static_assert(sizeof(KeepState) == 64, "one cache line quarter per pair");
struct KeepArgs { const PairDesc* desc; const unsigned long long* mask; uint32_t* list; KeepState* state; float bt2, br2; int on; int32_t* modes_next; int n_pairs; };

struct AuxDev {
    float* bounds; int32_t* n1_raw; int32_t* has_fit; float* mu1; float* sigma1; float* evecs1; float* l_diag;
    float* x_hist; float* htwh; float* htwdz; float* cond; int32_t* n2_raw; int32_t* n2_in; float* test_points;
    const int32_t* pair_user;
    int32_t* done_flag;
    uint32_t* done_count;
    int32_t done_pairs;
    float* xf_last;
};

struct Workspace {
    int32_t cap_pairs = 0; int64_t cap_n1 = 0; int32_t cap_V = 0;
    int32_t cap_regs = 0; int32_t cap_reg_V = 0;
    PairDesc* desc_reg = nullptr;
    int32_t* kf_of = nullptr;
    PairDesc* desc = nullptr;
    PairDesc* desc_rt = nullptr; float* rt2 = nullptr; int64_t cap_rt2 = 0;
    int32_t* seg_off = nullptr;
    float *r1 = nullptr;
    float *cart1 = nullptr;
    unsigned long long *key64A = nullptr, *key64B = nullptr;
    uint32_t *keyA = nullptr, *keyB = nullptr, *valA = nullptr, *valB = nullptr;
    uint32_t* splitters = nullptr; int32_t* n_buckets = nullptr; int32_t* bucket_start = nullptr;
    uint8_t* bkt = nullptr;
    uint16_t* binpos = nullptr;
    uint32_t* counts = nullptr; uint32_t* tile_base = nullptr; size_t cap_counts = 0;
    uint16_t* bin16 = nullptr;
    unsigned long long* execbits = nullptr;
    int32_t *pred = nullptr, *src = nullptr;
    int32_t *bin_count = nullptr, *bin_start = nullptr;
    SlotHot* hotD = nullptr; SlotFit* fitD = nullptr; int32_t* activeD = nullptr;
    FitMid* midD = nullptr;
    int32_t* live_bins = nullptr; int32_t* n_live = nullptr;
    void* fit_items = nullptr; size_t cap_fit_items = 0; uint32_t* fit_n_items = nullptr;
    SlotHot* hotS = nullptr; SlotFit* fitS = nullptr;
    int16_t* slot_of_voxel = nullptr; int32_t* n_slots = nullptr;
    uint32_t* acc = nullptr;
    uint32_t* near_over = nullptr; int64_t cap_n2 = 0; uint32_t* near_over_count = nullptr;
    uint32_t* gn_done() const { return near_over_count ? near_over_count + cap_regs : nullptr; }
    uint32_t* done_count() const { return near_over_count ? near_over_count + 2 * (size_t)cap_regs : nullptr; }
    float* xf = nullptr;
    float* gn_part = nullptr;
    float* X = nullptr;
    int32_t* flags = nullptr;
    int32_t* zero_rows = nullptr;
    int32_t* vrange = nullptr;
    int32_t* tile_vr = nullptr; size_t cap_tile_vr = 0;
    float* thr = nullptr; int thr_T = 0, thr_P = 0;
    void* lut = nullptr; int lut_Mt = 0, lut_Mp = 0;
    float guard_t = 0.f, guard_p = 0.f;
    int zero_voxel[4] = {0, 0, 0, 0};
    unsigned long long* keep_mask = nullptr; size_t cap_keep_mask = 0; uint32_t* keep_list = nullptr; size_t cap_keep_list = 0; KeepState* keep_state = nullptr; int32_t cap_keep_pairs = 0;
    int32_t* keep_modes = nullptr;
    float* edges = nullptr;
    void* sort_tmp = nullptr; size_t sort_tmp_bytes = 0;
};

#ifndef ICET_FUSE_DEFAULT
#define ICET_FUSE_DEFAULT 0
#endif
struct Tuning {
    int lds_slots = 0;
    int acc_pts = 4;
    int acc_blocks = 1536;
    int force_exact = 0;
    int library_sort = 0;
    int kf_pts = kKfMaxPtsPerThread;
    int batch_parts = 0;
    int batch_stage = 4;
    int rs_cap = 0;
    int rs_max_cell = 24;
    int exec_bits_lds = 1;
    int lds_rank = -1;
    int fuse_solve = ICET_FUSE_DEFAULT;
    int exec_pairwise = -1;
    double guard_scale = 1.0;
    double lut_polar_quantile = 0.25;
    int keep = 0;
    int keep_from = 1;
    double keep_budget_t = 0.08;
    double keep_budget_r = 0.008;
    double keep_check_scale = 1.0;
    double gn_cond_bound = 2.5e5;
};

struct LaunchCfg {
    int T, P, V, n, runlen;
    float thresh, buff;
    int n_pairs;
    int max_n1, max_n2;
    int64_t total_n1;
    int lds_slots = 0;
    int acc_min_pts_per_thread = 4;
    int acc_target_blocks = 1536;
    int kf_chunks = 1;
    int kf_pts_per_thread = kKfMaxPtsPerThread;
    hipEvent_t stage_event = nullptr;
    int stage_at = 0;
    int use_library_sort = 0;
    int vec4_ok = 0;
    int true_sort = 0;
    int force_exact = 0;
    int rs_cap = 0;
    int rs_max_cell = 24, exec_bits_lds = 1, exec_pairwise = -1;
    int fuse_solve = 0;
    int reject_moving = 0;
    int half_gap = 0;
    int rt2 = 0;
    int ref_w = 1;
    int lds_rank = 0;
    int keep = 0, keep_from = 1;
    float keep_bt = 0.f, keep_br = 0.f, keep_check_scale = 1.f;
    float gn_cond_bound2 = 6.25e10f;
    int32_t* done_flag = nullptr;
    const int32_t* pair_user = nullptr;
    const int32_t* kf_of = nullptr;
    const PairDesc* h_desc_up = nullptr; const int32_t* h_seg_up = nullptr;
};
constexpr float kRejectMovingThresh = 0.3f;
constexpr int kRejectMovingStartIter = 4;

hipError_t launch_keyframe(const Workspace& w, const LaunchCfg& c, const AuxDev* aux, hipStream_t st, const int32_t* d_n1 = nullptr);
hipError_t launch_init_state(const Workspace& w, const LaunchCfg& c, const float* d_x0, hipStream_t st, float* xf_last = nullptr, const int32_t* d_n2 = nullptr, const PairDesc* h_desc = nullptr, const int32_t* h_seg = nullptr);
hipError_t launch_gn_solve(const Workspace& w, const LaunchCfg& c, int iter, float* d_out, const AuxDev* aux, hipStream_t st, int keep_pass = 0);
hipError_t launch_gn_score(const Workspace& w, const LaunchCfg& c, int iter, ::icet_score* d_score, hipStream_t st);
hipError_t launch_select_best(const int32_t* d_members, const int32_t* d_offs, int n_groups, const ::icet_score* d_score, const float* d_out,
                              int32_t* d_best, float* d_best_out, hipStream_t st);
hipError_t launch_gn_tail_debug(const float* d_H, const float* d_g, float* d_out, int n, float bound2, hipStream_t st);
hipError_t launch_pinv3_debug(const float* d_A, float* d_out, int n, hipStream_t st);
hipError_t launch_pinv3_double_debug(const float* d_A, float* d_out, int n, hipStream_t st);
hipError_t launch_points2(const Workspace& w, const LaunchCfg& c, const float* xf, float* out, hipStream_t st);
struct FuseArgs { int iter; float* d_out; const AuxDev* aux; };
hipError_t launch_gn_accumulate(const Workspace& w, const LaunchCfg& c, hipStream_t st, const FuseArgs* fuse = nullptr, bool* fused = nullptr, int keep_pass = 0);
size_t acc_fixed_lds_bytes(int T, int P, int Mt, int Mp, bool small_batch, bool keep = false);
size_t acc_row_lds_bytes();
hipError_t launch_rt2_prepare(const Workspace& w, const LaunchCfg& c, hipStream_t st);
hipError_t launch_patch_counts(const Workspace& w, const LaunchCfg& c, const int32_t* d_n1, const int32_t* d_n2, hipStream_t st);
constexpr int kUploadDescMaxPairs = 64;
hipError_t launch_upload_desc(const Workspace& w, const PairDesc* h_desc, const int32_t* h_seg, int n_pairs, hipStream_t st);
constexpr int kStoreParkMax = 64;
struct StoreParkSlots { int32_t slot[kStoreParkMax]; };
hipError_t launch_keyframe_store_park(const Workspace& w, int V, int first, int count, const StoreParkSlots& dst,
                                      SlotHot* hot_dst, SlotFit* fit_dst, int16_t* sov_dst, int32_t* n_slots_dst, hipStream_t st);
constexpr int kClosureMaxQueries = 64, kClosureMaxCandidates = 32, kClosureMaxStarts = 16;
constexpr int kClosureTile = 1024;
struct PoseTable { int64_t* stamp; float* f; int32_t cap; };
struct PoseUpload { int32_t slot, pad; int64_t stamp; float tR[12]; };
static_assert(sizeof(PoseUpload) == 64, "read as one record per thread");
struct ClosureSearchArgs { float tx[kClosureMaxQueries], ty[kClosureMaxQueries], tz[kClosureMaxQueries]; int64_t stamp[kClosureMaxQueries]; };
struct ClosurePoseArgs { float R[kClosureMaxQueries][9]; float t[kClosureMaxQueries][3]; float off[kClosureMaxStarts][6]; };
static_assert(sizeof(ClosureSearchArgs) + 64 <= 4096 && sizeof(ClosurePoseArgs) + 128 <= 4096, "kernel arguments are at most 4 KB");
int closure_tiles(int32_t cap);
hipError_t launch_closure_search(const PoseTable& tab, const ClosureSearchArgs& qa, int n_queries, int K, float radius, int64_t min_gap,
                                 unsigned long long* d_part, int32_t* d_cand, unsigned long long* d_keys, hipStream_t st);
hipError_t launch_closure_resolve(const PoseTable& tab, const ClosurePoseArgs& pa, int n_queries, int K, int n_starts, int any_slot, const int32_t* d_cand,
                                  float* d_x0_base, float* d_x0, int32_t* d_kf_of, int32_t* d_rows, int32_t* d_members, int32_t* d_offs, hipStream_t st);
hipError_t launch_closure_apply(int32_t* dst, const int32_t* src, int n, hipStream_t st);
}
struct icet_closure;
namespace icet {
hipError_t launch_closure_record(const PoseTable& tab, int n_queries, int K, int n_starts, float max_chi2_per_voxel, int min_voxels, const int32_t* d_best,
                                 const int32_t* d_cand, const unsigned long long* d_keys, const float* d_x0, const float* d_out, const ::icet_score* d_score,
                                 ::icet_closure* d_closure, hipStream_t st);
hipError_t launch_closure_set_pose(const PoseTable& tab, const PoseUpload* h_up, int n, hipStream_t st);
hipError_t launch_closure_clear_pose(const PoseTable& tab, const StoreParkSlots& slots, int n, hipStream_t st);
}
namespace icet_appearance_rule { struct Consts; }
namespace icet {
constexpr int kAppBatch = 64;
struct AppScans { const float* ptr[kAppBatch]; int32_t n[kAppBatch]; int32_t ld[kAppBatch]; int32_t dst[kAppBatch]; };
struct AppStamps { int64_t stamp[kAppBatch]; int32_t slot[kAppBatch]; };
struct AppQueryStamps { int64_t stamp[kClosureMaxQueries]; };
struct AppOffsets { float off[kClosureMaxStarts][6]; };
static_assert(sizeof(AppScans) + 256 <= 4096 && kAppBatch >= kClosureMaxQueries && kAppBatch >= kStoreParkMax, "kernel arguments are at most 4 KB; a query's scans are one batch");
struct AppTable { uint32_t* desc; float* w; int32_t* has; int32_t cap, A, Rp; };
hipError_t launch_app_build(const AppScans& sc, int n_scans, const int32_t* d_rows, const icet_appearance_rule::Consts& c, uint32_t* d_scratch, hipStream_t st);
hipError_t launch_app_finish(const AppScans& sc, int n_scans, const icet_appearance_rule::Consts& c, uint32_t* d_scratch, const AppTable* tab,
                             uint8_t* d_desc, float* d_weight, hipStream_t st);
hipError_t launch_app_set_stamp(const PoseTable& tab, const AppStamps& s, int n, hipStream_t st);
hipError_t launch_app_search(const AppTable& tab, const PoseTable& poses, const uint32_t* d_qdesc, const float* d_qw, const AppQueryStamps& qs, int n_queries, int K,
                             float max_distance, int64_t min_gap, unsigned long long* d_keys_all, uint16_t* d_shift_all, unsigned long long* d_part,
                             int32_t* d_cand, unsigned long long* d_keys, hipStream_t st);
hipError_t launch_app_resolve(int cap, int A, const AppOffsets& off, int n_queries, int K, int n_starts, int any_slot, const int32_t* d_cand,
                              const unsigned long long* d_keys, const uint16_t* d_shift_all, float* d_dist, int32_t* d_shift, float* d_x0_base, int32_t* d_shift_of,
                              float* d_x0, int32_t* d_kf_of, int32_t* d_rows, int32_t* d_members, int32_t* d_offs, hipStream_t st);
hipError_t launch_app_record(const PoseTable& tab, int n_queries, int K, int n_starts, float max_chi2_per_voxel, int min_voxels, const int32_t* d_best,
                             const int32_t* d_cand, const unsigned long long* d_keys, const int32_t* d_shift_of, const float* d_x0, const float* d_out,
                             const ::icet_score* d_score, ::icet_closure* d_closure, hipStream_t st);
hipError_t launch_side_scan1(const Workspace& w, const LaunchCfg& c, float* sph, int32_t* index, hipStream_t st);
hipError_t launch_side_scan2(const Workspace& w, const LaunchCfg& c, const float* xf, float* pts, float* sph, int32_t* voxel, hipStream_t st);
hipError_t init_keyframe_kernels();
hipError_t lds_rank_selftest(int32_t* d_scratch, hipStream_t st, int* ok);
hipError_t init_accumulate_kernels();
hipError_t init_rank_sort_kernels();

hipError_t launch_rank_sort_splitters(const Workspace& w, const LaunchCfg& c, hipStream_t st, const int32_t* d_n1 = nullptr);
hipError_t launch_rank_sort(const Workspace& w, const LaunchCfg& c, hipStream_t st);

__device__ __forceinline__ int rank_sort_bucket_of(uint32_t key, const uint32_t* sp) {
    int lo = 0;
#pragma unroll
    for (int step = kRankSortMaxBuckets / 2; step > 0; step >>= 1) lo += (sp[lo + step] < key) ? step : 0;
    return lo;
}
hipError_t launch_class_scan(const uint32_t* counts, uint32_t* tile_base, int32_t* class_start, int n_classes, int chunks, int n_pairs, hipStream_t st,
                             int32_t* live = nullptr, int32_t* n_live = nullptr, int live_min = 0, uint32_t* n_items = nullptr, const int32_t* class_range = nullptr,
                             const int32_t* tile_vr = nullptr, int32_t* vrange_out = nullptr);

size_t sort_temp_bytes(int64_t total_n);
hipError_t sort_pairs_u64(void* tmp, size_t tmp_bytes, const unsigned long long* key_in, unsigned long long* key_out,
                          const uint32_t* val_in, uint32_t* val_out, int64_t total_n, int end_bit, hipStream_t st);
hipError_t sort_pairs_u32(void* tmp, size_t tmp_bytes, const uint32_t* key_in, uint32_t* key_out,
                          const uint32_t* val_in, uint32_t* val_out, int64_t total_n, int end_bit, hipStream_t st);

}

struct icet_ctx;
void icet_ctx_set_stream(icet_ctx* c, hipStream_t s);
```

Measured before the change: 127,000 scan-pairs/s.

## Issue first point loads early, skip empty parked pass, and merge two chunks per block

```diff
diff --git a/icet_amd/csrc/icet_accumulate.hip b/icet_amd/csrc/icet_accumulate.hip
--- a/icet_amd/csrc/icet_accumulate.hip
+++ b/icet_amd/csrc/icet_accumulate.hip
@@ -82,27 +82,54 @@
 }
 constexpr int kKeepOwn = 63;
 
-template <bool kVec4, bool kRT2, bool kSmall, bool kKeep, bool kIdx = false>
+template <bool kVec4, bool kRT2, bool kSmall, bool kKeep, bool kIdx = false, bool kEarly = false>
 __device__ __forceinline__ void gn_accumulate_body(const PairDesc* __restrict__ desc, const float* __restrict__ xf_all,
                                                           const int16_t* __restrict__ slot_of_voxel, const int32_t* __restrict__ n_slots,
                                                           const SlotHot* __restrict__ hotS, uint32_t* __restrict__ acc,
                                                           const float* __restrict__ thr, const LutCell* __restrict__ lut,
                                                           int T, int P, int Mt, int Mp, float guard_t, float guard_p,
-                                                          int lds_slots, int chunks, int n_pairs, int force_exact,
+                                                          int lds_slots, int chunks, int n_pairs, int flags,
                                                           uint32_t* __restrict__ near_over, uint32_t* __restrict__ near_over_count, const KeepDev& kd,
                                                           const int32_t* __restrict__ kf_of = nullptr) {
     constexpr uint32_t near_cap = kSmall ? kNearCapSmall : kNearCap;
     constexpr int kW = kAccBlock / 64;
     extern __shared__ __attribute__((aligned(16))) unsigned char smem[];
     const int V = T * P;
+    const int force_exact = flags & kAccForceExact;
+    static_assert(!kEarly || (kVec4 && !kKeep), "the early first trip is three unconditional 16-byte loads of the plain pass");
+    constexpr bool early = kEarly;
+    const int cpb = (flags & kAccTwoChunks) ? 2 : 1;
     int pair, chunk;
-    if (!decode_block(n_pairs, chunks, pair, chunk)) return;
+    if (!decode_block(n_pairs, (chunks + cpb - 1) / cpb, pair, chunk)) return;
+    chunk *= cpb;
     [[maybe_unused]] int mode_word = 0;
     if constexpr (kKeep) { pair = keep_pair_of_slot(kd.modes, n_pairs, pair, mode_word); if (pair < 0) return; }
+    int kf = pair;
+    if constexpr (kIdx) kf = __builtin_amdgcn_readfirstlane(kf_of[pair]);
+    const SlotHot* hs = hotS + (size_t)kf * V;
+    const uint32_t* gm = reinterpret_cast<const uint32_t*>(slot_of_voxel + (size_t)kf * ((V + 1) & ~1));
+    const uint2* gl = reinterpret_cast<const uint2*>(lut);
+    const int map_words = (V + 1) / 2;
+    const int n_lut = Mt + Mp + 2;
+    constexpr int kMapAhead = 2, kLutAhead = 3;
+    uint32_t mreg[kMapAhead]; uint2 lreg[kLutAhead];
+    SlotHot g0{};
+    auto request_tables = [&]() {
+#pragma unroll
+        for (int k = 0; k < kMapAhead; k++) { const int i = (int)threadIdx.x + k * kAccBlock; mreg[k] = (i < map_words) ? gm[i] : 0u; }
+#pragma unroll
+        for (int k = 0; k < kLutAhead; k++) { const int i = (int)threadIdx.x + k * kAccBlock; lreg[k] = (i < n_lut) ? gl[i] : make_uint2(0u, 0u); }
+    };
+    if constexpr (early) { request_tables(); g0 = hs[min((int)threadIdx.x, V - 1)]; }
     const PairDesc d = desc[pair];
+    const int ns = n_slots[kf];
+    const float* xf = xf_all + pair * kXf;
+    const float tx = xf[0], ty = xf[1], tz = xf[2];
+    const float R00 = xf[3], R01 = xf[4], R02 = xf[5], R10 = xf[6], R11 = xf[7], R12 = xf[8], R20 = xf[9], R21 = xf[10], R22 = xf[11];
     int cs = (d.n2 + chunks - 1) / chunks;
     cs = (cs + kAccPts * 64 - 1) / (kAccPts * 64) * (kAccPts * 64);
     const int begin = chunk * cs;
+    const int span = min(cpb, chunks - chunk) * cs;
     int list_mode = 0, nk = 0, tau_begin = 0, tau_end = 0;
     if constexpr (kKeep) { list_mode = mode_word > 0; nk = mode_word - 1; }
     if (kKeep && list_mode) {
@@ -111,7 +138,7 @@
         tau_begin = chunk * tpb; tau_end = min(n_trips, tau_begin + tpb);
         if (tau_begin >= n_trips) return;
     } else if (begin >= d.n2) return;
-    const int end = (kKeep && list_mode) ? d.n2 : min(d.n2, begin + cs);
+    const int end = (kKeep && list_mode) ? d.n2 : min(d.n2, begin + span);
     const int lane = (int)(threadIdx.x & 63u);
     const uint32_t* L = kd.list + ((size_t)d.off2 >> 2) + pair;
     const int e_max = max(nk - 1, 0);
@@ -125,50 +152,64 @@
     unsigned long long* lacc = reinterpret_cast<unsigned long long*>(lut_p + (Mp + 1));
     float* hot = reinterpret_cast<float*>(smem + (((size_t)(Mt + Mp + 2) * sizeof(LutCell) + (size_t)80 * lds_slots + 15) & ~(size_t)15));
     int16_t* map = reinterpret_cast<int16_t*>(hot + lds_slots * kHotWords);
-    const int map_words = (V + 1) / 2;
     uint32_t* nearq = reinterpret_cast<uint32_t*>(map) + (V + T + 4) / 2;
     [[maybe_unused]] float* k_edge_t = reinterpret_cast<float*>(nearq + near_cap + 5);
     [[maybe_unused]] float* k_edge_p = k_edge_t + (T + 2);
     [[maybe_unused]] uint8_t* k_nb = reinterpret_cast<uint8_t*>(k_edge_p + (P + 2)) + T;
-    int kf = pair;
-    if constexpr (kIdx) kf = __builtin_amdgcn_readfirstlane(kf_of[pair]);
-    const int ns = n_slots[kf];
     const int nl = min(ns, lds_slots);
-    const SlotHot* hs = hotS + (size_t)kf * V;
+    gfloat* px = (gfloat*)d.s2; gfloat* py = px + d.ld2; gfloat* pz = px + 2 * (size_t)d.ld2;
+    const auto load4 = [&](int i0, float (&X)[4], float (&Y)[4], float (&Z)[4]) {
+        if (kVec4 && i0 + 3 < end) {
+            const vfloat4 a = __builtin_nontemporal_load((gfloat4*)(px + i0)), b = __builtin_nontemporal_load((gfloat4*)(py + i0)), c = __builtin_nontemporal_load((gfloat4*)(pz + i0));
+            X[0] = a.x; X[1] = a.y; X[2] = a.z; X[3] = a.w; Y[0] = b.x; Y[1] = b.y; Y[2] = b.z; Y[3] = b.w; Z[0] = c.x; Z[1] = c.y; Z[2] = c.z; Z[3] = c.w;
+        } else {
+#pragma unroll
+            for (int j = 0; j < 4; j++) { const bool ok = i0 + j < end; X[j] = ok ? px[i0 + j] : __builtin_nanf(""); Y[j] = ok ? py[i0 + j] : 0.f; Z[j] = ok ? pz[i0 + j] : 0.f; }
+        }
+    };
+    float XN[4], YN[4], ZN[4];
+    vfloat4 ea, eb, ec;
     {
-        const uint32_t* gm = reinterpret_cast<const uint32_t*>(slot_of_voxel + (size_t)kf * ((V + 1) & ~1));
         uint32_t* lm = reinterpret_cast<uint32_t*>(map);
-        const uint2* gl = reinterpret_cast<const uint2*>(lut);
         uint2* ll = reinterpret_cast<uint2*>(lut_t);
-        const int n_lut = Mt + Mp + 2;
-        constexpr int kMapAhead = 2, kLutAhead = 3;
-        uint32_t mreg[kMapAhead]; uint2 lreg[kLutAhead];
-#pragma unroll
-        for (int k = 0; k < kMapAhead; k++) { const int i = (int)threadIdx.x + k * kAccBlock; mreg[k] = (i < map_words) ? gm[i] : 0u; }
-#pragma unroll
-        for (int k = 0; k < kLutAhead; k++) { const int i = (int)threadIdx.x + k * kAccBlock; lreg[k] = (i < n_lut) ? gl[i] : make_uint2(0u, 0u); }
-        SlotHot g0{};
-        if ((int)threadIdx.x < nl) g0 = hs[threadIdx.x];
-#pragma unroll
-        for (int k = 0; k < kMapAhead; k++) { const int i = (int)threadIdx.x + k * kAccBlock; if (i < map_words) lm[i] = mreg[k]; }
-        for (int i = (int)threadIdx.x + kMapAhead * kAccBlock; i < map_words; i += kAccBlock) lm[i] = gm[i];
+        const auto store_tables = [&]() {
+#pragma unroll
+            for (int k = 0; k < kMapAhead; k++) { const int i = (int)threadIdx.x + k * kAccBlock; if (i < map_words) lm[i] = mreg[k]; }
+#pragma unroll
+            for (int k = 0; k < kLutAhead; k++) { const int i = (int)threadIdx.x + k * kAccBlock; if (i < n_lut) ll[i] = lreg[k]; }
+            if ((int)threadIdx.x < nl) { float* h = hot + threadIdx.x * kHotWords; h[0] = g0.inner; h[1] = g0.outer; h[2] = g0.mu[0]; h[3] = g0.mu[1]; h[4] = g0.mu[2]; }
+        };
+        const auto copy_rest = [&]() {
+            for (int i = (int)threadIdx.x + kMapAhead * kAccBlock; i < map_words; i += kAccBlock) lm[i] = gm[i];
+            for (int i = (int)threadIdx.x + kLutAhead * kAccBlock; i < n_lut; i += kAccBlock) ll[i] = gl[i];
+            for (int i = (int)threadIdx.x + kAccBlock; i < nl; i += kAccBlock) {
+                const SlotHot g = hs[i];
+                float* h = hot + i * kHotWords;
+                h[0] = g.inner; h[1] = g.outer; h[2] = g.mu[0]; h[3] = g.mu[1]; h[4] = g.mu[2];
+            }
+        };
+        if constexpr (early) {
+            copy_rest();
+            {
+                const int i0 = begin + kAccPts * (int)threadIdx.x;
+                const bool full = i0 + 3 < end;
+                const int ia = full ? i0 : 0;
+                ea = __builtin_nontemporal_load((gfloat4*)(px + ia)); eb = __builtin_nontemporal_load((gfloat4*)(py + ia)); ec = __builtin_nontemporal_load((gfloat4*)(pz + ia));
+            }
+            store_tables();
+        } else {
+            request_tables();
+            if ((int)threadIdx.x < nl) g0 = hs[threadIdx.x];
+            store_tables();
+            copy_rest();
+        }
         for (int i = 2 * map_words + threadIdx.x; i < V + T + 2; i += kAccBlock) map[i] = (int16_t)-1;
-#pragma unroll
-        for (int k = 0; k < kLutAhead; k++) { const int i = (int)threadIdx.x + k * kAccBlock; if (i < n_lut) ll[i] = lreg[k]; }
-        for (int i = (int)threadIdx.x + kLutAhead * kAccBlock; i < n_lut; i += kAccBlock) ll[i] = gl[i];
-        for (int i = threadIdx.x; i < nl; i += kAccBlock) {
-            const SlotHot g = (i == (int)threadIdx.x) ? g0 : hs[i];
-            float* h = hot + i * kHotWords;
-            h[0] = g.inner; h[1] = g.outer; h[2] = g.mu[0]; h[3] = g.mu[1]; h[4] = g.mu[2];
-        }
         for (int i = threadIdx.x; i < 10 * nl; i += kAccBlock) lacc[i] = 0ull;
         if (threadIdx.x < 5) nearq[near_cap + threadIdx.x] = 0u;
     }
-    const float* xf = xf_all + pair * kXf;
-    const float tx = xf[0], ty = xf[1], tz = xf[2];
-    const float R00 = xf[3], R01 = xf[4], R02 = xf[5], R10 = xf[6], R11 = xf[7], R12 = xf[8], R20 = xf[9], R21 = xf[10], R22 = xf[11];
     const float cell_t = (float)Mt * 0.25f, cell_p = (float)Mp * 0.5f;
     __syncthreads();
+    if constexpr (early) asm volatile("" : "+v"(ea), "+v"(eb), "+v"(ec) : : "memory");
     if constexpr (kKeep) {
         if (!list_mode) {
             for (int i = threadIdx.x; i < T + P + 4; i += kAccBlock) {
@@ -187,23 +228,12 @@
         }
     }
 
-    gfloat* px = (gfloat*)d.s2; gfloat* py = px + d.ld2; gfloat* pz = px + 2 * (size_t)d.ld2;
     uint32_t* gacc = acc + (size_t)pair * V * kAccWords;
 
-    auto load4 = [&](int i0, float (&X)[4], float (&Y)[4], float (&Z)[4]) {
-        if (kVec4 && i0 + 3 < end) {
-            const vfloat4 a = __builtin_nontemporal_load((gfloat4*)(px + i0)), b = __builtin_nontemporal_load((gfloat4*)(py + i0)), c = __builtin_nontemporal_load((gfloat4*)(pz + i0));
-            X[0] = a.x; X[1] = a.y; X[2] = a.z; X[3] = a.w; Y[0] = b.x; Y[1] = b.y; Y[2] = b.z; Y[3] = b.w; Z[0] = c.x; Z[1] = c.y; Z[2] = c.z; Z[3] = c.w;
-        } else {
-#pragma unroll
-            for (int j = 0; j < 4; j++) { const bool ok = i0 + j < end; X[j] = ok ? px[i0 + j] : __builtin_nanf(""); Y[j] = ok ? py[i0 + j] : 0.f; Z[j] = ok ? pz[i0 + j] : 0.f; }
-        }
-    };
 #ifndef ICET_ACC_PHASE
 #define ICET_ACC_PHASE 9
 #endif
     [[maybe_unused]] float sink = 0.f;
-    float XN[4], YN[4], ZN[4];
     auto trip = [&](auto mode_c, const int i0, const bool have_next, const int i0_next, [[maybe_unused]] const int grp) {
       constexpr int kMode = decltype(mode_c)::value;
       [[maybe_unused]] const bool ghost = kMode == 2 && lane == 0;
@@ -417,13 +447,25 @@
             gc = gn; gn_raw = gnn_raw;
         }
     } else {
-        load4(begin + kAccPts * (int)threadIdx.x, XN, YN, ZN);
-        for (int t0 = begin + kAccPts * threadIdx.x; t0 < begin + cs; t0 += kAccPts * kAccBlock)
-            trip(std::integral_constant<int, kKeep ? 1 : 0>{}, t0, t0 + kAccPts * kAccBlock < begin + cs, t0 + kAccPts * kAccBlock, -1);
+        {
+            const int i0 = begin + kAccPts * (int)threadIdx.x;
+            if constexpr (early) {
+                const bool full = i0 + 3 < end;
+                const float nan = __builtin_nanf("");
+                XN[0] = full ? ea.x : nan; XN[1] = full ? ea.y : nan; XN[2] = full ? ea.z : nan; XN[3] = full ? ea.w : nan;
+                YN[0] = full ? eb.x : 0.f; YN[1] = full ? eb.y : 0.f; YN[2] = full ? eb.z : 0.f; YN[3] = full ? eb.w : 0.f;
+                ZN[0] = full ? ec.x : 0.f; ZN[1] = full ? ec.y : 0.f; ZN[2] = full ? ec.z : 0.f; ZN[3] = full ? ec.w : 0.f;
+            }
+            if (!early || ((i0 < end) & (i0 + 3 >= end))) load4(i0, XN, YN, ZN);
+        }
+        for (int t0 = begin + kAccPts * threadIdx.x; t0 < begin + span; t0 += kAccPts * kAccBlock)
+            trip(std::integral_constant<int, kKeep ? 1 : 0>{}, t0, t0 + kAccPts * kAccBlock < begin + span, t0 + kAccPts * kAccBlock, -1);
     }
     if (ICET_ACC_PHASE != 9 && sink == 1.2345e-30f) near_over_count[pair] = 1u;
     __syncthreads();
-    {
+    bool parked = true;
+    if (flags & kAccSkipParked) parked = (nearq[near_cap] | nearq[near_cap + 1] | nearq[near_cap + 2] | nearq[near_cap + 3] | nearq[near_cap + 4]) != 0u;
+    if (__ballot(parked) != 0ull) {
         const uint32_t nq = min(nearq[near_cap], near_cap);
         for (uint32_t e = threadIdx.x; e < nq; e += kAccBlock) {
             const int i = (int)nearq[e];
@@ -455,8 +497,8 @@
                 else atomicAdd(reinterpret_cast<unsigned long long*>(gacc + (size_t)pz.s * kAccWords), (unsigned long long)cnt);
             }
         }
-    }
-    __syncthreads();
+        __syncthreads();
+    }
     for (int s = threadIdx.x; s < nl; s += kAccBlock) {
         const unsigned long long* L = lacc + s * 10;
         const unsigned long long cnt = L[0];
@@ -472,7 +514,7 @@
     }
 }
 
-template <bool kVec4, bool kRT2, bool kSmall>
+template <bool kVec4, bool kRT2, bool kSmall, bool kEarly = false>
 __global__ __launch_bounds__(kAccBlock, kRT2 ? 1 : (kSmall ? 2 : kAccWavesPerSimd)) void k_gn_accumulate(const PairDesc* __restrict__ desc, const float* __restrict__ xf_all,
                                                           const int16_t* __restrict__ slot_of_voxel, const int32_t* __restrict__ n_slots,
                                                           const SlotHot* __restrict__ hotS, uint32_t* __restrict__ acc,
@@ -480,10 +522,10 @@
                                                           int T, int P, int Mt, int Mp, float guard_t, float guard_p,
                                                           int lds_slots, int chunks, int n_pairs, int force_exact,
                                                           uint32_t* __restrict__ near_over, uint32_t* __restrict__ near_over_count) {
-    gn_accumulate_body<kVec4, kRT2, kSmall, false>(desc, xf_all, slot_of_voxel, n_slots, hotS, acc, thr, lut, T, P, Mt, Mp, guard_t, guard_p, lds_slots, chunks, n_pairs, force_exact, near_over, near_over_count, KeepDev{});
-}
-
-template <bool kVec4, bool kRT2, bool kSmall>
+    gn_accumulate_body<kVec4, kRT2, kSmall, false, false, kEarly>(desc, xf_all, slot_of_voxel, n_slots, hotS, acc, thr, lut, T, P, Mt, Mp, guard_t, guard_p, lds_slots, chunks, n_pairs, force_exact, near_over, near_over_count, KeepDev{});
+}
+
+template <bool kVec4, bool kRT2, bool kSmall, bool kEarly = false>
 __global__ __launch_bounds__(kAccBlock, kRT2 ? 1 : (kSmall ? 2 : kAccWavesPerSimd)) void k_gn_accumulate_indexed(const PairDesc* __restrict__ desc, const float* __restrict__ xf_all,
                                                           const int16_t* __restrict__ slot_of_voxel, const int32_t* __restrict__ n_slots,
                                                           const SlotHot* __restrict__ hotS, uint32_t* __restrict__ acc,
@@ -491,7 +533,7 @@
                                                           int T, int P, int Mt, int Mp, float guard_t, float guard_p,
                                                           int lds_slots, int chunks, int n_pairs, int force_exact,
                                                           uint32_t* __restrict__ near_over, uint32_t* __restrict__ near_over_count, const int32_t* __restrict__ kf_of) {
-    gn_accumulate_body<kVec4, kRT2, kSmall, false, true>(desc, xf_all, slot_of_voxel, n_slots, hotS, acc, thr, lut, T, P, Mt, Mp, guard_t, guard_p, lds_slots, chunks, n_pairs, force_exact, near_over, near_over_count, KeepDev{}, kf_of);
+    gn_accumulate_body<kVec4, kRT2, kSmall, false, true, kEarly>(desc, xf_all, slot_of_voxel, n_slots, hotS, acc, thr, lut, T, P, Mt, Mp, guard_t, guard_p, lds_slots, chunks, n_pairs, force_exact, near_over, near_over_count, KeepDev{}, kf_of);
 }
 
 template <bool kVec4>
@@ -544,13 +586,15 @@
 
 hipError_t init_accumulate_kernels() {
     hipError_t e = hipSuccess;
-#define ICET_ACC_ATTR(V4, RT, SM) if (e == hipSuccess) e = hipFuncSetAttribute(reinterpret_cast<const void*>(k_gn_accumulate<V4, RT, SM>), hipFuncAttributeMaxDynamicSharedMemorySize, 160 * 1024)
+#define ICET_ACC_ATTR(...) if (e == hipSuccess) e = hipFuncSetAttribute(reinterpret_cast<const void*>(k_gn_accumulate<__VA_ARGS__>), hipFuncAttributeMaxDynamicSharedMemorySize, 160 * 1024)
     ICET_ACC_ATTR(true, false, false); ICET_ACC_ATTR(false, false, false); ICET_ACC_ATTR(true, true, false); ICET_ACC_ATTR(false, true, false);
     ICET_ACC_ATTR(true, false, true); ICET_ACC_ATTR(false, false, true); ICET_ACC_ATTR(true, true, true); ICET_ACC_ATTR(false, true, true);
+    ICET_ACC_ATTR(true, false, false, true); ICET_ACC_ATTR(true, false, true, true);
 #undef ICET_ACC_ATTR
-#define ICET_ACC_ATTR(V4, RT, SM) if (e == hipSuccess) e = hipFuncSetAttribute(reinterpret_cast<const void*>(k_gn_accumulate_indexed<V4, RT, SM>), hipFuncAttributeMaxDynamicSharedMemorySize, 160 * 1024)
+#define ICET_ACC_ATTR(...) if (e == hipSuccess) e = hipFuncSetAttribute(reinterpret_cast<const void*>(k_gn_accumulate_indexed<__VA_ARGS__>), hipFuncAttributeMaxDynamicSharedMemorySize, 160 * 1024)
     ICET_ACC_ATTR(true, false, false); ICET_ACC_ATTR(false, false, false); ICET_ACC_ATTR(true, true, false); ICET_ACC_ATTR(false, true, false);
     ICET_ACC_ATTR(true, false, true); ICET_ACC_ATTR(false, false, true); ICET_ACC_ATTR(true, true, true); ICET_ACC_ATTR(false, true, true);
+    ICET_ACC_ATTR(true, false, false, true); ICET_ACC_ATTR(true, false, true, true);
 #undef ICET_ACC_ATTR
     if (e == hipSuccess) e = hipFuncSetAttribute(reinterpret_cast<const void*>(k_gn_accumulate_keep<true>), hipFuncAttributeMaxDynamicSharedMemorySize, 160 * 1024);
     if (e == hipSuccess) e = hipFuncSetAttribute(reinterpret_cast<const void*>(k_gn_accumulate_keep<false>), hipFuncAttributeMaxDynamicSharedMemorySize, 160 * 1024);
@@ -603,21 +647,25 @@
     if (lds_slots > fit) lds_slots = fit;
     if (lds_slots > c.V) lds_slots = c.V;
     int chunks = chunks_for(c.n_pairs, c.max_n2, kAccBlock * c.acc_min_pts_per_thread, c.acc_target_blocks);
-    chunks = std::max(chunks, (int)(((long long)c.max_n2 + (1 << 20) - 1) >> 20));
+    const bool two_chunks = (c.acc_opts & kAccTwoChunks) && !fuse_it && !keep_pass && near_cap == kNearCap && chunks >= 2 && (long long)grid_groups(c.n_pairs) * chunks > 3ll * c.n_cus;
+    const int chunk_shift = two_chunks ? 19 : 20;
+    chunks = std::max(chunks, (int)(((long long)c.max_n2 + (1ll << chunk_shift) - 1) >> chunk_shift));
+    const int blocks_per_pair = two_chunks ? (chunks + 1) / 2 : chunks;
+    const int flags = (c.force_exact ? kAccForceExact : 0) | (c.acc_opts & kAccSkipParked) | (two_chunks ? kAccTwoChunks : 0);
     const size_t lds = fixed + (size_t)lds_slots * row;
-    dim3 grid(grid_groups(c.n_pairs) * chunks), blk(kAccBlock);
+    dim3 grid(grid_groups(c.n_pairs) * blocks_per_pair), blk(kAccBlock);
     const LutCell* lut = reinterpret_cast<const LutCell*>(w.lut);
-#define ICET_ACC_LAUNCH(V4, RT, SM) do { if (c.kf_of) k_gn_accumulate_indexed<V4, RT, SM><<<grid, blk, lds, st>>>(w.desc, w.xf, w.slot_of_voxel, w.n_slots, w.hotS, w.acc, w.thr, lut, c.T, c.P, w.lut_Mt, w.lut_Mp, \
-                                                     w.guard_t, w.guard_p, lds_slots, chunks, c.n_pairs, c.force_exact, w.near_over, w.near_over_count, c.kf_of); \
-                                      else k_gn_accumulate<V4, RT, SM><<<grid, blk, lds, st>>>(w.desc, w.xf, w.slot_of_voxel, w.n_slots, w.hotS, w.acc, w.thr, lut, c.T, c.P, w.lut_Mt, w.lut_Mp, \
-                                                     w.guard_t, w.guard_p, lds_slots, chunks, c.n_pairs, c.force_exact, w.near_over, w.near_over_count); } while (0)
+#define ICET_ACC_LAUNCH(...) do { if (c.kf_of) k_gn_accumulate_indexed<__VA_ARGS__><<<grid, blk, lds, st>>>(w.desc, w.xf, w.slot_of_voxel, w.n_slots, w.hotS, w.acc, w.thr, lut, c.T, c.P, w.lut_Mt, w.lut_Mp, \
+                                                     w.guard_t, w.guard_p, lds_slots, chunks, c.n_pairs, flags, w.near_over, w.near_over_count, c.kf_of); \
+                                      else k_gn_accumulate<__VA_ARGS__><<<grid, blk, lds, st>>>(w.desc, w.xf, w.slot_of_voxel, w.n_slots, w.hotS, w.acc, w.thr, lut, c.T, c.P, w.lut_Mt, w.lut_Mp, \
+                                                     w.guard_t, w.guard_p, lds_slots, chunks, c.n_pairs, flags, w.near_over, w.near_over_count); } while (0)
     if (fuse_it) {
         AuxDev aux{}; if (fuse->aux) aux = *fuse->aux;
         aux.pair_user = c.pair_user; aux.done_flag = (fuse->iter == c.runlen - 1) ? c.done_flag : nullptr;
         aux.done_count = aux.done_flag ? w.done_count() : nullptr; aux.done_pairs = c.n_pairs;
         const SolveFuse sf{w.fitS, w.X, fuse->d_out, aux, c.n, fuse->iter, c.runlen, c.reject_moving, c.gn_cond_bound2, w.gn_done()};
-        if (c.vec4_ok) k_gn_accumulate_solve<true><<<grid, blk, lds, st>>>(w.desc, w.xf, w.slot_of_voxel, w.n_slots, w.hotS, w.acc, w.thr, lut, c.T, c.P, w.lut_Mt, w.lut_Mp, w.guard_t, w.guard_p, lds_slots, chunks, c.n_pairs, c.force_exact, w.near_over, w.near_over_count, sf);
-        else k_gn_accumulate_solve<false><<<grid, blk, lds, st>>>(w.desc, w.xf, w.slot_of_voxel, w.n_slots, w.hotS, w.acc, w.thr, lut, c.T, c.P, w.lut_Mt, w.lut_Mp, w.guard_t, w.guard_p, lds_slots, chunks, c.n_pairs, c.force_exact, w.near_over, w.near_over_count, sf);
+        if (c.vec4_ok) k_gn_accumulate_solve<true><<<grid, blk, lds, st>>>(w.desc, w.xf, w.slot_of_voxel, w.n_slots, w.hotS, w.acc, w.thr, lut, c.T, c.P, w.lut_Mt, w.lut_Mp, w.guard_t, w.guard_p, lds_slots, chunks, c.n_pairs, flags, w.near_over, w.near_over_count, sf);
+        else k_gn_accumulate_solve<false><<<grid, blk, lds, st>>>(w.desc, w.xf, w.slot_of_voxel, w.n_slots, w.hotS, w.acc, w.thr, lut, c.T, c.P, w.lut_Mt, w.lut_Mp, w.guard_t, w.guard_p, lds_slots, chunks, c.n_pairs, flags, w.near_over, w.near_over_count, sf);
         ICET_LAUNCH_CHECK();
         if (fused) *fused = true;
         return hipSuccess;
@@ -626,13 +674,14 @@
         const double two_pi = 6.283185307179586476925286766559;
         const KeepDev kd{w.keep_mask, w.keep_list, w.edges, w.keep_modes + (size_t)(keep_pass >> 1) * c.n_pairs, 1.05f * c.keep_br + 1e-4f, 1.05f * c.keep_bt,
                          (float)std::min(two_pi / c.T, 0.5), (float)std::min(0.5 * two_pi / c.P, 0.5), 1.0f / (float)c.T};
-        if (c.vec4_ok) k_gn_accumulate_keep<true><<<grid, blk, lds, st>>>(w.desc, w.xf, w.slot_of_voxel, w.n_slots, w.hotS, w.acc, w.thr, lut, c.T, c.P, w.lut_Mt, w.lut_Mp, w.guard_t, w.guard_p, lds_slots, chunks, c.n_pairs, c.force_exact, w.near_over, w.near_over_count, kd);
-        else k_gn_accumulate_keep<false><<<grid, blk, lds, st>>>(w.desc, w.xf, w.slot_of_voxel, w.n_slots, w.hotS, w.acc, w.thr, lut, c.T, c.P, w.lut_Mt, w.lut_Mp, w.guard_t, w.guard_p, lds_slots, chunks, c.n_pairs, c.force_exact, w.near_over, w.near_over_count, kd);
+        if (c.vec4_ok) k_gn_accumulate_keep<true><<<grid, blk, lds, st>>>(w.desc, w.xf, w.slot_of_voxel, w.n_slots, w.hotS, w.acc, w.thr, lut, c.T, c.P, w.lut_Mt, w.lut_Mp, w.guard_t, w.guard_p, lds_slots, chunks, c.n_pairs, flags, w.near_over, w.near_over_count, kd);
+        else k_gn_accumulate_keep<false><<<grid, blk, lds, st>>>(w.desc, w.xf, w.slot_of_voxel, w.n_slots, w.hotS, w.acc, w.thr, lut, c.T, c.P, w.lut_Mt, w.lut_Mp, w.guard_t, w.guard_p, lds_slots, chunks, c.n_pairs, flags, w.near_over, w.near_over_count, kd);
         ICET_LAUNCH_CHECK();
         return hipSuccess;
     }
 #define ICET_ACC_LAUNCH2(V4, RT) do { if (near_cap == kNearCapSmall) ICET_ACC_LAUNCH(V4, RT, true); else ICET_ACC_LAUNCH(V4, RT, false); } while (0)
-    if (c.rt2) { if (c.vec4_ok) ICET_ACC_LAUNCH2(true, true); else ICET_ACC_LAUNCH2(false, true); }
+    if ((c.acc_opts & kAccEarlyLoads) && c.vec4_ok && !c.rt2) { if (near_cap == kNearCapSmall) ICET_ACC_LAUNCH(true, false, true, true); else ICET_ACC_LAUNCH(true, false, false, true); }
+    else if (c.rt2) { if (c.vec4_ok) ICET_ACC_LAUNCH2(true, true); else ICET_ACC_LAUNCH2(false, true); }
     else { if (c.vec4_ok) ICET_ACC_LAUNCH2(true, false); else ICET_ACC_LAUNCH2(false, false); }
 #undef ICET_ACC_LAUNCH2
 #undef ICET_ACC_LAUNCH
diff --git a/icet_amd/csrc/icet_capi.hip b/icet_amd/csrc/icet_capi.hip
--- a/icet_amd/csrc/icet_capi.hip
+++ b/icet_amd/csrc/icet_capi.hip
@@ -27,6 +27,7 @@
     Tuning tune;
     int32_t kf_pairs = 0; icet_params kf_params{};
     int max_lds = 160 * 1024;
+    int n_cus = 256;
     int lds_rank_ok = 0;
     std::string err;
     PairDesc* h_desc = nullptr; int32_t* h_seg = nullptr; int32_t h_cap_pairs = 0;
@@ -408,6 +409,8 @@
     cfg.rt2 = (p->flags & ICET_FLAG_ROUNDTRIP_SCAN2) ? 1 : 0;
     cfg.ref_w = (p->flags & ICET_FLAG_DOUBLE_W) ? 0 : 1;
     cfg.lds_slots = c->tune.lds_slots; cfg.acc_min_pts_per_thread = c->tune.acc_pts; cfg.acc_target_blocks = c->tune.acc_blocks;
+    cfg.n_cus = c->n_cus;
+    cfg.acc_opts = (c->tune.acc_early_loads ? kAccEarlyLoads : 0) | (c->tune.acc_skip_parked ? kAccSkipParked : 0) | (c->tune.acc_two_chunks ? kAccTwoChunks : 0);
     cfg.force_exact = c->tune.force_exact; cfg.use_library_sort = c->tune.library_sort; cfg.kf_pts_per_thread = c->tune.kf_pts; cfg.rs_cap = c->tune.rs_cap; cfg.rs_max_cell = c->tune.rs_max_cell; cfg.exec_bits_lds = c->tune.exec_bits_lds; cfg.exec_pairwise = c->tune.exec_pairwise; cfg.fuse_solve = c->tune.fuse_solve != 0 ? 1 : 0; cfg.lds_rank = (c->tune.lds_rank != 0 && c->lds_rank_ok) ? 1 : 0;
     cfg.gn_cond_bound2 = (float)(c->tune.gn_cond_bound * c->tune.gn_cond_bound);
     cfg.pair_user = (c->perm_active && c->perm_pairs == n_pairs) ? c->w.seg_off + n_pairs + 1 : nullptr;
@@ -656,6 +659,8 @@
     if (hipEventCreate(&c->ev_a) != hipSuccess || hipEventCreate(&c->ev_b) != hipSuccess || hipEventCreate(&c->ev_c) != hipSuccess) { delete c; return ICET_ERR_HIP; }
     int lds = 0;
     if (hipDeviceGetAttribute(&lds, hipDeviceAttributeMaxSharedMemoryPerBlock, device_id) == hipSuccess && lds > 0) c->max_lds = lds;
+    int cus = 0;
+    if (hipDeviceGetAttribute(&cus, hipDeviceAttributeMultiprocessorCount, device_id) == hipSuccess && cus > 0) c->n_cus = cus;
     if (init_keyframe_kernels() != hipSuccess || init_accumulate_kernels() != hipSuccess || init_rank_sort_kernels() != hipSuccess) {
         (void)hipGetLastError();
         if (c->own_stream) (void)hipStreamDestroy(c->stream);
@@ -831,7 +836,7 @@
     const LaunchCfg k = make_cfg(c, p, n_pairs, hd, hd ? nullptr : c->h_seg);
     auto bits = [](float f) { int32_t i; std::memcpy(&i, &f, 4); return (int64_t)i; };
     const int64_t vals[] = {k.T, k.P, k.V, k.n, k.runlen, bits(k.thresh), bits(k.buff), k.n_pairs, k.max_n1, k.max_n2, k.total_n1, k.lds_slots, k.acc_min_pts_per_thread,
-                            k.acc_target_blocks, k.kf_chunks, k.kf_pts_per_thread, k.use_library_sort, k.vec4_ok, k.true_sort, k.force_exact, k.rs_cap, k.rs_max_cell,
+                            k.acc_target_blocks + ((int64_t)k.acc_opts << 32), k.kf_chunks, k.kf_pts_per_thread, k.use_library_sort, k.vec4_ok, k.true_sort, k.force_exact, k.rs_cap, k.rs_max_cell,
                             k.exec_bits_lds, k.exec_pairwise, k.lds_rank, k.reject_moving, k.half_gap, k.rt2 + 2 * k.ref_w, p->flags, (int64_t)(intptr_t)a0, (int64_t)(intptr_t)a1, (int64_t)(intptr_t)a2, (int64_t)(intptr_t)a3,
                             (int64_t)(intptr_t)c->w.desc, (int64_t)(intptr_t)c->w.thr, (int64_t)(intptr_t)c->w.lut, (int64_t)(intptr_t)c->w.r1, (int64_t)(intptr_t)c->w.counts,
                             (int64_t)(intptr_t)c->w.near_over, (int64_t)(intptr_t)c->w.acc, (int64_t)(intptr_t)c->w.fit_items, (int64_t)(intptr_t)c->w.sort_tmp, (int64_t)(intptr_t)c->w.tile_vr,
@@ -2106,7 +2111,10 @@
     const int iv = (int)value;
     if (k == "lds_slots") t.lds_slots = iv < 0 ? 0 : iv;
     else if (k == "acc_pts") t.acc_pts = iv < 1 ? 1 : iv;
-    else if (k == "acc_blocks") t.acc_blocks = iv < 1 ? 1 : iv;
+    else if (k == "acc_blocks" || k == "acc_target_blocks") t.acc_blocks = iv < 1 ? 1 : iv;
+    else if (k == "acc_early_loads") t.acc_early_loads = iv != 0;
+    else if (k == "acc_skip_parked") t.acc_skip_parked = iv != 0;
+    else if (k == "acc_two_chunks") t.acc_two_chunks = iv != 0;
     else if (k == "force_exact") t.force_exact = iv != 0;
     else if (k == "library_sort") {
 #ifdef ICET_DIAG_LIBSORT
diff --git a/icet_amd/csrc/icet_internal.h b/icet_amd/csrc/icet_internal.h
--- a/icet_amd/csrc/icet_internal.h
+++ b/icet_amd/csrc/icet_internal.h
@@ -148,6 +148,9 @@
     int exec_pairwise = -1;
     double guard_scale = 1.0;
     double lut_polar_quantile = 0.25;
+    int acc_early_loads = 1;
+    int acc_skip_parked = 1;
+    int acc_two_chunks = 1;
     int keep = 0;
     int keep_from = 1;
     double keep_budget_t = 0.08;
@@ -155,6 +158,8 @@
     double keep_check_scale = 1.0;
     double gn_cond_bound = 2.5e5;
 };
+
+constexpr int kAccForceExact = 1, kAccEarlyLoads = 2, kAccSkipParked = 4, kAccTwoChunks = 8;
 
 struct LaunchCfg {
     int T, P, V, n, runlen;
@@ -165,6 +170,8 @@
     int lds_slots = 0;
     int acc_min_pts_per_thread = 4;
     int acc_target_blocks = 1536;
+    int n_cus = 256;
+    int acc_opts = 0;
     int kf_chunks = 1;
     int kf_pts_per_thread = kKfMaxPtsPerThread;
     hipEvent_t stage_event = nullptr;
```

Result: slower. 125,300 scan-pairs/s (-1.3%).
